# theAdamColton/spiht

Measured on AMD Instinct MI355X. Metric: Mpixels/sec encode+decode at fixed bpp; bitstream-exact vs Rust ref, higher is better.
Workload: dtype f64 DWT / int32 bit-plane coding; 1 GPU; cfg2 image (1920x1080 RGB, bior2.2 reflect level 7, q=50, 0.5 bpp) x 256 per GPU (cfg4 shard), encode+decode, HBM-resident; images_per_gpu=256, distinct_images_per_gpu=256, seeds=1000 + global image index, streams=1, images_per_launch=256, decoder_waves=8, max_bits=1036800

## Files before the change

include/spiht_hip.h:

```cpp
#ifndef SPIHT_HIP_H
#define SPIHT_HIP_H

#include <stdint.h>

#ifdef __cplusplus
extern "C" {
#endif

enum {
    SPIHT_OK = 0,
    SPIHT_ERR_LL = 1,
    SPIHT_ERR_EMPTY = 2,
    SPIHT_ERR_SHAPE = 3,
    SPIHT_ERR_CAPACITY = 4,
    SPIHT_ERR_HIP = 5,
    SPIHT_ERR_ARG = 6,
    SPIHT_ERR_MAGNITUDE = 7,
    SPIHT_ERR_INTERNAL = 8,
    SPIHT_ERR_TOO_LARGE = 9,
    SPIHT_ERR_NOMEM = 10
};

enum { SPIHT_MODE_REFLECT = 0, SPIHT_MODE_SYMMETRIC = 1, SPIHT_MODE_PERIODIC = 2, SPIHT_MODE_ZERO = 3,
       SPIHT_MODE_CONSTANT = 4,
// ... 85 lines not shown
                                 int64_t H, int64_t W, int wavelet, int mode, int level, double q_scale,
                                 const double *channel_mults, uint64_t max_bits, uint8_t *d_out, uint64_t slot_stride,
                                 uint64_t *d_nbits, uint8_t *d_max_n, int32_t *d_coeffs);
int spiht_decode_image_batch_u8(spiht_ctx *ctx, const uint8_t *d_data, uint64_t slot_stride,
                                const uint64_t *d_nbytes, const uint8_t *d_max_n, int64_t B, int64_t c, int64_t H,
                                int64_t W, int wavelet, int mode, int level, double q_scale,
                                const double *channel_mults, uint8_t *d_img_out, const int64_t *out_strides,
                                int32_t *d_rec);
int spiht_decode_image_batch_u16(spiht_ctx *ctx, const uint8_t *d_data, uint64_t slot_stride,
                                 const uint64_t *d_nbytes, const uint8_t *d_max_n, int64_t B, int64_t c, int64_t H,
                                 int64_t W, int wavelet, int mode, int level, double q_scale,
                                 const double *channel_mults, uint16_t *d_img_out, const int64_t *out_strides,
                                 int32_t *d_rec);

int spiht_dwt_quant_batch_f64(spiht_ctx *ctx, const double *d_img, int64_t B, int64_t c, int64_t H, int64_t W,
                              int wavelet, int mode, int level, double q_scale, const double *channel_mults,
                              int32_t *d_coeffs);
int spiht_dequant_idwt_batch_f64(spiht_ctx *ctx, const int32_t *d_rec, int64_t B, int64_t c, int64_t H, int64_t W,
                                 int wavelet, int mode, int level, double q_scale, const double *channel_mults,
                                 double *d_img_out);

int spiht_dwt_quant_batch_f32(spiht_ctx *ctx, const float *d_img, int64_t B, int64_t c, int64_t H, int64_t W,
                              int wavelet, int mode, int level, double q_scale, const double *channel_mults,
                              int32_t *d_coeffs);
int spiht_encode_image_batch_f32(spiht_ctx *ctx, const float *d_img, int64_t B, int64_t c, int64_t H, int64_t W,
                                 int wavelet, int mode, int level, double q_scale, const double *channel_mults,
                                 uint64_t max_bits, uint8_t *d_out, uint64_t slot_stride, uint64_t *d_nbits,
                                 uint8_t *d_max_n, int32_t *d_coeffs);

int spiht_pyramid_batch_i32(spiht_ctx *ctx, const int32_t *d_x, int64_t B, int64_t c, int64_t h, int64_t w,
                            int64_t ll_h, int64_t ll_w, uint8_t *d_dmsb, uint8_t *d_lmsb, uint32_t *d_maxabs);

int spiht_dwt_pyramid_batch_f64(spiht_ctx *ctx, const double *d_img, int64_t B, int64_t c, int64_t H, int64_t W,
                                int wavelet, int mode, int level, double q_scale, const double *channel_mults,
                                int32_t *d_coeffs, uint8_t *d_dmsb, uint8_t *d_lmsb, uint32_t *d_maxabs);
int spiht_dwt_pyramid_batch_u8(spiht_ctx *ctx, const uint8_t *d_img, const int64_t *strides, int64_t B, int64_t c, int64_t H,
                               int64_t W, int wavelet, int mode, int level, double q_scale, const double *channel_mults,
                               int32_t *d_coeffs, uint8_t *d_dmsb, uint8_t *d_lmsb, uint32_t *d_maxabs);
int spiht_dwt_pyramid_batch_u16(spiht_ctx *ctx, const uint16_t *d_img, const int64_t *strides, int64_t B, int64_t c, int64_t H,
                                int64_t W, int wavelet, int mode, int level, double q_scale, const double *channel_mults,
                                int32_t *d_coeffs, uint8_t *d_dmsb, uint8_t *d_lmsb, uint32_t *d_maxabs);
int spiht_encode_lists_batch_i32(spiht_ctx *ctx, const int32_t *d_x, const uint8_t *d_dmsb, const uint8_t *d_lmsb,
                                 const uint32_t *d_maxabs, int64_t B, int64_t c, int64_t h, int64_t w, int64_t ll_h,
                                 int64_t ll_w, uint64_t max_bits, uint8_t *d_out, uint64_t slot_stride,
                                 uint64_t *d_nbits, uint8_t *d_max_n);
int spiht_decode_lists_batch_i32(spiht_ctx *ctx, const uint8_t *d_data, uint64_t slot_stride, const uint64_t *d_nbytes,
                                 const uint8_t *d_max_n, int64_t B, int64_t c, int64_t h, int64_t w, int64_t ll_h,
                                 int64_t ll_w, int32_t *d_out_zeroed);
int spiht_unscatter_lists_batch_i32(spiht_ctx *ctx, int32_t *d_out, int64_t B, int64_t c, int64_t h, int64_t w);
int spiht_l1_flags_words(int64_t c, int64_t H, int64_t W, int wavelet, int mode, int level, uint64_t *words_per_image);
int spiht_decode_lists_flags_batch_i32(spiht_ctx *ctx, const uint8_t *d_data, uint64_t slot_stride, const uint64_t *d_nbytes,
                                       const uint8_t *d_max_n, int64_t B, int64_t c, int64_t H, int64_t W, int wavelet,
                                       int mode, int level, int32_t *d_out_zeroed, uint32_t *d_flags);
int spiht_dequant_idwt_flags_batch_f64(spiht_ctx *ctx, const int32_t *d_rec, const uint32_t *d_flags, int64_t B, int64_t c,
                                       int64_t H, int64_t W, int wavelet, int mode, int level, double q_scale,
                                       const double *channel_mults, double *d_img_out);
int spiht_dequant_idwt_flags_batch_u8(spiht_ctx *ctx, const int32_t *d_rec, const uint32_t *d_flags, int64_t B, int64_t c,
                                      int64_t H, int64_t W, int wavelet, int mode, int level, double q_scale,
                                      const double *channel_mults, uint8_t *d_img_out, const int64_t *out_strides);
int spiht_dequant_idwt_flags_batch_u16(spiht_ctx *ctx, const int32_t *d_rec, const uint32_t *d_flags, int64_t B, int64_t c,
                                       int64_t H, int64_t W, int wavelet, int mode, int level, double q_scale,
                                       const double *channel_mults, uint16_t *d_img_out, const int64_t *out_strides);
int spiht_ctx_set_option(spiht_ctx *ctx, const char *name, int64_t value);
int spiht_ctx_get_option(spiht_ctx *ctx, const char *name, int64_t *value);
int spiht_ctx_wide_stats(spiht_ctx *ctx, uint32_t *groups, uint32_t *gave_up);

int spiht_idwt_coarse_batch_f64(spiht_ctx *ctx, const int32_t *d_rec, int64_t B, int64_t c, int64_t H, int64_t W,
                                int wavelet, int mode, int level, double q_scale, const double *channel_mults,
                                double *d_approx);
int spiht_idwt_level1_batch_f64(spiht_ctx *ctx, const int32_t *d_rec, const double *d_approx, int64_t B, int64_t c,
                                int64_t H, int64_t W, int wavelet, int mode, int level, double q_scale,
                                const double *channel_mults, double *d_img_out);
int spiht_idwt_approx_shape(int64_t H, int64_t W, int wavelet, int level, int64_t *a_h, int64_t *a_w);
int spiht_idwt_level1_flags_batch_f64(spiht_ctx *ctx, const int32_t *d_rec, const double *d_approx, const uint32_t *d_flags,
                                      int64_t B, int64_t c, int64_t H, int64_t W, int wavelet, int mode, int level, double q_scale,
                                      const double *channel_mults, double *d_img_out);
int spiht_idwt_level1_flags_batch_u8(spiht_ctx *ctx, const int32_t *d_rec, const double *d_approx, const uint32_t *d_flags,
                                     int64_t B, int64_t c, int64_t H, int64_t W, int wavelet, int mode, int level, double q_scale,
                                     const double *channel_mults, uint8_t *d_img_out, const int64_t *out_strides);
int spiht_idwt_level1_flags_batch_u16(spiht_ctx *ctx, const int32_t *d_rec, const double *d_approx, const uint32_t *d_flags,
                                      int64_t B, int64_t c, int64_t H, int64_t W, int wavelet, int mode, int level, double q_scale,
                                      const double *channel_mults, uint16_t *d_img_out, const int64_t *out_strides);

int spiht_color3_batch_f64(spiht_ctx *ctx, const double *d_in, double *d_out, int64_t B, int64_t npix, const double *A,
                           const double *M, double p);
int spiht_ctx_set_color3(spiht_ctx *ctx, const double *A_f, const double *M_f, double p_f, const double *A_i,
                         const double *M_i, double p_i);
int spiht_ctx_get_color3(spiht_ctx *ctx, int *on, double *A_f, double *M_f, double *p_f, double *A_i, double *M_i, double *p_i);

int spiht_decode_budgets_i32(spiht_ctx *ctx, const uint8_t *data, uint64_t nbytes, uint8_t n, int64_t c, int64_t h, int64_t w,
                             int64_t ll_h, int64_t ll_w, const uint64_t *budgets_bits, int64_t K, int32_t *out);
int spiht_decode_budgets_dev_i32(spiht_ctx *ctx, const uint8_t *data, uint64_t nbytes, uint8_t n, int64_t c, int64_t h,
                                 int64_t w, int64_t ll_h, int64_t ll_w, const uint64_t *budgets_bits, int64_t K, int32_t *d_out);

int spiht_ctx_lock(spiht_ctx *ctx);
int spiht_ctx_unlock(spiht_ctx *ctx);

int spiht_ctx_set_decoder_waves(spiht_ctx *ctx, int waves);

int spiht_nbits_to_nbytes(spiht_ctx *ctx, const uint64_t *d_nbits, int64_t B, uint64_t *d_nbytes);

int spiht_encode_image_host_f64(spiht_ctx *ctx, const double *img, int64_t c, int64_t H, int64_t W, int wavelet,
                                int mode, int level, double q_scale, const double *channel_mults, uint64_t max_bits,
                                uint8_t *out, uint64_t out_cap, uint64_t *out_nbits, uint8_t *max_n);
int spiht_encode_image_host_f32(spiht_ctx *ctx, const float *img, int64_t c, int64_t H, int64_t W, int wavelet,
                                int mode, int level, double q_scale, const double *channel_mults, uint64_t max_bits,
                                uint8_t *out, uint64_t out_cap, uint64_t *out_nbits, uint8_t *max_n);
int spiht_decode_image_host_f64(spiht_ctx *ctx, const uint8_t *data, uint64_t nbytes, uint8_t n, int64_t c, int64_t H,
                                int64_t W, int wavelet, int mode, int level, double q_scale, const double *channel_mults,
                                double *img_out);
int spiht_dequant_idwt_host_f64(spiht_ctx *ctx, const int32_t *rec, int64_t c, int64_t H, int64_t W, int wavelet, int mode,
                                int level, double q_scale, const double *channel_mults, double *img_out);
int spiht_encode_image_host_u8(spiht_ctx *ctx, const uint8_t *img, const int64_t *strides, int64_t c, int64_t H, int64_t W,
                               int wavelet, int mode, int level, double q_scale, const double *channel_mults,
                               uint64_t max_bits, uint8_t *out, uint64_t out_cap, uint64_t *out_nbits, uint8_t *max_n);
int spiht_encode_image_host_u16(spiht_ctx *ctx, const uint16_t *img, const int64_t *strides, int64_t c, int64_t H, int64_t W,
                                int wavelet, int mode, int level, double q_scale, const double *channel_mults,
                                uint64_t max_bits, uint8_t *out, uint64_t out_cap, uint64_t *out_nbits, uint8_t *max_n);
int spiht_decode_image_host_u8(spiht_ctx *ctx, const uint8_t *data, uint64_t nbytes, uint8_t n, int64_t c, int64_t H,
                               int64_t W, int wavelet, int mode, int level, double q_scale, const double *channel_mults,
                               uint8_t *img_out, const int64_t *strides);
int spiht_decode_image_host_u16(spiht_ctx *ctx, const uint8_t *data, uint64_t nbytes, uint8_t n, int64_t c, int64_t H,
                                int64_t W, int wavelet, int mode, int level, double q_scale, const double *channel_mults,
                                uint16_t *img_out, const int64_t *strides);

int spiht_reduced_shape(int64_t H, int64_t W, int wavelet, int mode, int level, int reduce, int *level_used, int64_t *rec_h,
                        int64_t *rec_w, int64_t *pic_h, int64_t *pic_w, int64_t *off_y, int64_t *off_x, int64_t *in_h,
                        int64_t *in_w);
int spiht_dequant_idwt_reduced_batch_f64(spiht_ctx *ctx, const int32_t *d_rec, int64_t B, int64_t c, int64_t H, int64_t W,
                                         int wavelet, int mode, int level, double q_scale, const double *channel_mults,
                                         double *d_img_out, int reduce);
int spiht_dequant_idwt_reduced_batch_u8(spiht_ctx *ctx, const int32_t *d_rec, int64_t B, int64_t c, int64_t H, int64_t W,
                                        int wavelet, int mode, int level, double q_scale, const double *channel_mults,
                                        uint8_t *d_img_out, const int64_t *out_strides, int reduce);
int spiht_dequant_idwt_reduced_batch_u16(spiht_ctx *ctx, const int32_t *d_rec, int64_t B, int64_t c, int64_t H, int64_t W,
// ... 277 lines not shown
```

spiht_amd/_lib.py:

```python
import ctypes as C
import os
import threading

_HERE = os.path.dirname(os.path.abspath(__file__))
LIB_PATH = os.environ.get("SPIHT_HIP_LIB") or os.path.join(_HERE, "libspiht_hip.so")

OK, ERR_LL, ERR_EMPTY, ERR_SHAPE, ERR_CAPACITY, ERR_HIP, ERR_ARG, ERR_MAGNITUDE, ERR_INTERNAL, ERR_TOO_LARGE, \
    ERR_NOMEM = range(11)
ERR_BUSY, ERR_TIMEOUT, ERR_IDLE = 11, 12, 13

MODES = {"reflect": 0, "symmetric": 1, "periodic": 2, "zero": 3, "constant": 4}


class SpihtHipError(RuntimeError):
    """A HIP runtime failure or an internal guard of libspiht_hip."""


class PanicException(BaseException):
    """Counterpart of pyo3_runtime.PanicException, which the reference raises when the Rust core panics
    (assert!(ll_h > 1), encoder_decoder.rs:160-161; out-of-bounds index; unwrap on an empty array).
    Like PyO3's, it derives from BaseException."""


_lib = None
_lib_lock = threading.Lock()

SYMBOLS = [
    "spiht_strerror", "spiht_last_hip_error", "spiht_abi_version", "spiht_ctx_create", "spiht_ctx_create_priority", "spiht_ctx_resident_ticket", "spiht_ctx_wait_resident",
    "spiht_ctx_destroy",
    "spiht_ctx_synchronize", "spiht_ctx_wait_on", "spiht_event_create", "spiht_event_destroy", "spiht_event_record",
    "spiht_ctx_wait_event", "spiht_ctx_stream", "spiht_dwt_pyramid_batch_f64", "spiht_encode_lists_batch_i32",
    "spiht_decode_lists_batch_i32", "spiht_unscatter_lists_batch_i32", "spiht_ctx_set_timing", "spiht_ctx_reset_timing", "spiht_ctx_num_stages",
    "spiht_ctx_stage_name", "spiht_ctx_get_timing", "spiht_encode_i32", "spiht_encode_bound", "spiht_decode_i32",
    "spiht_decode_with_metadata_i32", "spiht_encode_batch_i32", "spiht_decode_batch_i32", "spiht_wavelet_id", "spiht_mode_id", "spiht_geometry",
    "spiht_encode_image_batch_f64", "spiht_decode_image_batch_f64", "spiht_dwt_quant_batch_f64",
    "spiht_encode_image_batch_f32", "spiht_dwt_quant_batch_f32",
    "spiht_dequant_idwt_batch_f64", "spiht_pyramid_batch_i32", "spiht_color3_batch_f64", "spiht_ctx_set_color3", "spiht_ctx_get_color3", "spiht_ctx_set_decoder_waves", "spiht_decode_budgets_i32", "spiht_decode_budgets_dev_i32", "spiht_nbits_to_nbytes", "spiht_dev_alloc", "spiht_dev_free", "spiht_host_alloc", "spiht_host_free",
    "spiht_dev_upload", "spiht_dev_download", "spiht_dev_memset", "spiht_dev_copy",
    "spiht_idwt_coarse_batch_f64", "spiht_idwt_level1_batch_f64", "spiht_idwt_level1_flags_batch_f64", "spiht_idwt_approx_shape",
    "spiht_encode_image_host_f64", "spiht_encode_image_host_f32", "spiht_decode_image_host_f64",
    "spiht_dequant_idwt_host_f64",
    "spiht_comm_unique_id", "spiht_comm_create", "spiht_comm_destroy", "spiht_comm_info", "spiht_gather_streams", "spiht_gather_row_offsets",
    "spiht_comm_barrier", "spiht_comm_allreduce_max_f64", "spiht_rccl_library", "spiht_ctx_lock", "spiht_ctx_unlock",
    "spiht_pipeline_create", "spiht_pipeline_create_on", "spiht_pipeline_destroy", "spiht_pipeline_info", "spiht_pipeline_set_color3", "spiht_pipeline_submit",
    "spiht_pipeline_submit_gather", "spiht_pipeline_flush", "spiht_pipeline_synchronize", "spiht_pipeline_contexts",
    "spiht_geometry_mode", "spiht_wavelet_taps", "spiht_ctx_set_option", "spiht_ctx_get_option", "spiht_ctx_wide_stats", "spiht_l1_flags_words", "spiht_decode_lists_flags_batch_i32", "spiht_dequant_idwt_flags_batch_f64",
    "spiht_encode_image_batch_u8", "spiht_decode_image_batch_u8", "spiht_encode_image_host_u8", "spiht_decode_image_host_u8",
    "spiht_dwt_pyramid_batch_u8", "spiht_dequant_idwt_flags_batch_u8", "spiht_idwt_level1_flags_batch_u8", "spiht_pipeline_submit_u8",
    "spiht_check_view_u8", "spiht_decode_with_metadata_batch_i32",
    "spiht_encode_image_batch_u16", "spiht_decode_image_batch_u16", "spiht_encode_image_host_u16", "spiht_decode_image_host_u16",
    "spiht_dwt_pyramid_batch_u16", "spiht_dequant_idwt_flags_batch_u16", "spiht_idwt_level1_flags_batch_u16", "spiht_pipeline_submit_u16",
    "spiht_check_view_u16",
    "spiht_reduced_shape",
    "spiht_dequant_idwt_reduced_batch_f64", "spiht_dequant_idwt_reduced_batch_u8", "spiht_dequant_idwt_reduced_batch_u16",
    "spiht_decode_image_reduced_batch_f64", "spiht_decode_image_reduced_batch_u8", "spiht_decode_image_reduced_batch_u16",
    "spiht_decode_image_reduced_host_f64", "spiht_decode_image_reduced_host_u8", "spiht_decode_image_reduced_host_u16",
    "spiht_sqerr_i32", "spiht_sse_f64", "spiht_sse_u8", "spiht_sse_u16",
    "spiht_tile_grid", "spiht_tile_cut_u8", "spiht_tile_cut_u16", "spiht_tile_cut_f32", "spiht_tile_cut_f64",
    "spiht_tile_paste_u8", "spiht_tile_paste_u16", "spiht_tile_paste_f32", "spiht_tile_paste_f64",
    "spiht_tile_pack", "spiht_tile_unpack",
    "spiht_tile_reduced_grid", "spiht_tile_mosaic_u8", "spiht_tile_mosaic_u16", "spiht_tile_mosaic_f64",
    "spiht_tile_prefix_slots", "spiht_sse_tiles_f64", "spiht_sse_tiles_u8", "spiht_sse_tiles_u16", "spiht_tile_allocate",
    "spiht_layer_pack", "spiht_layer_unpack",
    "spiht_sse_tiles_w_f64", "spiht_sse_tiles_w_u8", "spiht_sse_tiles_w_u16",
    "spiht_tile_allocate_target",
    "spiht_tile_cut_overlap_u8", "spiht_tile_cut_overlap_u16", "spiht_tile_cut_overlap_f32", "spiht_tile_cut_overlap_f64",
    "spiht_tile_blend_u8", "spiht_tile_blend_u16", "spiht_tile_blend_f64",
    "spiht_check_view_flt", "spiht_convert_batch_flt", "spiht_decode_image_batch_flt", "spiht_decode_image_host_flt",
    "spiht_dequant_idwt_flags_batch_flt", "spiht_dequant_idwt_reduced_batch_flt", "spiht_decode_image_reduced_batch_flt",
    "spiht_decode_image_reduced_host_flt", "spiht_tile_blend_flt", "spiht_tile_paste_f32s", "spiht_tile_mosaic_f32",
    "spiht_dwt_addr32",
    "spiht_widen_batch_flt", "spiht_encode_image_batch_flt", "spiht_encode_image_host_flt", "spiht_dwt_pyramid_batch_flt",
    "spiht_sse_tiles_flt", "spiht_sse_tiles_w_flt", "spiht_tile_cut_f32s", "spiht_tile_cut_overlap_f32s",
    "spiht_hstream_create", "spiht_hstream_destroy", "spiht_hstream_info", "spiht_hstream_input", "spiht_hstream_decode_input",
    "spiht_hstream_submit", "spiht_hstream_next", "spiht_hstream_pending",
    "spiht_tile_cut_set", "spiht_tile_paste_set",
]


class HStreamResult(C.Structure):
    _fields_ = [("n", C.c_int64), ("nbytes", C.c_uint64), ("bytes", C.c_void_p), ("lens", C.c_void_p), ("max_n", C.c_void_p),
                ("pictures", C.c_void_p), ("step", C.c_uint64)]


class TileSetPic(C.Structure):
    _fields_ = [("d_img", C.c_void_p), ("sc", C.c_int64), ("sh", C.c_int64), ("sw", C.c_int64), ("H", C.c_int64), ("W", C.c_int64)]


class TileSetItem(C.Structure):
    _fields_ = [("d_out", C.c_void_p), ("sc", C.c_int64), ("sh", C.c_int64), ("sw", C.c_int64), ("H", C.c_int64), ("W", C.c_int64),
                ("i0", C.c_int64), ("i1", C.c_int64), ("j0", C.c_int64), ("j1", C.c_int64),
                ("y0", C.c_int64), ("x0", C.c_int64), ("wh", C.c_int64), ("ww", C.c_int64)]


def lib():
    global _lib
    with _lib_lock:
        if _lib is not None:
            return _lib
        if not os.path.exists(LIB_PATH):
            raise ImportError(
                "libspiht_hip.so is missing (%s): build it with `python -c 'import __graft_entry__ as g; g.build()'` "
                "or `make -C spiht_amd/csrc`; spiht_amd has no CPU fallback" % LIB_PATH)
        try:
            L = C.CDLL(LIB_PATH)
        except OSError as e:
            raise ImportError("cannot load %s: %s" % (LIB_PATH, e))
        i64, u64, u8, i32 = C.c_int64, C.c_uint64, C.c_uint8, C.c_int
        vp = C.c_void_p
        L.spiht_strerror.restype = C.c_char_p
        L.spiht_strerror.argtypes = [i32]
        L.spiht_last_hip_error.restype = C.c_char_p
        L.spiht_ctx_create.argtypes = [i32, C.POINTER(vp)]
        L.spiht_ctx_create_priority.argtypes = [i32, i32, C.POINTER(vp)]
        L.spiht_ctx_resident_ticket.argtypes = [vp, C.POINTER(vp), C.POINTER(C.c_uint32)]
        L.spiht_ctx_wait_resident.argtypes = [vp, vp, C.c_uint32, C.c_uint32]
        L.spiht_ctx_destroy.argtypes = [vp]
        L.spiht_ctx_destroy.restype = None
        L.spiht_ctx_synchronize.argtypes = [vp]
        L.spiht_ctx_wait_on.argtypes = [vp, vp]
        L.spiht_event_create.argtypes = [vp, C.POINTER(vp)]
        L.spiht_event_destroy.argtypes = [vp]
        L.spiht_event_destroy.restype = None
        L.spiht_event_record.argtypes = [vp, vp]
        L.spiht_ctx_wait_event.argtypes = [vp, vp]
        L.spiht_ctx_stream.argtypes = [vp, C.POINTER(vp)]
        L.spiht_dwt_pyramid_batch_f64.argtypes = [vp, vp, i64, i64, i64, i64, i32, i32, i32, C.c_double, vp, vp, vp, vp, vp]
        L.spiht_encode_lists_batch_i32.argtypes = [vp, vp, vp, vp, vp, i64, i64, i64, i64, i64, i64, u64, vp, u64, vp, vp]
        L.spiht_decode_lists_batch_i32.argtypes = [vp, vp, u64, vp, vp, i64, i64, i64, i64, i64, i64, vp]
        L.spiht_unscatter_lists_batch_i32.argtypes = [vp, vp, i64, i64, i64, i64]
        L.spiht_color3_batch_f64.argtypes = [vp, vp, vp, i64, i64, vp, vp, C.c_double]
        L.spiht_ctx_set_color3.argtypes = [vp, vp, vp, C.c_double, vp, vp, C.c_double]
        L.spiht_ctx_get_color3.argtypes = [vp, C.POINTER(i32), vp, vp, C.POINTER(C.c_double), vp, vp, C.POINTER(C.c_double)]
        L.spiht_ctx_set_decoder_waves.argtypes = [vp, C.c_int]
        L.spiht_decode_budgets_i32.argtypes = [vp, vp, u64, C.c_uint8, i64, i64, i64, i64, i64, vp, i64, vp]
        L.spiht_decode_budgets_dev_i32.argtypes = [vp, vp, u64, C.c_uint8, i64, i64, i64, i64, i64, vp, i64, vp]
        L.spiht_ctx_set_timing.argtypes = [vp, i32]
        L.spiht_ctx_reset_timing.argtypes = [vp]
        L.spiht_ctx_stage_name.restype = C.c_char_p
        L.spiht_ctx_stage_name.argtypes = [i32]
        L.spiht_ctx_get_timing.argtypes = [vp, i32, C.POINTER(C.c_double), C.POINTER(u64)]
        L.spiht_encode_i32.argtypes = [vp, vp, i64, i64, i64, i64, i64, i64, i64, i64, u64, vp, u64, C.POINTER(u64),
                                       C.POINTER(u8)]
        L.spiht_encode_bound.argtypes = [i64, i64, i64, i64, i64, C.c_uint32, u64, C.POINTER(u64)]
        L.spiht_decode_i32.argtypes = [vp, vp, u64, u8, i64, i64, i64, i64, i64, vp]
        L.spiht_decode_with_metadata_i32.argtypes = [vp, vp, u64, u8, i64, i64, i64, i64, i64, vp, vp, i64, vp, vp]
        L.spiht_encode_batch_i32.argtypes = [vp, vp, i64, i64, i64, i64, i64, i64, u64, vp, u64, vp, vp]
        L.spiht_decode_batch_i32.argtypes = [vp, vp, u64, vp, vp, i64, i64, i64, i64, i64, i64, vp]
        L.spiht_decode_with_metadata_batch_i32.argtypes = [vp, vp, u64, vp, vp, i64, i64, i64, i64, i64, i64, vp, vp, i64, vp,
                                                           vp, u64]
        L.spiht_wavelet_id.argtypes = [C.c_char_p]
        L.spiht_mode_id.argtypes = [C.c_char_p]
        L.spiht_wavelet_taps.argtypes = [i32]
        L.spiht_geometry.argtypes = [i64, i64, i32, i32, C.POINTER(i32)] + [C.POINTER(i64)] * 6
        L.spiht_encode_image_batch_f64.argtypes = [vp, vp, i64, i64, i64, i64, i32, i32, i32, C.c_double, vp, u64, vp,
                                                   u64, vp, vp, vp]
        L.spiht_decode_image_batch_f64.argtypes = [vp, vp, u64, vp, vp, i64, i64, i64, i64, i32, i32, i32, C.c_double,
                                                   vp, vp, vp]
        L.spiht_dwt_quant_batch_f64.argtypes = [vp, vp, i64, i64, i64, i64, i32, i32, i32, C.c_double, vp, vp]
        L.spiht_dwt_quant_batch_f32.argtypes = L.spiht_dwt_quant_batch_f64.argtypes
        L.spiht_encode_image_batch_f32.argtypes = L.spiht_encode_image_batch_f64.argtypes
        L.spiht_dequant_idwt_batch_f64.argtypes = [vp, vp, i64, i64, i64, i64, i32, i32, i32, C.c_double, vp, vp]
        L.spiht_pyramid_batch_i32.argtypes = [vp, vp, i64, i64, i64, i64, i64, i64, vp, vp, vp]
        L.spiht_nbits_to_nbytes.argtypes = [vp, vp, i64, vp]
        L.spiht_dev_alloc.argtypes = [vp, u64, C.POINTER(vp)]
        L.spiht_dev_free.argtypes = [vp, vp]
        L.spiht_dev_upload.argtypes = [vp, vp, vp, u64]
        L.spiht_dev_download.argtypes = [vp, vp, vp, u64]
        L.spiht_dev_memset.argtypes = [vp, vp, i32, u64]
        L.spiht_dev_copy.argtypes = [vp, vp, vp, u64]
        L.spiht_idwt_coarse_batch_f64.argtypes = [vp, vp, i64, i64, i64, i64, i32, i32, i32, C.c_double, vp, vp]
        L.spiht_idwt_level1_batch_f64.argtypes = [vp, vp, vp, i64, i64, i64, i64, i32, i32, i32, C.c_double, vp, vp]
        L.spiht_idwt_level1_flags_batch_f64.argtypes = [vp, vp, vp, vp, i64, i64, i64, i64, i32, i32, i32, C.c_double, vp, vp]
        L.spiht_idwt_approx_shape.argtypes = [i64, i64, i32, i32, C.POINTER(i64), C.POINTER(i64)]
        L.spiht_encode_image_host_f64.argtypes = [vp, vp, i64, i64, i64, i32, i32, i32, C.c_double, vp, u64, vp, u64,
                                                  C.POINTER(u64), C.POINTER(u8)]
        L.spiht_encode_image_host_f32.argtypes = L.spiht_encode_image_host_f64.argtypes
        L.spiht_decode_image_host_f64.argtypes = [vp, vp, u64, u8, i64, i64, i64, i32, i32, i32, C.c_double, vp, vp]
        L.spiht_dequant_idwt_host_f64.argtypes = [vp, vp, i64, i64, i64, i32, i32, i32, C.c_double, vp, vp]
        L.spiht_comm_unique_id.argtypes = [vp]
        L.spiht_comm_create.argtypes = [vp, vp, i32, i32, C.POINTER(vp)]
        L.spiht_comm_destroy.argtypes = [vp]
        L.spiht_comm_destroy.restype = None
        L.spiht_comm_info.argtypes = [vp, C.POINTER(i32), C.POINTER(i32), C.POINTER(i32)]
        L.spiht_gather_streams.argtypes = [vp, vp, vp, vp, vp, i64, u64, vp, vp, vp]
        L.spiht_gather_row_offsets.argtypes = [i32, i32, i64, u64, C.POINTER(u64), C.POINTER(u64), C.POINTER(u64)]
        L.spiht_comm_barrier.argtypes = [vp, vp]
        L.spiht_comm_allreduce_max_f64.argtypes = [vp, vp, C.POINTER(C.c_double)]
        L.spiht_rccl_library.restype = C.c_char_p
        L.spiht_rccl_library.argtypes = []
        L.spiht_host_alloc.argtypes = [u64, C.POINTER(vp)]
        L.spiht_host_free.argtypes = [vp]
        L.spiht_ctx_set_option.argtypes = [vp, C.c_char_p, i64]
        L.spiht_ctx_get_option.argtypes = [vp, C.c_char_p, C.POINTER(i64)]
        L.spiht_ctx_wide_stats.argtypes = [vp, C.POINTER(C.c_uint32), C.POINTER(C.c_uint32)]
        L.spiht_l1_flags_words.argtypes = [i64, i64, i64, i32, i32, i32, C.POINTER(u64)]
        L.spiht_decode_lists_flags_batch_i32.argtypes = [vp, vp, u64, vp, vp, i64, i64, i64, i64, i32, i32, i32, vp, vp]
        L.spiht_geometry_mode.argtypes = [i64, i64, i32, i32, i32, C.POINTER(i32)] + [C.POINTER(i64)] * 6
        L.spiht_dequant_idwt_flags_batch_f64.argtypes = [vp, vp, vp, i64, i64, i64, i64, i32, i32, i32, C.c_double, vp, vp]
        L.spiht_pipeline_create.argtypes = [i32, i64, i64, i64, i64, i32, i32, i32, C.c_double, vp, u64, C.POINTER(vp)]
        L.spiht_pipeline_create_on.argtypes = [vp, i32, i64, i64, i64, i64, i32, i32, i32, C.c_double, vp, u64, C.POINTER(vp)]
        L.spiht_pipeline_destroy.argtypes = [vp]
        L.spiht_pipeline_destroy.restype = None
        L.spiht_pipeline_info.argtypes = [vp, C.POINTER(u64), C.POINTER(i64), C.POINTER(i64)]
        L.spiht_pipeline_set_color3.argtypes = [vp, vp, vp, C.c_double, vp, vp, C.c_double]
        L.spiht_pipeline_submit.argtypes = [vp, vp, vp, vp, vp, vp]
        L.spiht_pipeline_submit_gather.argtypes = [vp, vp, vp, vp, vp, vp, vp, vp, vp, vp, i32]
        L.spiht_pipeline_flush.argtypes = [vp]
        L.spiht_pipeline_synchronize.argtypes = [vp]
        L.spiht_pipeline_contexts.argtypes = [vp, C.POINTER(vp), C.POINTER(vp), C.POINTER(vp)]
        L.spiht_encode_image_batch_u8.argtypes = [vp, vp, vp, i64, i64, i64, i64, i32, i32, i32, C.c_double, vp, u64, vp,
                                                  u64, vp, vp, vp]
        L.spiht_decode_image_batch_u8.argtypes = [vp, vp, u64, vp, vp, i64, i64, i64, i64, i32, i32, i32, C.c_double,
                                                  vp, vp, vp, vp]
        L.spiht_encode_image_host_u8.argtypes = [vp, vp, vp, i64, i64, i64, i32, i32, i32, C.c_double, vp, u64, vp, u64,
                                                 C.POINTER(u64), C.POINTER(u8)]
        L.spiht_decode_image_host_u8.argtypes = [vp, vp, u64, u8, i64, i64, i64, i32, i32, i32, C.c_double, vp, vp, vp]
        L.spiht_dwt_pyramid_batch_u8.argtypes = [vp, vp, vp, i64, i64, i64, i64, i32, i32, i32, C.c_double, vp, vp, vp, vp, vp]
        L.spiht_dequant_idwt_flags_batch_u8.argtypes = [vp, vp, vp, i64, i64, i64, i64, i32, i32, i32, C.c_double, vp, vp, vp]
        L.spiht_idwt_level1_flags_batch_u8.argtypes = [vp, vp, vp, vp, i64, i64, i64, i64, i32, i32, i32, C.c_double, vp, vp, vp]
        L.spiht_pipeline_submit_u8.argtypes = [vp, vp, vp, vp, vp, vp, vp, vp]
        L.spiht_check_view_u8.argtypes = [i64, i64, i64, i64, vp, i32]
        L.spiht_reduced_shape.argtypes = [i64, i64, i32, i32, i32, i32, C.POINTER(i32)] + [C.POINTER(i64)] * 8
        L.spiht_dequant_idwt_reduced_batch_f64.argtypes = L.spiht_dequant_idwt_batch_f64.argtypes + [i32]
        L.spiht_dequant_idwt_reduced_batch_u8.argtypes = [vp, vp, i64, i64, i64, i64, i32, i32, i32, C.c_double, vp, vp, vp, i32]
        L.spiht_decode_image_reduced_batch_f64.argtypes = L.spiht_decode_image_batch_f64.argtypes + [i32]
        L.spiht_decode_image_reduced_batch_u8.argtypes = L.spiht_decode_image_batch_u8.argtypes + [i32]
        L.spiht_decode_image_reduced_host_f64.argtypes = L.spiht_decode_image_host_f64.argtypes + [i32]
        L.spiht_decode_image_reduced_host_u8.argtypes = L.spiht_decode_image_host_u8.argtypes + [i32]
        L.spiht_sqerr_i32.argtypes = [vp, vp, vp, i64, i64, i64, i64, vp]
        L.spiht_sse_f64.argtypes = [vp, vp, vp, i64, i64, i64, i64, i64, i64, vp]
        L.spiht_sse_u8.argtypes = [vp, vp, vp, vp, i64, i64, i64, i64, vp]
        L.spiht_tile_grid.argtypes = [i64, i64, i64, i64, C.POINTER(i64), C.POINTER(i64)]
        L.spiht_tile_cut_u8.argtypes = [vp, vp, vp] + [i64] * 6 + [vp]
        L.spiht_tile_cut_f32.argtypes = L.spiht_tile_cut_f64.argtypes = [vp, vp] + [i64] * 6 + [vp]
        L.spiht_tile_paste_u8.argtypes = [vp, vp] + [i64] * 15 + [vp, vp]
        L.spiht_tile_paste_f32.argtypes = L.spiht_tile_paste_f64.argtypes = [vp, vp] + [i64] * 15 + [vp]
        L.spiht_tile_pack.argtypes = [vp, vp, u64, vp, i64, vp, u64, vp]
        L.spiht_tile_unpack.argtypes = [vp, vp, u64, vp, i64, vp, u64, vp]
        L.spiht_tile_reduced_grid.argtypes = [i64, i64, i64, i64, i32, i32, i32, i32, C.POINTER(i32)] + [C.POINTER(i64)] * 12
        L.spiht_tile_mosaic_u8.argtypes = [vp, vp] + [i64] * 17 + [vp, vp]
        L.spiht_tile_mosaic_f64.argtypes = [vp, vp] + [i64] * 17 + [vp]
        L.spiht_tile_prefix_slots.argtypes = [vp, vp, u64, vp, i64, i64, i64, i64, vp, u64, vp, vp, vp]
        L.spiht_sse_tiles_f64.argtypes = L.spiht_sse_tiles_u8.argtypes = [vp, vp, vp] + [i64] * 9 + [vp]
        L.spiht_tile_allocate.argtypes = [vp, vp, vp, i32, i64, i64, i64, u64, vp, vp]
        L.spiht_tile_allocate_target.argtypes = [vp, vp, vp, i32, i64, i64, i64, u64, vp, vp, vp, vp, vp]
        L.spiht_sse_tiles_w_f64.argtypes = L.spiht_sse_tiles_w_u8.argtypes = L.spiht_sse_tiles_f64.argtypes + [vp, u64]
        L.spiht_layer_pack.argtypes = [vp, vp, u64, vp, i64, i64, i64, vp, u64, vp, vp]
        L.spiht_layer_unpack.argtypes = [vp, vp, u64, vp, i64, i64, i64, vp, i64, vp, u64, vp]
        L.spiht_tile_cut_overlap_u8.argtypes = [vp, vp, vp] + [i64] * 7 + [vp]
        L.spiht_tile_cut_overlap_f32.argtypes = L.spiht_tile_cut_overlap_f64.argtypes = [vp, vp] + [i64] * 7 + [vp]
        L.spiht_tile_blend_u8.argtypes = [vp, vp] + [i64] * 16 + [vp, vp]
        L.spiht_tile_blend_f64.argtypes = [vp, vp] + [i64] * 16 + [vp]
        for name in SYMBOLS:
            if name.endswith("_u16"):
                getattr(L, name).argtypes = getattr(L, name[:-2] + "8").argtypes
                getattr(L, name).restype = getattr(L, name[:-2] + "8").restype
        for name in SYMBOLS:
            if name.endswith("_flt") and name not in ("spiht_convert_batch_flt", "spiht_widen_batch_flt"):
                a = getattr(L, name[:-3] + "u8").argtypes
                getattr(L, name).argtypes = [i32] + a if name == "spiht_check_view_flt" else a[:1] + [i32] + a[1:]
        L.spiht_convert_batch_flt.argtypes = [vp, i32, vp] + [i64] * 6 + [vp, vp]
        L.spiht_widen_batch_flt.argtypes = [vp, i32, vp, vp] + [i64] * 4 + [vp]
        L.spiht_tile_paste_f32s.argtypes = L.spiht_tile_paste_u8.argtypes
        L.spiht_tile_cut_f32s.argtypes = L.spiht_tile_cut_u8.argtypes
        L.spiht_tile_cut_overlap_f32s.argtypes = L.spiht_tile_cut_overlap_u8.argtypes
        L.spiht_tile_mosaic_f32.argtypes = L.spiht_tile_mosaic_u8.argtypes
        L.spiht_ctx_lock.argtypes = [vp]
        L.spiht_ctx_unlock.argtypes = [vp]
        L.spiht_hstream_create.argtypes = [vp, i32, i32, i64, i32, i64, i64, i64, i32, i32, i32, C.c_double, vp, u64, vp, C.POINTER(vp)]
        L.spiht_hstream_destroy.argtypes = [vp]
        L.spiht_hstream_info.argtypes = [vp, C.POINTER(u64), C.POINTER(u64), C.POINTER(i64), C.POINTER(i64)]
        L.spiht_hstream_input.argtypes = [vp, C.POINTER(vp)]
# ... 186 lines not shown
```

spiht_amd/csrc/api_coder.cpp:

```cpp
#include "api_internal.h"

int make_geom(int64_t c, int64_t h, int64_t w, int64_t ll_h, int64_t ll_w, Geom *g) {
    if (!(ll_h > 1) || !(ll_w > 1)) return SPIHT_ERR_LL;
    if (c <= 0 || h <= 0 || w <= 0) return SPIHT_ERR_EMPTY;
    int64_t need_h = (ll_h % 2 == 0) ? 2 * ll_h : 2 * ll_h - 1;
    int64_t need_w = (ll_w % 2 == 0) ? 2 * ll_w : 2 * ll_w - 1;
    if (h < need_h || w < need_w) return SPIHT_ERR_SHAPE;
    if ((double)c * (double)h * (double)w >= 1073741824.0) return SPIHT_ERR_TOO_LARGE;
    g->c = (int32_t)c; g->h = (int32_t)h; g->w = (int32_t)w;
    g->ll_h = (int32_t)ll_h; g->ll_w = (int32_t)ll_w;
    g->hw = (uint32_t)(h * w);
    g->n = (uint32_t)(c * h * w);
    g->pad = 0;
    g->div_w = fastdiv_make((uint32_t)w);
    g->div_hw = fastdiv_make(g->hw);
    return SPIHT_OK;
}

static void instance_counts(const Geom &g, uint64_t *nodes, uint64_t *parents) {
    const uint64_t h = (uint64_t)g.h, w = (uint64_t)g.w;
    const uint64_t he = h & ~1ull, we = w & ~1ull;
    const uint64_t hp = h / 2, wp = w / 2;
    uint64_t nn = (uint64_t)g.ll_h * g.ll_w, pp = 0;
    for (int64_t i = 0; i < g.ll_h; i++)
// ... 165 lines not shown
        static std::mutex wide_mu;
        static hipEvent_t wide_last[64] = {};
        {
            std::lock_guard<std::mutex> wl(wide_mu);
            hipEvent_t &ev = wide_last[ctx->device & 63];
            if (ev) HIPCHK(hipStreamWaitEvent(ctx->stream, ev, 0));
            else HIPCHK(hipEventCreateWithFlags(&ev, hipEventDisableTiming));
            LAUNCHCHK(spiht_launch_encode_wide(&a, &w, B, ctx->stream));
            HIPCHK(hipEventRecord(ev, ctx->stream));
        }
        a.redo = w.ctl;
        a.nslots = B;
        LAUNCHCHK(spiht_launch_encode(&a, ctx->stream));
        return SPIHT_OK;
    }
    {
        StageTimer t(ctx, ST_ENC_LISTS);
        LAUNCHCHK(spiht_launch_encode(&a, ctx->stream));
    }
    return SPIHT_OK;
}

int decode_device(spiht_ctx *ctx, const Geom &g, const uint8_t *d_data, uint64_t slot_stride, const uint64_t *d_nbytes,
                  const uint8_t *d_maxn, int B, int32_t *d_out, uint32_t *d_tr_ent, uint8_t *d_tr_act, uint64_t tr_stride,
                  bool zero_out, DecArgs *args_out, const L1Flags *fl) {
    if (slot_stride % 4 != 0) return SPIHT_ERR_ARG;
    if (slot_stride * 8 >= 0xFFFFFF00ull) return SPIHT_ERR_TOO_LARGE;
    ListCaps caps;
    list_caps(g, slot_stride * 8, &caps, nullptr);
    int nslots = 0;
    ListPtrs lp;
    CHK(alloc_lists(ctx, caps, std::min(B, ctx->num_cu * 8), true, &nslots, &lp));
    if (zero_out) {
        StageTimer t(ctx, ST_MEMSET);
        HIPCHK(hipMemsetAsync(d_out, 0, (size_t)B * g.n * 4, ctx->stream));
    }
    DecArgs a;
    memset(&a, 0, sizeof(a));
    a.g = g;
    a.caps = caps;
    a.B = B;
    a.nslots = nslots;
    a.data = d_data;
    a.slot_stride = slot_stride;
    a.nbytes = d_nbytes;
    a.max_n = d_maxn;
    a.out = d_out;
    a.lip0 = lp.lip0; a.lip1 = lp.lip1; a.lsp_idx = lp.lsp; a.lsp_val = lp.lsp_val;
    a.lis0 = lp.lis0; a.lis1 = lp.lis1; a.lis2 = lp.lis2;
    a.err = (uint32_t *)ctx->err.p;
    a.tr_ent = d_tr_ent; a.tr_act = d_tr_act; a.tr_stride = tr_stride;
    if (fl && fl->p) {
        a.fl = *fl;
        HIPCHK(hipMemsetAsync(fl->p, 0, (size_t)B * g.c * fl->gy * fl->gx * 4, ctx->stream));
    }
    if (args_out) {
        CHK(ensure(ctx, ctx->lspcnt, (size_t)nslots * 4));
        a.lsp_count = (uint32_t *)ctx->lspcnt.p;
    }
    {
        StageTimer t(ctx, ST_DEC_LISTS);
        LAUNCHCHK(ctx->dec_waves == 8 ? spiht_launch_decode_w8(&a, ctx->stream) : spiht_launch_decode(&a, ctx->stream));
    }
    if (args_out) *args_out = a;
    return SPIHT_OK;
}


extern "C" int spiht_encode_bound(int64_t c, int64_t h, int64_t w, int64_t ll_h, int64_t ll_w, uint32_t max_abs,
                                  uint64_t max_bits, uint64_t *bound_bytes) {
    if (!bound_bytes) return SPIHT_ERR_ARG;
    Geom g;
    CHK(make_geom(c, h, w, ll_h, ll_w, &g));
    uint64_t bits = bound_bits(g, max_abs);
    if (max_bits != 0) bits = std::min(bits, max_bits);
    *bound_bytes = ((bits + 7) / 8 + 3) & ~3ull;
    return SPIHT_OK;
}

int read_encoded(spiht_ctx *ctx, uint8_t *out, uint64_t out_cap, uint64_t *out_nbits, uint8_t *max_n) {
    uint64_t nbits = 0;
    uint8_t mn = 0;
    HIPCHK(hipMemcpyAsync(&nbits, ctx->nbits.p, 8, hipMemcpyDeviceToHost, ctx->stream));
    HIPCHK(hipMemcpyAsync(&mn, ctx->maxn.p, 1, hipMemcpyDeviceToHost, ctx->stream));
    CHK(take_err(ctx));
    *out_nbits = nbits;
    *max_n = mn;
    const uint64_t nbytes = (nbits + 7) / 8;
    if (nbytes > out_cap) return SPIHT_ERR_CAPACITY;
    if (nbytes) {
        StageTimer t(ctx, ST_D2H);
        HIPCHK(hipMemcpyAsync(out, ctx->out.p, nbytes, hipMemcpyDeviceToHost, ctx->stream));
    }
    HIPCHK(hipStreamSynchronize(ctx->stream));
    return SPIHT_OK;
}

int stage_stream(spiht_ctx *ctx, const uint8_t *data, uint64_t nbytes, uint8_t n, uint64_t *slot) {
    *slot = std::max<uint64_t>(4, (nbytes + 3) & ~3ull);
    CHK(ensure(ctx, ctx->data, *slot));
    CHK(ensure(ctx, ctx->nbytes, 8));
    CHK(ensure(ctx, ctx->maxn, 4));
    CHK(take_err(ctx));
    StageTimer t(ctx, ST_H2D);
    HIPCHK(hipMemsetAsync((char *)ctx->data.p + (*slot - 4), 0, 4, ctx->stream));
    if (nbytes) HIPCHK(hipMemcpyAsync(ctx->data.p, data, nbytes, hipMemcpyHostToDevice, ctx->stream));
    HIPCHK(hipMemcpyAsync(ctx->nbytes.p, &nbytes, 8, hipMemcpyHostToDevice, ctx->stream));
// ... 343 lines not shown
        StageTimer t(ctx, ST_PYRAMID);
        LAUNCHCHK(spiht_launch_pyramid(&g, (int)B, d_x, d_dmsb, d_lmsb, ctx->stream));
    }
    return SPIHT_OK;
}

extern "C" int spiht_encode_lists_batch_i32(spiht_ctx *ctx, const int32_t *d_x, const uint8_t *d_dmsb,
                                            const uint8_t *d_lmsb, const uint32_t *d_maxabs, int64_t B, int64_t c,
                                            int64_t h, int64_t w, int64_t ll_h, int64_t ll_w, uint64_t max_bits_in,
                                            uint8_t *d_out, uint64_t slot_stride, uint64_t *d_nbits, uint8_t *d_max_n) {
    if (!ctx || !d_x || !d_dmsb || !d_lmsb || !d_maxabs || !d_out || !d_nbits || !d_max_n || B < 0) return SPIHT_ERR_ARG;
    Geom g;
    CHK(make_geom(c, h, w, ll_h, ll_w, &g));
    if (B == 0) return SPIHT_OK;
    if (slot_stride % 4 != 0) return SPIHT_ERR_ARG;
    std::lock_guard<std::recursive_mutex> lk(ctx->mu);
    HIPCHK(hipSetDevice(ctx->device));
    const uint64_t max_bits = max_bits_in == 0 ? SPIHT_MAX_BITS_UNLIMITED : max_bits_in;
    ListCaps caps;
    list_caps(g, std::min<uint64_t>(max_bits, slot_stride * 8), &caps, nullptr);
    return batch_chunks(B, c, [&](int64_t b0, int nb) -> int {
        int nslots = 0;
        ListPtrs lp;
        CHK(alloc_lists(ctx, caps, std::min(nb, ctx->num_cu), false, &nslots, &lp));
        return encode_lists_device(ctx, g, d_x + (size_t)b0 * g.n, d_dmsb + (size_t)b0 * g.n, d_lmsb + (size_t)b0 * g.n,
                                   d_maxabs + b0, nb, max_bits, caps, nslots, lp, d_out + (size_t)b0 * slot_stride, slot_stride,
                                   d_nbits + b0, d_max_n + b0);
    });
}

static int decode_lists_batch(spiht_ctx *ctx, const uint8_t *d_data, uint64_t slot_stride, const uint64_t *d_nbytes,
                              const uint8_t *d_max_n, int64_t B, const Geom &g, int32_t *d_out_zeroed, const L1Flags *fl) {
    if (B == 0) return SPIHT_OK;
    std::lock_guard<std::recursive_mutex> lk(ctx->mu);
    HIPCHK(hipSetDevice(ctx->device));
    DecArgs da;
    CHK(decode_device(ctx, g, d_data, slot_stride, d_nbytes, d_max_n, (int)B, d_out_zeroed, nullptr, nullptr, 0, false, &da, fl));
    ctx->last_dec = da;
    ctx->last_dec_valid = da.nslots >= (int)B;
    return SPIHT_OK;
}
extern "C" int spiht_decode_lists_batch_i32(spiht_ctx *ctx, const uint8_t *d_data, uint64_t slot_stride,
                                            const uint64_t *d_nbytes, const uint8_t *d_max_n, int64_t B, int64_t c,
                                            int64_t h, int64_t w, int64_t ll_h, int64_t ll_w, int32_t *d_out_zeroed) {
    if (!ctx || !d_data || !d_nbytes || !d_max_n || !d_out_zeroed || B < 0) return SPIHT_ERR_ARG;
    Geom g;
    CHK(make_geom(c, h, w, ll_h, ll_w, &g));
    return decode_lists_batch(ctx, d_data, slot_stride, d_nbytes, d_max_n, B, g, d_out_zeroed, nullptr);
}
extern "C" int spiht_decode_lists_flags_batch_i32(spiht_ctx *ctx, const uint8_t *d_data, uint64_t slot_stride,
                                                  const uint64_t *d_nbytes, const uint8_t *d_max_n, int64_t B, int64_t c,
                                                  int64_t H, int64_t W, int wavelet, int mode, int level, int32_t *d_out_zeroed,
                                                  uint32_t *d_flags) {
    if (!ctx || !d_data || !d_nbytes || !d_max_n || !d_out_zeroed || B < 0) return SPIHT_ERR_ARG;
    ImgCall k;
    int st;
    if (!k.open(&st, ctx, 1, c, H, W, wavelet, mode, level, true)) return st;
    L1Flags fl;
    const bool flagged = d_flags && l1flags_geometry(k.ig, k.F, &fl);
    if (flagged) fl.p = d_flags;
    return decode_lists_batch(ctx, d_data, slot_stride, d_nbytes, d_max_n, B, k.g, d_out_zeroed, flagged ? &fl : nullptr);
}

extern "C" int spiht_unscatter_lists_batch_i32(spiht_ctx *ctx, int32_t *d_out, int64_t B, int64_t c, int64_t h, int64_t w) {
    if (!ctx || !d_out || B < 0 || c < 1 || h < 1 || w < 1) return SPIHT_ERR_ARG;
    if (B == 0) return SPIHT_OK;
    std::lock_guard<std::recursive_mutex> lk(ctx->mu);
    HIPCHK(hipSetDevice(ctx->device));
    StageTimer t(ctx, ST_MEMSET);
    const DecArgs &da = ctx->last_dec;
    if (ctx->last_dec_valid && da.out == d_out && da.B == (int)B && (int64_t)da.g.n == c * h * w) {
        LAUNCHCHK(spiht_launch_unscatter(&da, ctx->stream));
    } else {
        HIPCHK(hipMemsetAsync(d_out, 0, (size_t)B * (size_t)(c * h * w) * 4, ctx->stream));
    }
    return SPIHT_OK;
}

extern "C" int spiht_nbits_to_nbytes(spiht_ctx *ctx, const uint64_t *d_nbits, int64_t B, uint64_t *d_nbytes) {
    if (!ctx || !d_nbits || !d_nbytes || B < 0) return SPIHT_ERR_ARG;
    if (B == 0) return SPIHT_OK;
    std::lock_guard<std::recursive_mutex> lk(ctx->mu);
    HIPCHK(hipSetDevice(ctx->device));
    LAUNCHCHK(spiht_launch_nbits_to_nbytes(d_nbits, (int)B, d_nbytes, ctx->stream));
    return SPIHT_OK;
}
```

spiht_amd/csrc/api_dwt.cpp:

```cpp
#include "api_internal.h"
#include "wavelets.h"

static int dwt_max_level(int64_t len, int F) {
    if (F <= 1 || len < F - 1) return 0;
    int64_t q = len / (F - 1);
    int l = 0;
    while (q > 1) { q >>= 1; l++; }
    return l;
}

int img_geometry(int64_t H, int64_t W, int F_real, int level, ImgGeom *g, int mode) {
    if (H < 1 || W < 1) return SPIHT_ERR_ARG;
    int L = level;
    if (L < 0) L = std::min(dwt_max_level(H, F_real), dwt_max_level(W, F_real));
    if (L > SPIHT_MAX_LEVELS) return SPIHT_ERR_ARG;
    g->per = mode == SPIHT_MODE_PERIODIZATION;
    g->l0 = 0;
    const int F = g->per ? 2 : F_real;
    g->L = L;
    g->hs[0] = H;
    g->ws[0] = W;
    for (int l = 1; l <= L; l++) {
        g->hs[l] = (g->hs[l - 1] + F - 1) / 2;
        g->ws[l] = (g->ws[l - 1] + F - 1) / 2;
// ... 294 lines not shown
        memcpy(a.hi_f, wv.dec_hi_f, sizeof(float) * Fc);
        if (twopass) {
            StageTimer t(ctx, l == 1 ? ST_DWT_L1 : ST_DWT_REST);
            const size_t esz = f32 ? 4 : 8;
            const size_t n_t = (size_t)a.out_h * a.in_w, n_b = (size_t)a.out_h * a.out_w;
            const size_t per_plane = (2 * n_t + 4 * n_b) * esz;
            int pc = (int)std::max<size_t>(1, ((size_t)1 << 30) / per_plane);
            pc = std::max(c, pc / c * c);
            CHK(ensure(ctx, ctx->exttmp, per_plane * (size_t)std::min(pc, planes)));
            for (int p0 = 0; p0 < planes; p0 += pc) {
                const int np = std::min(pc, planes - p0);
                DwtKArgs b = a;
                b.in = (const double *)((const char *)a.in + (size_t)p0 * a.in_h * a.in_w * esz);
                if (b.ll_out) b.ll_out = (double *)((char *)a.ll_out + (size_t)p0 * n_b * esz);
                b.coeffs = a.coeffs + (size_t)p0 * a.enc_h * a.enc_w;
                if (b.maxabs) b.maxabs = a.maxabs + p0 / c;
                char *base = (char *)ctx->exttmp.p;
                void *t_lo = base, *t_hi = base + (size_t)np * n_t * esz;
                char *bb = base + 2 * (size_t)np * n_t * esz;
                LAUNCHCHK(spiht_launch_dwt_level_ext(&b, np, t_lo, t_hi, bb, bb + (size_t)np * n_b * esz, bb + 2 * (size_t)np * n_b * esz,
                                                     bb + 3 * (size_t)np * n_b * esz, d_filt, ctx->stream));
            }
        } else {
            StageTimer t(ctx, l == 1 ? ST_DWT_L1 : ST_DWT_REST);
            LAUNCHCHK(spiht_launch_dwt_level(&a, planes, ctx->stream));
        }
        d_img = a.ll_out;
    }
    return SPIHT_OK;
}

bool l1flags_geometry(const ImgGeom &ig, int F, L1Flags *fl) {
    memset(fl, 0, sizeof(*fl));
    if (ig.per) return false;
    if (ig.L < 2 || F / 2 - 1 > IW_TH / 2 || F / 2 - 1 > IW_TW / 2) return false;
    fl->off_h = (int32_t)ig.offh[1]; fl->off_w = (int32_t)ig.offw[1];
    fl->band_h = (int32_t)ig.hs[1]; fl->band_w = (int32_t)ig.ws[1];
    fl->hf1 = F / 2 - 1;
    fl->gx = (int32_t)((2 * ig.ws[1] - F + 2 + IW_TW - 1) / IW_TW);
    fl->gy = (int32_t)((2 * ig.hs[1] - F + 2 + IW_TH - 1) / IW_TH);
    return fl->gx > 0 && fl->gy > 0;
}
extern "C" int spiht_l1_flags_words(int64_t c, int64_t H, int64_t W, int wavelet, int mode, int level, uint64_t *words_per_image) {
    if (!words_per_image || wavelet < 0 || wavelet >= SPIHT_NWAVELETS || c < 1 || mode < 0 || mode > SPIHT_MODE_PERIODIZATION)
        return SPIHT_ERR_ARG;
    ImgGeom ig;
    CHK(img_geometry(H, W, SPIHT_WAVELETS[wavelet].F, level, &ig, mode));
    L1Flags fl;
    *words_per_image = l1flags_geometry(ig, SPIHT_WAVELETS[wavelet].F, &fl) ? (uint64_t)c * fl.gy * fl.gx : 0;
    return SPIHT_OK;
}

int dwt_inverse(spiht_ctx *ctx, const int32_t *d_rec, int planes, int c, const ImgGeom &ig, int wavelet, double q,
                const double *d_mults, const Pic &out, int l_hi, int l_lo, const double *d_a_in, const uint32_t *d_flags) {
    const WaveletDef &wv = SPIHT_WAVELETS[wavelet];
    const int F = wv.F;
    if (l_hi < 0) l_hi = ig.L;
    const bool strided = out.strided;
    if (strided && (l_lo != 1 || (ig.L == 0 && ig.l0 == 0))) return SPIHT_ERR_ARG;
    double *d_out = strided ? nullptr : (double *)out.p;
    const bool color = ctx->color_on && c == 3;
    if (ig.L == 0 && ig.l0 > 0) {
        StageTimer t(ctx, ST_IDWT_REST);
        LlPicArgs a;
        memset(&a, 0, sizeof(a));
        a.rec = d_rec;
        a.enc_h = (int32_t)ig.enc_h; a.enc_w = (int32_t)ig.enc_w; a.ll_h = (int32_t)ig.ll_h; a.ll_w = (int32_t)ig.ll_w;
        a.c = c; a.mults = d_mults; a.q = q; a.out = d_out;
        if (color) { a.color = 1; a.col = ctx->col_inv; }
        if (strided) a.px = out.view();
        LAUNCHCHK(spiht_launch_ll_to_pic(&a, planes, ctx->stream));
        return SPIHT_OK;
    }
    if (ig.L == 0) {
        StageTimer t(ctx, ST_IDWT_REST);
        LAUNCHCHK(spiht_launch_dequant_plain(d_rec, d_out, (size_t)ig.enc_h * ig.enc_w, planes, c, d_mults, q, ctx->stream));
        if (color)
            LAUNCHCHK(spiht_launch_color3(d_out, d_out, planes / 3, (size_t)ig.enc_h * ig.enc_w, ctx->col_inv.A, ctx->col_inv.M,
                                          ctx->col_inv.p, ctx->stream));
        return SPIHT_OK;
    }
    size_t maxa = 0;
    const int Fg = ig.per ? 2 : F;
    for (int l = l_hi; l > l_lo; l--) maxa = std::max(maxa, (size_t)(2 * ig.hs[l] - Fg + 2) * (size_t)(2 * ig.ws[l] - Fg + 2));
    if (maxa) {
        CHK(ensure(ctx, ctx->a0, maxa * planes * 8));
        CHK(ensure(ctx, ctx->a1, maxa * planes * 8));
    }
    const double *a_in = d_a_in;
    int64_t ah = ig.ll_h, aw = ig.ll_w;
    if (l_hi < ig.L) { ah = 2 * ig.hs[l_hi + 1] - Fg + 2; aw = 2 * ig.ws[l_hi + 1] - Fg + 2; }
    for (int l = l_hi; l >= l_lo; l--) {
        IdwtKArgs a;
        memset(&a, 0, sizeof(a));
        a.c = c;
        a.F = F;
        a.band_h = (int32_t)ig.hs[l]; a.band_w = (int32_t)ig.ws[l];
        a.out_h = (int32_t)(2 * ig.hs[l] - F + 2); a.out_w = (int32_t)(2 * ig.ws[l] - F + 2);
        a.a_h = (int32_t)ah; a.a_w = (int32_t)aw;
        if (!((ah == ig.hs[l] || ah == ig.hs[l] + 1) && (aw == ig.ws[l] || aw == ig.ws[l] + 1))) return SPIHT_ERR_ARG;
        if (ig.per) { a.out_h = (int32_t)(2 * ig.hs[l]); a.out_w = (int32_t)(2 * ig.ws[l]); }
        a.off_h = (int32_t)ig.offh[l]; a.off_w = (int32_t)ig.offw[l];
        a.enc_h = (int32_t)ig.enc_h; a.enc_w = (int32_t)ig.enc_w;
        a.first = (l == ig.L) ? 1 : 0;
        a.a_in = a_in;
        a.rec = d_rec;
        a.out = (l == l_lo) ? d_out : (double *)((l & 1) ? ctx->a1.p : ctx->a0.p);
        a.mults = d_mults;
        a.q = q;
        if (color && l == 1) { a.color = 1; a.col = ctx->col_inv; }
        if (l == 1 && !a.first && !a.color) a.flags = d_flags;
        memcpy(a.lo, wv.rec_lo, sizeof(double) * std::min(F, SPIHT_MAX_TAPS));
        memcpy(a.hi, wv.rec_hi, sizeof(double) * std::min(F, SPIHT_MAX_TAPS));
        const bool conv8 = strided && l == 1 && (ig.per || F > SPIHT_MAX_TAPS);
        if (conv8) {
            CHK(ensure(ctx, ctx->pix, (size_t)planes * a.out_h * a.out_w * 8));
            a.out = (double *)ctx->pix.p;
        }
        if (ig.per || F > SPIHT_MAX_TAPS) {
            const double *d_filt;
            CHK(upload_filters(ctx, wavelet, &d_filt));
            StageTimer t(ctx, l + ig.l0 == 1 ? ST_IDWT_L1 : ST_IDWT_REST);
            a.color = 0;
            const size_t per_plane = (size_t)2 * a.band_h * a.out_w * 8;
            int pc = (int)std::max<size_t>(1, ((size_t)1 << 30) / per_plane);
            pc = std::max(c, pc / c * c);
            CHK(ensure(ctx, ctx->exttmp, per_plane * (size_t)std::min(pc, planes)));
            for (int p0 = 0; p0 < planes; p0 += pc) {
                const int np = std::min(pc, planes - p0);
                IdwtKArgs b = a;
                if (b.a_in) b.a_in = a.a_in + (size_t)p0 * a.a_h * a.a_w;
                b.rec = a.rec + (size_t)p0 * a.enc_h * a.enc_w;
                b.out = a.out + (size_t)p0 * a.out_h * a.out_w;
                double *t_lo = (double *)ctx->exttmp.p, *t_hi = t_lo + (size_t)np * a.band_h * a.out_w;
                LAUNCHCHK(spiht_launch_idwt_level_per(&b, np, t_lo, t_hi, d_filt, ig.per ? 1 : 0, ctx->stream));
            }
            if (color && l == 1)
                LAUNCHCHK(spiht_launch_color3(a.out, a.out, planes / 3, (size_t)a.out_h * a.out_w, ctx->col_inv.A, ctx->col_inv.M,
                                              ctx->col_inv.p, ctx->stream));
            if (conv8) {
                const PxView px = out.view();
                LAUNCHCHK(spiht_launch_f64_to_px(a.out, a.out_h, a.out_w, &px, planes / c, ctx->stream));
            }
        } else {
            if (strided && l == 1) a.px = out.view();
            StageTimer t(ctx, l + ig.l0 == 1 ? ST_IDWT_L1 : ST_IDWT_REST);
            LAUNCHCHK(spiht_launch_idwt_level(&a, planes, ctx->stream, ctx->tilectr.dev ? &ctx->tilectr : nullptr));
        }
        a_in = a.out;
        ah = a.out_h;
        aw = a.out_w;
    }
    return SPIHT_OK;
}

bool ImgCall::open(int *st, spiht_ctx *ctx_, int64_t B_, int64_t c_, int64_t H, int64_t W, int wavelet, int mode, int level, bool coded) {
    ctx = ctx_; B = B_; c = c_;
    *st = check_img_args(wavelet, mode, B, c, H, W);
    if (*st != SPIHT_OK || B == 0) return false;
    F = SPIHT_WAVELETS[wavelet].F;
    *st = img_geometry(H, W, F, level, &ig, mode);
    if (*st == SPIHT_OK && coded) *st = make_geom(c, ig.enc_h, ig.enc_w, ig.ll_h, ig.ll_w, &g);
    pig = ig;
    return *st == SPIHT_OK;
// ... 15 lines not shown
```

spiht_amd/csrc/api_image.cpp:

```cpp
#include "api_internal.h"

static int dwt_quant_batch(spiht_ctx *ctx, const Pic &in, int64_t B, int64_t c, int64_t H, int64_t W, int wavelet, int mode,
                           int level, double q_scale, const double *channel_mults, int32_t *d_coeffs) {
    if (!ctx || !in.p || !d_coeffs) return SPIHT_ERR_ARG;
    ImgCall k;
    int st;
    if (!k.open(&st, ctx, B, c, H, W, wavelet, mode, level, false)) return st;
    CHK(k.enter(channel_mults));
    return k.chunks([&](int64_t b0, int nb) -> int {
        return dwt_forward(ctx, k.at(in, b0), nb * (int)c, (int)c, k.ig, wavelet, mode, q_scale, k.d_mults,
                           d_coeffs + (size_t)b0 * c * k.ig.enc_h * k.ig.enc_w);
    });
}
extern "C" int spiht_dwt_quant_batch_f64(spiht_ctx *ctx, const double *d_img, int64_t B, int64_t c, int64_t H, int64_t W,
                                         int wavelet, int mode, int level, double q_scale, const double *channel_mults,
                                         int32_t *d_coeffs) {
    return dwt_quant_batch(ctx, dense_pic(d_img, EL_F64), B, c, H, W, wavelet, mode, level, q_scale, channel_mults, d_coeffs);
}
extern "C" int spiht_dwt_quant_batch_f32(spiht_ctx *ctx, const float *d_img, int64_t B, int64_t c, int64_t H, int64_t W,
                                         int wavelet, int mode, int level, double q_scale, const double *channel_mults,
                                         int32_t *d_coeffs) {
    return dwt_quant_batch(ctx, dense_pic(d_img, EL_F32), B, c, H, W, wavelet, mode, level, q_scale, channel_mults, d_coeffs);
}

// ... 3 lines not shown
    if (!ctx || !d_rec || !out.p) return SPIHT_ERR_ARG;
    ImgCall k;
    int st;
    if (!k.open(&st, ctx, B, c, H, W, wavelet, mode, level, false) || !k.reduce(&st, reduce, q_scale)) return st;
    CHK(k.enter(channel_mults));
    L1Flags fl;
    const bool flagged = d_flags && reduce == 0 && !(ctx->color_on && c == 3) && l1flags_geometry(k.ig, k.F, &fl);
    return k.chunks([&](int64_t b0, int nb) -> int {
        return dwt_inverse(ctx, d_rec + (size_t)b0 * c * k.ig.enc_h * k.ig.enc_w, nb * (int)c, (int)c, k.pig, wavelet, k.q,
                           k.d_mults, k.at(out, b0), -1, 1, nullptr, flagged ? d_flags + (size_t)b0 * c * fl.gy * fl.gx : nullptr);
    });
}
extern "C" int spiht_dequant_idwt_batch_f64(spiht_ctx *ctx, const int32_t *d_rec, int64_t B, int64_t c, int64_t H,
                                            int64_t W, int wavelet, int mode, int level, double q_scale,
                                            const double *channel_mults, double *d_img_out) {
    return dequant_idwt_batch(ctx, d_rec, nullptr, B, c, H, W, wavelet, mode, level, q_scale, channel_mults,
                              dense_pic(d_img_out, EL_F64, true));
}
extern "C" int spiht_dequant_idwt_flags_batch_f64(spiht_ctx *ctx, const int32_t *d_rec, const uint32_t *d_flags, int64_t B,
                                                  int64_t c, int64_t H, int64_t W, int wavelet, int mode, int level,
                                                  double q_scale, const double *channel_mults, double *d_img_out) {
    return dequant_idwt_batch(ctx, d_rec, d_flags, B, c, H, W, wavelet, mode, level, q_scale, channel_mults,
                              dense_pic(d_img_out, EL_F64, true));
}
static int dequant_idwt_flags_view(PicElem el, spiht_ctx *ctx, const int32_t *d_rec, const uint32_t *d_flags, int64_t B, int64_t c,
                                   int64_t H, int64_t W, int wavelet, int mode, int level, double q_scale,
                                   const double *channel_mults, void *d_img_out, const int64_t *out_strides) {
    Pic out;
    CHK(view_pic(&out, d_img_out, el, true, out_strides, 4, B, c, H, W, PIC_NULL_FIRST));
    return dequant_idwt_batch(ctx, d_rec, d_flags, B, c, H, W, wavelet, mode, level, q_scale, channel_mults, out);
}
extern "C" int spiht_dequant_idwt_flags_batch_u8(spiht_ctx *ctx, const int32_t *d_rec, const uint32_t *d_flags, int64_t B,
                                                 int64_t c, int64_t H, int64_t W, int wavelet, int mode, int level, double q_scale,
                                                 const double *channel_mults, uint8_t *d_img_out, const int64_t *out_strides) {
    return dequant_idwt_flags_view(EL_U8, ctx, d_rec, d_flags, B, c, H, W, wavelet, mode, level, q_scale, channel_mults, d_img_out,
                                   out_strides);
}
extern "C" int spiht_dequant_idwt_flags_batch_u16(spiht_ctx *ctx, const int32_t *d_rec, const uint32_t *d_flags, int64_t B,
                                                  int64_t c, int64_t H, int64_t W, int wavelet, int mode, int level, double q_scale,
                                                  const double *channel_mults, uint16_t *d_img_out, const int64_t *out_strides) {
    return dequant_idwt_flags_view(EL_U16, ctx, d_rec, d_flags, B, c, H, W, wavelet, mode, level, q_scale, channel_mults, d_img_out,
                                   out_strides);
}
extern "C" int spiht_dequant_idwt_flags_batch_flt(spiht_ctx *ctx, int kind, const int32_t *d_rec, const uint32_t *d_flags,
                                                  int64_t B, int64_t c, int64_t H, int64_t W, int wavelet, int mode, int level,
                                                  double q_scale, const double *channel_mults, void *d_img_out,
                                                  const int64_t *out_strides) {
    return dequant_idwt_flags_view(el_of_kind(kind), ctx, d_rec, d_flags, B, c, H, W, wavelet, mode, level, q_scale, channel_mults,
                                   d_img_out, out_strides);
}

static int idwt_part(spiht_ctx *ctx, const int32_t *d_rec, double *d_approx, int64_t B, int64_t c, int64_t H, int64_t W,
                     int wavelet, int mode, int level, double q_scale, const double *channel_mults, const Pic &out,
                     const uint32_t *d_flags = nullptr) {
    if (!ctx || !d_rec || (!d_approx && !out.p)) return SPIHT_ERR_ARG;
    ImgCall k;
    int st;
    if (!k.open(&st, ctx, B, c, H, W, wavelet, mode, level, false)) return st;
    const ImgGeom &ig = k.ig;
    if (ig.per) return SPIHT_ERR_ARG;
    const bool coarse = !out.p;
    if (coarse && ig.L < 2) return SPIHT_OK;
    if (!coarse && ig.L >= 2 && !d_approx) return SPIHT_ERR_ARG;
    CHK(k.enter(channel_mults));
    const int F = k.F;
    const size_t a_plane = ig.L >= 2 ? (size_t)(2 * ig.hs[2] - F + 2) * (size_t)(2 * ig.ws[2] - F + 2) : 0;
    L1Flags fl;
    const bool flagged = d_flags && !(ctx->color_on && c == 3) && l1flags_geometry(ig, F, &fl);
    return k.chunks([&](int64_t b0, int nb) -> int {
        const int32_t *rec = d_rec + (size_t)b0 * c * ig.enc_h * ig.enc_w;
        double *ap = d_approx ? d_approx + (size_t)b0 * c * a_plane : nullptr;
        if (coarse)
            return dwt_inverse(ctx, rec, nb * (int)c, (int)c, ig, wavelet, q_scale, k.d_mults, dense_pic(ap, EL_F64, true), ig.L, 2,
                               nullptr);
        return dwt_inverse(ctx, rec, nb * (int)c, (int)c, ig, wavelet, q_scale, k.d_mults, k.at(out, b0), std::min(ig.L, 1), 1,
                           ig.L >= 2 ? ap : nullptr, flagged ? d_flags + (size_t)b0 * c * fl.gy * fl.gx : nullptr);
    });
}
extern "C" int spiht_idwt_coarse_batch_f64(spiht_ctx *ctx, const int32_t *d_rec, int64_t B, int64_t c, int64_t H, int64_t W,
                                           int wavelet, int mode, int level, double q_scale, const double *channel_mults,
                                           double *d_approx) {
    return idwt_part(ctx, d_rec, d_approx, B, c, H, W, wavelet, mode, level, q_scale, channel_mults, Pic());
}
extern "C" int spiht_idwt_level1_batch_f64(spiht_ctx *ctx, const int32_t *d_rec, const double *d_approx, int64_t B, int64_t c,
                                           int64_t H, int64_t W, int wavelet, int mode, int level, double q_scale,
                                           const double *channel_mults, double *d_img_out) {
    return spiht_idwt_level1_flags_batch_f64(ctx, d_rec, d_approx, nullptr, B, c, H, W, wavelet, mode, level, q_scale, channel_mults,
                                             d_img_out);
}
extern "C" int spiht_idwt_level1_flags_batch_f64(spiht_ctx *ctx, const int32_t *d_rec, const double *d_approx, const uint32_t *d_flags,
                                                 int64_t B, int64_t c, int64_t H, int64_t W, int wavelet, int mode, int level,
                                                 double q_scale, const double *channel_mults, double *d_img_out) {
    if (!d_img_out) return SPIHT_ERR_ARG;
    return idwt_part(ctx, d_rec, const_cast<double *>(d_approx), B, c, H, W, wavelet, mode, level, q_scale, channel_mults,
                     dense_pic(d_img_out, EL_F64, true), d_flags);
}
static int idwt_level1_flags_view(PicElem el, spiht_ctx *ctx, const int32_t *d_rec, const double *d_approx, const uint32_t *d_flags,
                                  int64_t B, int64_t c, int64_t H, int64_t W, int wavelet, int mode, int level, double q_scale,
                                  const double *channel_mults, void *d_img_out, const int64_t *out_strides) {
    Pic out;
    CHK(view_pic(&out, d_img_out, el, true, out_strides, 4, B, c, H, W, PIC_NULL_FIRST));
    return idwt_part(ctx, d_rec, const_cast<double *>(d_approx), B, c, H, W, wavelet, mode, level, q_scale, channel_mults, out,
                     d_flags);
}
extern "C" int spiht_idwt_level1_flags_batch_u8(spiht_ctx *ctx, const int32_t *d_rec, const double *d_approx, const uint32_t *d_flags,
                                                int64_t B, int64_t c, int64_t H, int64_t W, int wavelet, int mode, int level,
                                                double q_scale, const double *channel_mults, uint8_t *d_img_out,
                                                const int64_t *out_strides) {
    return idwt_level1_flags_view(EL_U8, ctx, d_rec, d_approx, d_flags, B, c, H, W, wavelet, mode, level, q_scale, channel_mults,
                                  d_img_out, out_strides);
}
extern "C" int spiht_idwt_level1_flags_batch_u16(spiht_ctx *ctx, const int32_t *d_rec, const double *d_approx, const uint32_t *d_flags,
                                                 int64_t B, int64_t c, int64_t H, int64_t W, int wavelet, int mode, int level,
                                                 double q_scale, const double *channel_mults, uint16_t *d_img_out,
                                                 const int64_t *out_strides) {
    return idwt_level1_flags_view(EL_U16, ctx, d_rec, d_approx, d_flags, B, c, H, W, wavelet, mode, level, q_scale, channel_mults,
                                  d_img_out, out_strides);
}

int encode_image_batch(spiht_ctx *ctx, const Pic &in, int64_t B, int64_t c, int64_t H, int64_t W, int wavelet, int mode, int level,
                       double q_scale, const double *channel_mults, uint64_t max_bits, uint8_t *d_out, uint64_t slot_stride,
                       uint64_t *d_nbits, uint8_t *d_max_n, int32_t *d_coeffs) {
    if (!ctx || !in.p || !d_out || !d_nbits || !d_max_n) return SPIHT_ERR_ARG;
    ImgCall k;
    int st;
    if (!k.open(&st, ctx, B, c, H, W, wavelet, mode, level, true)) return st;
    CHK(k.enter(channel_mults));
    const Geom &g = k.g;
    return k.chunks([&](int64_t b0, int nb) -> int {
        int32_t *co = d_coeffs ? d_coeffs + (size_t)b0 * g.n : nullptr;
        if (!co) {
            CHK(ensure(ctx, ctx->coeffs, (size_t)nb * g.n * 4));
            co = (int32_t *)ctx->coeffs.p;
        }
        CHK(ensure(ctx, ctx->maxabs, (size_t)nb * 4));
        HIPCHK(hipMemsetAsync(ctx->maxabs.p, 0, (size_t)nb * 4, ctx->stream));
        CHK(dwt_forward(ctx, k.at(in, b0), nb * (int)c, (int)c, k.ig, wavelet, mode, q_scale, k.d_mults, co,
                        (uint32_t *)ctx->maxabs.p));
        return encode_device(ctx, g, co, nb, max_bits, d_out + (size_t)b0 * slot_stride, slot_stride, d_nbits + b0, d_max_n + b0,
                             true);
    });
}
extern "C" int spiht_encode_image_batch_f64(spiht_ctx *ctx, const double *d_img, int64_t B, int64_t c, int64_t H, int64_t W,
                                            int wavelet, int mode, int level, double q_scale, const double *channel_mults,
                                            uint64_t max_bits, uint8_t *d_out, uint64_t slot_stride, uint64_t *d_nbits,
                                            uint8_t *d_max_n, int32_t *d_coeffs) {
    return encode_image_batch(ctx, dense_pic(d_img, EL_F64), B, c, H, W, wavelet, mode, level, q_scale, channel_mults, max_bits,
                              d_out, slot_stride, d_nbits, d_max_n, d_coeffs);
}
extern "C" int spiht_encode_image_batch_f32(spiht_ctx *ctx, const float *d_img, int64_t B, int64_t c, int64_t H, int64_t W,
                                            int wavelet, int mode, int level, double q_scale, const double *channel_mults,
                                            uint64_t max_bits, uint8_t *d_out, uint64_t slot_stride, uint64_t *d_nbits,
                                            uint8_t *d_max_n, int32_t *d_coeffs) {
    return encode_image_batch(ctx, dense_pic(d_img, EL_F32), B, c, H, W, wavelet, mode, level, q_scale, channel_mults, max_bits,
                              d_out, slot_stride, d_nbits, d_max_n, d_coeffs);
}
int encode_image_batch_view(PicElem el, spiht_ctx *ctx, const void *d_img, const int64_t *strides, int64_t B, int64_t c, int64_t H,
                            int64_t W, int wavelet, int mode, int level, double q_scale, const double *channel_mults,
                            uint64_t max_bits, uint8_t *d_out, uint64_t slot_stride, uint64_t *d_nbits, uint8_t *d_max_n,
                            int32_t *d_coeffs) {
    Pic in;
    CHK(view_pic(&in, d_img, el, false, strides, 4, B, c, H, W, PIC_NULL_FIRST | PIC_IMG_ARGS, wavelet, mode));
    return encode_image_batch(ctx, in, B, c, H, W, wavelet, mode, level, q_scale, channel_mults, max_bits, d_out, slot_stride,
                              d_nbits, d_max_n, d_coeffs);
}
extern "C" int spiht_encode_image_batch_u8(spiht_ctx *ctx, const uint8_t *d_img, const int64_t *strides, int64_t B, int64_t c,
                                           int64_t H, int64_t W, int wavelet, int mode, int level, double q_scale,
                                           const double *channel_mults, uint64_t max_bits, uint8_t *d_out,
                                           uint64_t slot_stride, uint64_t *d_nbits, uint8_t *d_max_n, int32_t *d_coeffs) {
    return encode_image_batch_view(EL_U8, ctx, d_img, strides, B, c, H, W, wavelet, mode, level, q_scale, channel_mults, max_bits,
                                   d_out, slot_stride, d_nbits, d_max_n, d_coeffs);
}
extern "C" int spiht_encode_image_batch_u16(spiht_ctx *ctx, const uint16_t *d_img, const int64_t *strides, int64_t B, int64_t c,
                                            int64_t H, int64_t W, int wavelet, int mode, int level, double q_scale,
                                            const double *channel_mults, uint64_t max_bits, uint8_t *d_out,
                                            uint64_t slot_stride, uint64_t *d_nbits, uint8_t *d_max_n, int32_t *d_coeffs) {
    return encode_image_batch_view(EL_U16, ctx, d_img, strides, B, c, H, W, wavelet, mode, level, q_scale, channel_mults, max_bits,
                                   d_out, slot_stride, d_nbits, d_max_n, d_coeffs);
}
extern "C" int spiht_encode_image_batch_flt(spiht_ctx *ctx, int kind, const void *d_img, const int64_t *strides, int64_t B,
                                            int64_t c, int64_t H, int64_t W, int wavelet, int mode, int level, double q_scale,
                                            const double *channel_mults, uint64_t max_bits, uint8_t *d_out,
                                            uint64_t slot_stride, uint64_t *d_nbits, uint8_t *d_max_n, int32_t *d_coeffs) {
    return encode_image_batch_view(el_of_kind(kind), ctx, d_img, strides, B, c, H, W, wavelet, mode, level, q_scale, channel_mults,
                                   max_bits, d_out, slot_stride, d_nbits, d_max_n, d_coeffs);
}

int decode_image_batch(spiht_ctx *ctx, const uint8_t *d_data, uint64_t slot_stride, const uint64_t *d_nbytes, const uint8_t *d_max_n,
                       int64_t B, int64_t c, int64_t H, int64_t W, int wavelet, int mode, int level, double q_scale,
                       const double *channel_mults, const Pic &out, int32_t *d_rec, int reduce) {
    if (!ctx || !d_data || !d_nbytes || !d_max_n || !out.p) return SPIHT_ERR_ARG;
    ImgCall k;
    int st;
    if (!k.open(&st, ctx, B, c, H, W, wavelet, mode, level, true) || !k.reduce(&st, reduce, q_scale)) return st;
    CHK(k.enter(channel_mults));
    const Geom &g = k.g;
    return k.chunks([&](int64_t b0, int nb) -> int {
        int32_t *rec = d_rec ? d_rec + (size_t)b0 * g.n : nullptr;
        L1Flags fl;
        const bool flagged = ctx->opt_l1_flags && reduce == 0 && !(ctx->color_on && c == 3) && l1flags_geometry(k.ig, k.F, &fl);
        if (flagged) {
            CHK(ensure(ctx, ctx->l1flags, (size_t)nb * c * fl.gy * fl.gx * 4));
            fl.p = (uint32_t *)ctx->l1flags.p;
        }
        if (rec) {
            CHK(decode_device(ctx, g, d_data + (size_t)b0 * slot_stride, slot_stride, d_nbytes + b0, d_max_n + b0, nb, rec,
                              nullptr, nullptr, 0, true, nullptr, flagged ? &fl : nullptr));
            return dwt_inverse(ctx, rec, nb * (int)c, (int)c, k.pig, wavelet, k.q, k.d_mults, k.at(out, b0), -1, 1, nullptr,
                               flagged ? fl.p : nullptr);
        }
        const size_t old_cap = ctx->recz.cap;
        CHK(ensure(ctx, ctx->recz, (size_t)nb * g.n * 4));
        if (ctx->recz.cap != old_cap || !ctx->recz_clean) {
            StageTimer t(ctx, ST_MEMSET);
            HIPCHK(hipMemsetAsync(ctx->recz.p, 0, ctx->recz.cap, ctx->stream));
            ctx->recz_clean = true;
        }
        rec = (int32_t *)ctx->recz.p;
        DecArgs da;
        CHK(decode_device(ctx, g, d_data + (size_t)b0 * slot_stride, slot_stride, d_nbytes + b0, d_max_n + b0, nb, rec, nullptr,
                          nullptr, 0, false, &da, flagged ? &fl : nullptr));
        CHK(dwt_inverse(ctx, rec, nb * (int)c, (int)c, k.pig, wavelet, k.q, k.d_mults, k.at(out, b0), -1, 1, nullptr,
                        flagged ? fl.p : nullptr));
        if (da.nslots >= nb) {
            StageTimer t(ctx, ST_MEMSET);
            LAUNCHCHK(spiht_launch_unscatter(&da, ctx->stream));
        } else {
            ctx->recz_clean = false;
        }
        return SPIHT_OK;
    });
}
extern "C" int spiht_decode_image_batch_f64(spiht_ctx *ctx, const uint8_t *d_data, uint64_t slot_stride,
                                            const uint64_t *d_nbytes, const uint8_t *d_max_n, int64_t B, int64_t c,
                                            int64_t H, int64_t W, int wavelet, int mode, int level, double q_scale,
                                            const double *channel_mults, double *d_img_out, int32_t *d_rec) {
    return decode_image_batch(ctx, d_data, slot_stride, d_nbytes, d_max_n, B, c, H, W, wavelet, mode, level, q_scale,
                              channel_mults, dense_pic(d_img_out, EL_F64, true), d_rec);
}
int decode_image_batch_view(PicElem el, spiht_ctx *ctx, const uint8_t *d_data, uint64_t slot_stride, const uint64_t *d_nbytes,
                            const uint8_t *d_max_n, int64_t B, int64_t c, int64_t H, int64_t W, int wavelet, int mode, int level,
                            double q_scale, const double *channel_mults, void *d_img_out, const int64_t *out_strides,
                            int32_t *d_rec) {
    Pic out;
    CHK(view_pic(&out, d_img_out, el, true, out_strides, 4, B, c, H, W, PIC_NULL_FIRST | PIC_IMG_ARGS, wavelet, mode));
    return decode_image_batch(ctx, d_data, slot_stride, d_nbytes, d_max_n, B, c, H, W, wavelet, mode, level, q_scale,
                              channel_mults, out, d_rec);
}
extern "C" int spiht_decode_image_batch_u8(spiht_ctx *ctx, const uint8_t *d_data, uint64_t slot_stride, const uint64_t *d_nbytes,
                                           const uint8_t *d_max_n, int64_t B, int64_t c, int64_t H, int64_t W, int wavelet,
                                           int mode, int level, double q_scale, const double *channel_mults, uint8_t *d_img_out,
                                           const int64_t *out_strides, int32_t *d_rec) {
    return decode_image_batch_view(EL_U8, ctx, d_data, slot_stride, d_nbytes, d_max_n, B, c, H, W, wavelet, mode, level, q_scale,
                                   channel_mults, d_img_out, out_strides, d_rec);
}
extern "C" int spiht_decode_image_batch_u16(spiht_ctx *ctx, const uint8_t *d_data, uint64_t slot_stride, const uint64_t *d_nbytes,
                                            const uint8_t *d_max_n, int64_t B, int64_t c, int64_t H, int64_t W, int wavelet,
                                            int mode, int level, double q_scale, const double *channel_mults, uint16_t *d_img_out,
                                            const int64_t *out_strides, int32_t *d_rec) {
    return decode_image_batch_view(EL_U16, ctx, d_data, slot_stride, d_nbytes, d_max_n, B, c, H, W, wavelet, mode, level, q_scale,
                                   channel_mults, d_img_out, out_strides, d_rec);
}
extern "C" int spiht_decode_image_batch_flt(spiht_ctx *ctx, int kind, const uint8_t *d_data, uint64_t slot_stride,
                                            const uint64_t *d_nbytes, const uint8_t *d_max_n, int64_t B, int64_t c, int64_t H,
                                            int64_t W, int wavelet, int mode, int level, double q_scale,
                                            const double *channel_mults, void *d_img_out, const int64_t *out_strides,
                                            int32_t *d_rec) {
    return decode_image_batch_view(el_of_kind(kind), ctx, d_data, slot_stride, d_nbytes, d_max_n, B, c, H, W, wavelet, mode, level,
                                   q_scale, channel_mults, d_img_out, out_strides, d_rec);
}

static int encode_image_host(spiht_ctx *ctx, const Pic &img, int64_t c, int64_t H, int64_t W, int wavelet, int mode, int level,
                             double q_scale, const double *channel_mults, uint64_t max_bits, uint8_t *out, uint64_t out_cap,
                             uint64_t *out_nbits, uint8_t *max_n) {
    if (!ctx || !img.p || !out_nbits || !max_n || (!out && out_cap)) return SPIHT_ERR_ARG;
    ImgCall k;
// ... 352 lines not shown
```

spiht_amd/csrc/api_internal.h:

```cpp
#pragma once
#include "../../include/spiht_hip.h"

#include <math.h>
#include <stdio.h>
#include <stdlib.h>
#include <string.h>

#include <algorithm>
#include <cmath>
#include <mutex>
#include <string>
#include <vector>

#include "alloc.h"
#include "common.h"
#include "floatpx.h"
#include "rd.h"
#include "tiles.h"
#include "tileset.h"

#pragma GCC visibility push(hidden)

extern thread_local std::string g_hip_err;

// ... 188 lines not shown
        v.p = (char *)base;
        return v;
    }
};
static inline Pic dense_pic(const void *p, PicElem el, bool out = false) {
    Pic v;
    v.el = el;
    v.p = (char *)p;
    v.out = out;
    return v;
}
enum { PIC_NULL_FIRST = 1, PIC_IMG_ARGS = 2, PIC_EMPTY_OK = 4 };
int view_pic(Pic *v, const void *p, PicElem el, bool out, const int64_t *strides, int n, int64_t B, int64_t c, int64_t h,
             int64_t w, int rules = 0, int wavelet = 0, int mode = 0);
int check_view(PicElem el, int64_t B, int64_t c, int64_t H, int64_t W, const int64_t *strides, int output);

struct ImgCall {
    spiht_ctx *ctx = nullptr;
    int64_t B = 0, c = 0;
    int F = 0;
    ImgGeom ig;
    ImgGeom pig;
    double q = 0;
    Geom g;
    const double *d_mults = nullptr;
    std::unique_lock<std::recursive_mutex> lk;

    bool open(int *st, spiht_ctx *ctx_, int64_t B_, int64_t c_, int64_t H, int64_t W, int wavelet, int mode, int level, bool coded);
    bool reduce(int *st, int k, double q_scale);
    int enter(const double *channel_mults);
    template <class Fn> int chunks(Fn fn) const { return batch_chunks(B, c, fn); }
    void extents(const Pic &v, int64_t *h, int64_t *w) const {
        const ImgGeom &vg = v.out ? pig : ig;
        const bool rec = v.out && !v.strided;
        *h = rec ? vg.rec_H : vg.hs[0];
        *w = rec ? vg.rec_W : vg.ws[0];
    }
    uint64_t bytes(const Pic &v, int64_t nb) const {
        int64_t h, w;
        extents(v, &h, &w);
        return v.bytes(nb, c, h, w);
    }
    Pic at(const Pic &v, int64_t b0) const {
        int64_t h, w;
        extents(v, &h, &w);
        return v.at(b0, c, h, w);
    }
};

int dwt_forward(spiht_ctx *ctx, const Pic &in, int planes, int c, const ImgGeom &ig, int wavelet, int mode, double q,
                const double *d_mults, int32_t *d_coeffs, uint32_t *d_maxabs = nullptr);
int dwt_inverse(spiht_ctx *ctx, const int32_t *d_rec, int planes, int c, const ImgGeom &ig, int wavelet, double q,
                const double *d_mults, const Pic &out, int l_hi = -1, int l_lo = 1, const double *d_a_in = nullptr,
                const uint32_t *d_flags = nullptr);

int encode_image_batch(spiht_ctx *ctx, const Pic &in, int64_t B, int64_t c, int64_t H, int64_t W, int wavelet, int mode, int level,
                       double q_scale, const double *channel_mults, uint64_t max_bits, uint8_t *d_out, uint64_t slot_stride,
                       uint64_t *d_nbits, uint8_t *d_max_n, int32_t *d_coeffs);
int decode_image_batch(spiht_ctx *ctx, const uint8_t *d_data, uint64_t slot_stride, const uint64_t *d_nbytes, const uint8_t *d_max_n,
                       int64_t B, int64_t c, int64_t H, int64_t W, int wavelet, int mode, int level, double q_scale,
                       const double *channel_mults, const Pic &out, int32_t *d_rec, int reduce = 0);
int encode_image_batch_view(PicElem el, spiht_ctx *ctx, const void *d_img, const int64_t *strides, int64_t B, int64_t c, int64_t H,
                            int64_t W, int wavelet, int mode, int level, double q_scale, const double *channel_mults,
                            uint64_t max_bits, uint8_t *d_out, uint64_t slot_stride, uint64_t *d_nbits, uint8_t *d_max_n,
                            int32_t *d_coeffs);
int decode_image_batch_view(PicElem el, spiht_ctx *ctx, const uint8_t *d_data, uint64_t slot_stride, const uint64_t *d_nbytes,
                            const uint8_t *d_max_n, int64_t B, int64_t c, int64_t H, int64_t W, int wavelet, int mode, int level,
                            double q_scale, const double *channel_mults, void *d_img_out, const int64_t *out_strides,
                            int32_t *d_rec);

#pragma GCC visibility pop
```

spiht_amd/csrc/common.h:

```cpp
#pragma once
#include <hip/hip_runtime.h>
#include <stdint.h>

#define SPIHT_MAX_LEVELS 32
#define SPIHT_MAX_TAPS 20

struct FastDiv {
    uint32_t m, sh, d, pad;
};

static inline FastDiv fastdiv_make(uint32_t d) {
    FastDiv f;
    f.d = d;
    f.pad = 0;
    if (d < 2) { f.m = 0; f.sh = 0; return f; }
    uint32_t l = 0;
    while ((1ull << l) < d) l++;
    uint64_t m = ((1ull << 32) * ((1ull << l) - d)) / d + 1;
    f.m = (uint32_t)m;
    f.sh = l - 1;
    return f;
}

#ifdef __HIPCC__
// ... 40 lines not shown

#define ENT_A 0x80000000u
#define ENT_LEAF 0x40000000u
#define ENT_IDX 0x3FFFFFFFu

struct ListCaps {
    uint32_t lip, lsp, lis;
    uint32_t pad;
};

struct WideCtl {
    uint32_t bar_count, bar_gen;
    uint32_t go;
    uint32_t bad;
    uint32_t st[12];
    uint32_t tot[8];
    uint32_t bad_at;
    uint32_t pad[3];
};
struct WideArgs {
    WideCtl *ctl;
    uint64_t *desc;
    uint32_t maxchunks;
    uint32_t G;
    uint32_t solo;
    uint32_t pad;
};

struct EncArgs {
    Geom g;
    ListCaps caps;
    int32_t B;
    int32_t nslots;
    const int32_t *x;
    const uint8_t *dmsb;
    const uint8_t *lmsb;
    const uint32_t *maxabs;
    uint64_t max_bits;
    uint8_t *out;
    uint64_t slot_stride;
    uint64_t *out_nbits;
    uint8_t *out_maxn;
    uint32_t *lip0, *lip1, *lsp, *lis0, *lis1, *lis2;
    uint32_t *err;
    const WideCtl *redo;
    float log2_thresh[32];
};

#define IW_TH 24
#define IW_TW 128

struct L1Flags {
    uint32_t *p;
    int32_t off_h, off_w;
    int32_t band_h, band_w;
    int32_t hf1;
    int32_t gx, gy;
    int32_t pad;
};

struct DecArgs {
    Geom g;
    ListCaps caps;
    int32_t B;
    int32_t nslots;
    const uint8_t *data;
    uint64_t slot_stride;
    const uint64_t *nbytes;
    const uint8_t *max_n;
    int32_t *out;
    uint32_t *lip0, *lip1, *lsp_idx, *lis0, *lis1, *lis2;
    int32_t *lsp_val;
    uint32_t *err;
    uint32_t *lsp_count;
    L1Flags fl;
    uint32_t *tr_ent;
    uint8_t *tr_act;
    uint64_t tr_stride;
};

#define ENT_IDX_META 0x0FFFFFFFu
#define ENT_FILT_SHIFT 28
#define TR_NONE 0xFFu

struct MetaArgs {
    Geom g;
    int32_t level;
    int32_t pad;
    uint64_t rows;
    const uint32_t *tr_ent;
    const uint8_t *tr_act;
    const uint8_t *data;
    const int32_t *slices;
    int32_t *meta;
    const uint32_t *skey;
    const uint32_t *spos;
};

#define META_MAX_GEN 32
struct MetaBatchArgs {
    Geom g;
    int32_t level;
    int32_t nb;
    uint32_t tr_stride;
    uint32_t pad0;
    FastDiv div_tr;
// ... 53 lines not shown
    float lo_f[SPIHT_MAX_TAPS], hi_f[SPIHT_MAX_TAPS];
    int32_t color, pad2;
    Color3 col;
    PxView px;
    FastDivU dv_gx, dv_gy, dv_c;
    uint32_t gx, gy, nt;
    int32_t narrow;
    uint32_t in_pb;
    uint32_t in_rb, in_cb;
    uint32_t co_pb, co_rb;
    uint32_t ll_pb, ll_rb;
    uint32_t pad3;
};

static inline bool dwt_narrow_ok(int64_t in_h, int64_t in_w, int64_t out_h, int64_t out_w, int64_t enc_h, int64_t enc_w, int px_es,
                                 int64_t px_sh, int64_t px_sw) {
    const int64_t lim = (int64_t)1 << 30;
    if (in_h < 1 || in_w < 1 || out_h < 1 || out_w < 1 || enc_h < 1 || enc_w < 1) return false;
    if (in_h >= lim || in_w >= lim || out_h >= lim / 16 || out_w >= lim / 16 || enc_h >= lim || enc_w >= lim) return false;
    if (px_es) {
        if (px_sh < 0 || px_sw < 0 || px_sh >= lim || px_sw >= lim) return false;
        if ((in_h - 1) * px_sh + (in_w - 1) * px_sw + px_es >= lim) return false;
    } else if (in_h * in_w * 8 >= lim) return false;
    if (enc_h * enc_w * 4 >= lim) return false;
    if (out_h * out_w * 8 >= lim) return false;
    if ((out_h + 64) * enc_w * 4 >= 2 * lim || (out_h + 64) * out_w * 8 >= 2 * lim) return false;
    return true;
}

struct TileCtr {
    uint32_t *dev;
    uint32_t base[8];
    int32_t wg_per_cu;
    int32_t num_cu;
    int32_t lds_per_cu;
    uint32_t started;
};
#define TILECTR_WORDS (9 * 32)
#define TILECTR_STARTED (8 * 32)
struct TileBase { uint32_t v[8]; };

struct IdwtKArgs {
    int32_t c;
    int32_t F;
    int32_t band_h, band_w;
    int32_t out_h, out_w;
    int32_t a_h, a_w;
    int32_t off_h, off_w, enc_h, enc_w;
    int32_t first;
    int32_t planes;
    const double *a_in;
    const int32_t *rec;
    const uint32_t *flags;
    double *out;
    const double *mults;
    double q;
    double lo[SPIHT_MAX_TAPS], hi[SPIHT_MAX_TAPS];
    int32_t color, pad2;
    Color3 col;
    PxView px;
};

struct LlPicArgs {
    const int32_t *rec;
    int32_t enc_h, enc_w, ll_h, ll_w;
    int32_t c, color;
    const double *mults;
    double q;
    double *out;
    PxView px;
    Color3 col;
};

extern "C" {
int spiht_launch_absmax(const int32_t *d_x, int B, uint32_t n, uint32_t *d_maxabs, hipStream_t st);
int spiht_launch_pyramid(const Geom *g, int B, const int32_t *d_x, uint8_t *d_dmsb, uint8_t *d_lmsb, hipStream_t st);
int spiht_launch_encode(const EncArgs *a, hipStream_t st);
int spiht_launch_encode_wide(const EncArgs *a, const WideArgs *w, int groups, hipStream_t st);
int spiht_wide_groups_per_cu(void);
int spiht_launch_decode(const DecArgs *a, hipStream_t st);
int spiht_launch_decode_w8(const DecArgs *a, hipStream_t st);
int spiht_launch_unscatter(const DecArgs *a, hipStream_t st);
int spiht_meta_sort_temp_bytes(uint64_t rows, size_t *bytes);
int spiht_launch_metadata(const MetaArgs *a, uint32_t *keys_in, uint32_t *vals_in, uint32_t *keys_out, uint32_t *vals_out,
                          void *temp, size_t temp_bytes, hipStream_t st);
int spiht_launch_budget_fold(const MetaArgs *a, uint32_t *keys_in, uint32_t *vals_in, uint32_t *keys_out, uint32_t *vals_out,
                             void *temp, size_t temp_bytes, const uint64_t *d_budgets, int K, int32_t *d_out, hipStream_t st);
int spiht_meta_batch_sort_temp_bytes(const MetaBatchArgs *a, size_t *bytes);
int spiht_launch_metadata_batch(const MetaBatchArgs *a, uint32_t *keys_in, uint32_t *vals_in, uint32_t *keys_out,
                                uint32_t *vals_out, void *temp, size_t temp_bytes, hipStream_t st);
int spiht_launch_nbits_to_nbytes(const uint64_t *d_nbits, int B, uint64_t *d_nbytes, hipStream_t st);
int spiht_launch_color3(const double *d_in, double *d_out, int B, size_t npix, const double *A, const double *M, double p,
                        hipStream_t st);
int spiht_launch_dwt_level(const DwtKArgs *a, int planes, hipStream_t st);
int spiht_launch_dwt_level_ext(const DwtKArgs *a, int planes, void *t_lo, void *t_hi, void *b_aa, void *b_ad, void *b_da,
                               void *b_dd, const double *d_filt, hipStream_t st);
int spiht_launch_idwt_level_per(const IdwtKArgs *a, int planes, double *t_lo, double *t_hi, const double *d_filt, int per,
                                hipStream_t st);
int spiht_launch_idwt_level(const IdwtKArgs *a, int planes, hipStream_t st, TileCtr *tc);
int spiht_launch_px_to_f64(const PxView *px, int64_t B, double *out, hipStream_t st);
int spiht_launch_f64_to_px(const double *in, int rec_h, int rec_w, const PxView *px, int64_t B, hipStream_t st);
int spiht_launch_quant_plain(const double *in, int32_t *out, size_t n_per_plane, int planes, int c, const double *mults,
                             double q, uint32_t *maxabs, hipStream_t st);
int spiht_launch_zero_pads(int L, const int64_t *hs, const int64_t *ws, const int64_t *offh, const int64_t *offw, int enc_h,
                           int enc_w, int32_t *coeffs, int planes, hipStream_t st);
int spiht_launch_ll_to_pic(const LlPicArgs *a, int planes, hipStream_t st);
// ... 7 lines not shown
```

spiht_amd/csrc/decode.hip:

```cpp
#include "common.h"

#ifndef DEC_NW
#define DEC_NW 12
#endif
#define DEC_NWK (DEC_NW - 2)
#define DEC_WK(wave) ((wave) - 2)
#define DEC_IS_WORKER(wave) ((wave) >= 2)
#define DEC_PREP 64
#define DEC_PREP_B 32
#ifndef DEC_RING
#define DEC_RING 64
#endif
static_assert((DEC_RING & (DEC_RING - 1)) == 0 && DEC_RING <= DEC_NW * 64, "ring: power of two, reset by one pass of the block");
#ifndef DEC_WSLEEP
#define DEC_WSLEEP 1
#endif
#define SEQ_OPEN 0xFFFFFFFFu
#define SPIN_LIMIT (1u << 24)

#ifdef DEC_PROF
#define PF_ADD(k) do { uint64_t _n = __builtin_amdgcn_s_memtime(); pf[k] += _n - pt; pt = _n; } while (0)
#define PF_CNT(k, v) pf[k] += (v)
#else
#define PF_ADD(k)
// ... 263 lines not shown
#endif
        while (__ballot(lds_load(&sh.wdone[w]) < need) != 0) {
            __builtin_amdgcn_s_sleep(1);
            if (++spins > SPIN_LIMIT) { sh.bad = 2; break; }
        }
#ifdef DEC_PROF
        if (pfw) *pfw += __builtin_amdgcn_s_memtime() - tws;
#endif
    }
}

__device__ __forceinline__ void seq_publish(DecShared &sh, uint32_t seq, uint32_t &fc, uint64_t fm, uint32_t e_start,
                                            uint32_t pos0, uint32_t pos1, uint32_t lane, uint32_t kw, uint64_t *pfw = nullptr) {
    if (fc == 0) seq_ring_check(sh, seq, fc, lane, kw, pfw);
    asm volatile("s_add_i32 %0, %0, -1" : "+s"(fc) : : "scc");
    if (lane == 0) {
        Slot *slot = &sh.ring[seq % DEC_RING];
        *reinterpret_cast<uint4 *>(slot) = make_uint4((uint32_t)fm, (uint32_t)(fm >> 32), e_start, pos0 | (pos1 << 8));
        asm volatile("" ::: "memory");
        __hip_atomic_store(&slot->ready, seq + 1, __ATOMIC_RELAXED, __HIP_MEMORY_SCOPE_WORKGROUP);
    }
}

__device__ __forceinline__ Item slot_unpack(DecShared &sh, const BitSrc &bs, uint32_t k) {
    const uint4 a = *reinterpret_cast<const uint4 *>(&sh.ring[k % DEC_RING]);
    const uint32_t seq0 = sh.ph.seq0;
    const uint32_t widx = sh.ph.widx0 + (k - seq0);
    Item it;
    it.kind = 1; it.cin = 0; it.m_rem = 0; it.b_nxt = 0;
    it.fm = (uint64_t)a.x | ((uint64_t)a.y << 32);
    it.e_start = a.z;
    it.pos0 = a.w & 0xFFu; it.pos1 = (a.w >> 8) & 0xFFu;
    it.first = k == seq0;
    it.b_lsp = sh.ph.b_lsp; it.b_lip = sh.ph.b_lip; it.b_ret = sh.ph.b_ret;
    it.Wb = widx << 6;
    const uint64_t *wb = sh.wbits[(k - seq0) % (DEC_PREP + DEC_RING)];
    it.lo = wb[0];
    it.hi = wb[1];
    return it;
}

struct Trace {
    uint32_t *ent;
    uint8_t *act;
    uint32_t nbits;
};
__device__ __forceinline__ void tr_put(const Trace &tr, uint32_t pos, uint32_t act, int n, uint32_t e) {
    if (pos <= tr.nbits) {
        tr.ent[pos] = e;
        tr.act[pos] = (uint8_t)(act | ((uint32_t)n << 3));
    }
}

__device__ __forceinline__ void l1_mark(const Geom &g, const L1Flags &f, uint32_t plane0, uint32_t idx) {
    uint32_t k, i, j;
    decomp(g, idx, k, i, j);
    if ((int)i < f.off_h && (int)j < f.off_w) return;
    const uint32_t bi = (int)i >= f.off_h ? i - (uint32_t)f.off_h : i, bj = (int)j >= f.off_w ? j - (uint32_t)f.off_w : j;
    if (bi >= (uint32_t)f.band_h || bj >= (uint32_t)f.band_w) return;
    constexpr uint32_t TR = IW_TH / 2, TC = IW_TW / 2;
    const uint32_t ty = bi / TR, tx = bj / TC;
    const bool up = bi - ty * TR < (uint32_t)f.hf1 && ty > 0, lf = bj - tx * TC < (uint32_t)f.hf1 && tx > 0;
    const uint32_t gx = (uint32_t)f.gx, gy = (uint32_t)f.gy;
    uint32_t *p = f.p + (size_t)(plane0 + k) * gy * gx;
    if (ty < gy && tx < gx) p[ty * gx + tx] = 1u;
    if (up && ty - 1u < gy && tx < gx) p[(ty - 1u) * gx + tx] = 1u;
    if (lf && ty < gy && tx - 1u < gx) p[ty * gx + tx - 1u] = 1u;
    if (up && lf && ty - 1u < gy && tx - 1u < gx) p[(ty - 1u) * gx + tx - 1u] = 1u;
}

__device__ __forceinline__ bool dup_cell(const Geom &g, uint32_t idx) {
    uint32_t k, i, j;
    decomp(g, idx, k, i, j);
    const uint32_t lh = (uint32_t)g.ll_h, lw = (uint32_t)g.ll_w;
    const int si = (int)__clz((int)lh) - (int)__clz((int)i), sj = (int)__clz((int)lw) - (int)__clz((int)j);
    const bool ri = (lh & 1u) && i >= lh && (i >> si) == lh, rj = (lw & 1u) && j >= lw && (j >> sj) == lw;
    if (!ri && !rj) return false;
    while (!((i >> 1) < lh && (j >> 1) < lw)) { i >>= 1; j >>= 1; }
    const bool io = i >= lh && (((i - lh) & ~1u) + 1u) < lh;
    const bool jo = j >= lw && (((j - lw) & ~1u) + 1u) < lw;
    return ((lh & 1u) && i == lh && jo) || ((lw & 1u) && j == lw && io);
}

__device__ __forceinline__ int32_t replay_dup(const uint32_t (&ts)[3], const int32_t (&vs)[3], int cnt, uint32_t ref_plane,
                                              uint32_t ref_count) {
    int nx[3] = {-1, -1, -1};
    uint32_t mag[3] = {0, 0, 0};
    int top = 0;
#pragma unroll
    for (int q = 0; q < 3; q++) {
        if (q < cnt) {
            mag[q] = (uint32_t)(vs[q] < 0 ? -vs[q] : vs[q]);
            nx[q] = 31 - (int)__clz((int)mag[q]);
            top = nx[q] > top ? nx[q] : top;
        }
    }
    int32_t cur = 0;
    for (int m = top; m >= 0; --m) {
#pragma unroll
        for (int q = 0; q < 3; q++)
            if (q < cnt && nx[q] == m) {
                const int32_t base = m == 0 ? 1 : (int32_t)(3u << (m - 1));
                cur = vs[q] < 0 ? -base : base;
            }
        if ((uint32_t)m >= ref_plane) {
#pragma unroll
            for (int q = 0; q < 3; q++)
                if (q < cnt && nx[q] > m && ((uint32_t)m > ref_plane || ts[q] < ref_count)) cur = set_bit_i32(cur, (uint32_t)m, (mag[q] >> m) & 1u);
        }
    }
    return cur;
}

__device__ __forceinline__ uint32_t ld_l2(const uint32_t *p) {
    return __hip_atomic_load(p, __ATOMIC_RELAXED, __HIP_MEMORY_SCOPE_AGENT);
}

template <uint32_t IDXM>
__device__ __forceinline__ void resolve_dups(const Geom &g, int32_t *out, const uint32_t *lsp_idx, const int32_t *lsp_val,
                                             uint32_t lsp_len, uint32_t *mailA, uint32_t *mailB, uint32_t ref_plane,
                                             uint32_t ref_count, const uint32_t *dlist, uint32_t ndup) {
// ... 1112 lines not shown
```

spiht_amd/csrc/dwt_inv.hip:

```cpp
#include "dwt_device.h"


template <int F, uint32_t LOM, uint32_t HIM, int PX = PX_F64>
__global__ __launch_bounds__(DW_BLOCK) void k_idwt_level(IdwtKArgs a) {
    constexpr int HF = F / 2;
    constexpr int KH = IW_TH / 2 + HF - 1;
    constexpr int KW = IW_TW / 2 + HF - 1;
    constexpr int KHH = IW_TH / 4 + HF - 1;
    __shared__ double s_b[4][KH][KW + 1];
    uint32_t tbx, tby, tbz;
    xcd_tile((a.out_w + IW_TW - 1) / IW_TW, (a.out_h + IW_TH - 1) / IW_TH, a.planes, tbx, tby, tbz);
    const int plane = (int)tbz;
    const int k = plane % a.c;
    const int m0 = (int)tby * IW_TH, n0 = (int)tbx * IW_TW;
    const int kh0 = m0 / 2, kw0 = n0 / 2;
    const bool has_m = a.mults != nullptr;
    const double mk = has_m ? a.mults[k] : 1.0;
    const bool zero_ok = (!has_m || mk > 0.0) && a.q > 0.0;
    const int32_t *__restrict__ rec = a.rec + (size_t)plane * a.enc_h * a.enc_w;
    const double *__restrict__ ain = a.first ? nullptr : a.a_in + (size_t)plane * a.a_h * a.a_w;
    const int tid = threadIdx.x;
    const bool occupied = a.flags == nullptr ||
        a.flags[((size_t)plane * ((a.out_h + IW_TH - 1) / IW_TH) + tby) * ((a.out_w + IW_TW - 1) / IW_TW) + tbx] != 0u;

    for (int p = tid; p < KH * KW; p += DW_BLOCK) {
        const int r = p / KW, cidx = p - r * KW;
        const int bi = kh0 + r, bj = kw0 + cidx;
        double vaa = 0.0, vad = 0.0, vda = 0.0, vdd = 0.0;
        if (bi < a.band_h && bj < a.band_w) {
            const int32_t rad = occupied ? rec[(size_t)bi * a.enc_w + a.off_w + bj] : 0;
            const int32_t rda = occupied ? rec[(size_t)(a.off_h + bi) * a.enc_w + bj] : 0;
            const int32_t rdd = occupied ? rec[(size_t)(a.off_h + bi) * a.enc_w + a.off_w + bj] : 0;
            if (a.first) {
                const int32_t raa = rec[(size_t)bi * a.enc_w + bj];
                vaa = (raa == 0 && zero_ok) ? 0.0 : dequant(raa, mk, a.q, has_m);
            } else {
                vaa = ain[(size_t)bi * a.a_w + bj];
            }
            vad = (rad == 0 && zero_ok) ? 0.0 : dequant(rad, mk, a.q, has_m);
            vda = (rda == 0 && zero_ok) ? 0.0 : dequant(rda, mk, a.q, has_m);
            vdd = (rdd == 0 && zero_ok) ? 0.0 : dequant(rdd, mk, a.q, has_m);
        }
        s_b[0][r][cidx] = vaa; s_b[1][r][cidx] = vad; s_b[2][r][cidx] = vda; s_b[3][r][cidx] = vdd;
    }
    __syncthreads();

    const int nn = tid & (IW_TW - 1), half = tid / IW_TW;
    const int n = n0 + nn;
    const int np = n & 1;
    const int cl = nn / 2;
    double tlo[HF], thi[HF];
#pragma unroll
    for (int s = 0; s < HF; s++) {
        tlo[s] = a.lo[np + F - 2 - 2 * s];
        thi[s] = a.hi[np + F - 2 - 2 * s];
    }
    double wl[HF], wh[HF];
#pragma unroll
    for (int s = 0; s < HF; s++) { wl[s] = 0.0; wh[s] = 0.0; }
    double *__restrict__ out = PX ? nullptr : a.out + (size_t)plane * a.out_h * a.out_w;
    uint8_t *__restrict__ out8 = PX ? a.px.out + (int64_t)(plane / a.c) * a.px.sb + (int64_t)(plane % a.c) * a.px.sc : nullptr;
    const int rbase = half * (IW_TH / 4);
#pragma unroll
    for (int rr = 0; rr < KHH; rr++) {
        const int r = rbase + rr;
        double ta = 0.0, td = 0.0, ua = 0.0, ud = 0.0;
#pragma unroll
        for (int j = 0; j < HF; j++) {
            const int s = HF - 1 - j;
            constexpr uint32_t PAIR = 3u;
            const bool lnz = ((LOM >> (F - 2 - 2 * s)) & PAIR) != 0, hnz = ((HIM >> (F - 2 - 2 * s)) & PAIR) != 0;
            if (lnz) {
                ta += s_b[0][r][cl + s] * tlo[s];
                ua += s_b[2][r][cl + s] * tlo[s];
            }
            if (hnz) {
                td += s_b[1][r][cl + s] * thi[s];
                ud += s_b[3][r][cl + s] * thi[s];
            }
        }
        const double tl = (0.0 + ta) + td, th = (0.0 + ua) + ud;
#pragma unroll
        for (int s = 0; s < HF - 1; s++) { wl[s] = wl[s + 1]; wh[s] = wh[s + 1]; }
        wl[HF - 1] = tl;
        wh[HF - 1] = th;
        if (rr >= HF - 1) {
            const int m = 2 * (kh0 + r - (HF - 1));
#pragma unroll
            for (int mp = 0; mp < 2; mp++) {
                double sa = 0.0, sd = 0.0;
#pragma unroll
                for (int j = 0; j < HF; j++) {
                    const int s = HF - 1 - j;
                    const bool lnz = (LOM >> (mp + F - 2 - 2 * s)) & 1u, hnz = (HIM >> (mp + F - 2 - 2 * s)) & 1u;
                    if (lnz) sa += wl[s] * a.lo[mp + F - 2 - 2 * s];
                    if (hnz) sd += wh[s] * a.hi[mp + F - 2 - 2 * s];
                }
                const double sacc = (0.0 + sa) + sd;
                if (PX) {
                    if (m + mp < a.px.h && n < a.px.w) PX_STORE(PX, out8, (int64_t)(m + mp) * a.px.sh + (int64_t)n * a.px.sw, sacc, a.px.kind);
                } else {
                    if (m + mp < a.out_h && n < a.out_w) out[(size_t)(m + mp) * a.out_w + n] = sacc;
                }
            }
        }
    }
}

#ifndef IWP_WG
#define IWP_WG 4
#endif

template <int F, uint32_t LOM, uint32_t HIM, bool FIRST, bool FLAGS = false, int PX = PX_F64>
__global__ __launch_bounds__(DW_BLOCK) void k_idwt_level_pf(IdwtKArgs a, uint32_t gx, uint32_t gy, uint32_t *ctr,
                                                                      TileBase cb) {
    static_assert(!(FIRST && FLAGS), "the flags are those of level 1 of a transform with two levels or more");
    constexpr int HF = F / 2;
    constexpr int KH = IW_TH / 2 + HF - 1, KW = IW_TW / 2 + HF - 1, KHH = IW_TH / 4 + HF - 1;
    constexpr int NE = (KH * KW + DW_BLOCK - 1) / DW_BLOCK;
    __shared__ double s_b[4][KH][KW + 1];
    const int tid = threadIdx.x;
    const uint32_t nt = gx * gy * (uint32_t)a.planes;
    const uint32_t x = blockIdx.x & 7u, q = nt >> 3, r8 = nt & 7u;
    const uint32_t base = x * q + (x < r8 ? x : r8), cnt = q + (x < r8 ? 1u : 0u);
    __shared__ uint32_t s_next[2];
    uint32_t *const myctr = ctr + 32u * x;
    const uint32_t cbase = cb.v[x];
    if (tid == 0) atomicAdd(ctr + TILECTR_STARTED, 1u);
    uint32_t k, kn;
    if (tid == 0) {
        s_next[0] = atomicAdd(myctr, 1u) - cbase;
        s_next[1] = atomicAdd(myctr, 1u) - cbase;
    }
    __syncthreads();
    k = __builtin_amdgcn_readfirstlane(s_next[0]);
    kn = __builtin_amdgcn_readfirstlane(s_next[1]);
    __syncthreads();

    struct Stage {
        int32_t rad[NE], rda[NE], rdd[NE], raa[NE];
        double vaa[NE];
        double mk;
    };
    auto request = [&](Stage &g, uint32_t T, uint32_t occ) {
        const uint32_t bx = T % gx, t2 = T / gx, by = t2 % gy, plane = t2 / gy;
        const int kh0 = (int)(by * IW_TH) / 2, kw0 = (int)(bx * IW_TW) / 2;
        const int32_t *__restrict__ rec = a.rec + (size_t)plane * a.enc_h * a.enc_w;
        const double *__restrict__ ain = FIRST ? nullptr : a.a_in + (size_t)plane * a.a_h * a.a_w;
        const __amdgpu_buffer_rsrc_t rrsrc = plane_rsrc(rec, (uint32_t)a.enc_h * (uint32_t)a.enc_w * 4u);
#pragma unroll
        for (int e = 0; e < NE; e++) {
            const int p = min(tid + e * DW_BLOCK, KH * KW - 1);
            const int rr = p / KW, cidx = p - rr * KW;
            const int bi = min(kh0 + rr, a.band_h - 1), bj = min(kw0 + cidx, a.band_w - 1);
            if (FLAGS) {
                const uint32_t o_ad = ((uint32_t)bi * (uint32_t)a.enc_w + (uint32_t)(a.off_w + bj)) * 4u;
                const uint32_t o_da = ((uint32_t)(a.off_h + bi) * (uint32_t)a.enc_w + (uint32_t)bj) * 4u;
                g.rad[e] = __builtin_amdgcn_raw_buffer_load_b32(rrsrc, occ ? o_ad : BUF_OOB, 0, 0);
                g.rda[e] = __builtin_amdgcn_raw_buffer_load_b32(rrsrc, occ ? o_da : BUF_OOB, 0, 0);
                g.rdd[e] = __builtin_amdgcn_raw_buffer_load_b32(rrsrc, occ ? o_da + (uint32_t)a.off_w * 4u : BUF_OOB, 0, 0);
            } else {
                g.rad[e] = rec[(size_t)bi * a.enc_w + a.off_w + bj];
                g.rda[e] = rec[(size_t)(a.off_h + bi) * a.enc_w + bj];
                g.rdd[e] = rec[(size_t)(a.off_h + bi) * a.enc_w + a.off_w + bj];
            }
            if (FIRST) { g.raa[e] = rec[(size_t)bi * a.enc_w + bj]; g.vaa[e] = 0.0; }
            else { g.vaa[e] = ain[(size_t)bi * a.a_w + bj]; g.raa[e] = 0; }
        }
        g.mk = a.mults != nullptr ? a.mults[plane % (uint32_t)a.c] : 1.0;
    };
    const int nn = tid & (IW_TW - 1), half = tid / IW_TW, np = nn & 1, cl = nn / 2;
    double tlo[HF], thi[HF];
#pragma unroll
    for (int s2 = 0; s2 < HF; s2++) {
        tlo[s2] = a.lo[np + F - 2 - 2 * s2];
        thi[s2] = a.hi[np + F - 2 - 2 * s2];
    }
    const bool has_m = a.mults != nullptr;
    auto tile = [&](Stage &g, uint32_t kk, uint32_t knext, uint32_t occ_next) {
        const uint32_t T = base + kk;
        const uint32_t bx = T % gx, t2 = T / gx, by = t2 % gy, plane = t2 / gy;
        const int kh0s = (int)(by * IW_TH) / 2, kw0s = (int)(bx * IW_TW) / 2;
        const double mk = g.mk;
        const bool zero_ok = (!has_m || mk > 0.0) && a.q > 0.0;
#pragma unroll
        for (int e = 0; e < NE; e++) {
            const int p = tid + e * DW_BLOCK;
            if (p < KH * KW) {
                const int rr = p / KW, cidx = p - rr * KW;
                const bool in = kh0s + rr < a.band_h && kw0s + cidx < a.band_w;
                const double va = FIRST ? ((g.raa[e] == 0 && zero_ok) ? 0.0 : dequant(g.raa[e], mk, a.q, has_m)) : g.vaa[e];
                s_b[0][rr][cidx] = in ? va : 0.0;
                s_b[1][rr][cidx] = (!in || (g.rad[e] == 0 && zero_ok)) ? 0.0 : dequant(g.rad[e], mk, a.q, has_m);
                s_b[2][rr][cidx] = (!in || (g.rda[e] == 0 && zero_ok)) ? 0.0 : dequant(g.rda[e], mk, a.q, has_m);
                s_b[3][rr][cidx] = (!in || (g.rdd[e] == 0 && zero_ok)) ? 0.0 : dequant(g.rdd[e], mk, a.q, has_m);
            }
        }
        uint32_t drawn = 0;
        if (tid == 0) drawn = atomicAdd(myctr, 1u);
        request(g, base + min(knext, cnt - 1u), occ_next);
        lds_barrier();
        const int m0 = (int)by * IW_TH, n0 = (int)bx * IW_TW, kh0 = m0 / 2;
        const int n = n0 + nn;
        double wl[HF], wh[HF];
#pragma unroll
        for (int s2 = 0; s2 < HF; s2++) { wl[s2] = 0.0; wh[s2] = 0.0; }
        const int rbase = half * (IW_TH / 4);
        const uint32_t row_bytes = (uint32_t)a.out_w * 8u;
        const __amdgpu_buffer_rsrc_t orsrc = PX ? plane_rsrc(a.px.out + (int64_t)(plane / (uint32_t)a.c) * a.px.sb + (int64_t)(plane % (uint32_t)a.c) * a.px.sc,
                                                             (uint32_t)((int64_t)(a.px.h - 1) * a.px.sh + (int64_t)(a.px.w - 1) * a.px.sw + (PX == PX_FLT ? a.px.es : PX)))
                                                : plane_rsrc(a.out + (size_t)plane * a.out_h * a.out_w, (uint32_t)a.out_h * row_bytes);
        const uint32_t voff0 = n < a.out_w ? (uint32_t)(2 * (kh0 + rbase)) * row_bytes + (uint32_t)n * 8u : BUF_OOB;
        const int y0 = 2 * (kh0 + rbase);
        const uint32_t voff8 = n < a.px.w ? (uint32_t)y0 * (uint32_t)a.px.sh + (uint32_t)n * (uint32_t)a.px.sw : BUF_OOB;
#pragma unroll
        for (int rr = 0; rr < KHH; rr++) {
            const int r = rbase + rr;
            double ta = 0.0, td = 0.0, ua = 0.0, ud = 0.0;
#pragma unroll
            for (int j = 0; j < HF; j++) {
                const int s2 = HF - 1 - j;
                constexpr uint32_t PAIR = 3u;
                const bool lnz = ((LOM >> (F - 2 - 2 * s2)) & PAIR) != 0, hnz = ((HIM >> (F - 2 - 2 * s2)) & PAIR) != 0;
                if (lnz) {
                    ta += s_b[0][r][cl + s2] * tlo[s2];
                    ua += s_b[2][r][cl + s2] * tlo[s2];
                }
                if (hnz) {
                    td += s_b[1][r][cl + s2] * thi[s2];
                    ud += s_b[3][r][cl + s2] * thi[s2];
                }
            }
            const double tl = (0.0 + ta) + td, th = (0.0 + ua) + ud;
#pragma unroll
            for (int s2 = 0; s2 < HF - 1; s2++) { wl[s2] = wl[s2 + 1]; wh[s2] = wh[s2 + 1]; }
            wl[HF - 1] = tl;
            wh[HF - 1] = th;
            if (rr >= HF - 1) {
#pragma unroll
                for (int mp = 0; mp < 2; mp++) {
                    double sa = 0.0, sd = 0.0;
#pragma unroll
                    for (int j = 0; j < HF; j++) {
                        const int s2 = HF - 1 - j;
                        const bool lnz = (LOM >> (mp + F - 2 - 2 * s2)) & 1u, hnz = (HIM >> (mp + F - 2 - 2 * s2)) & 1u;
                        if (lnz) sa += wl[s2] * a.lo[mp + F - 2 - 2 * s2];
                        if (hnz) sd += wh[s2] * a.hi[mp + F - 2 - 2 * s2];
                    }
                    const double sacc = (0.0 + sa) + sd;
                    if constexpr (PX == PX_U8) {
                        const int dy = 2 * (rr - (HF - 1)) + mp;
                        __builtin_amdgcn_raw_buffer_store_b8(px8_store_value(sacc), orsrc,
                                                             y0 + dy < a.px.h ? voff8 + (uint32_t)dy * (uint32_t)a.px.sh : BUF_OOB, 0, 0);
                    } else if constexpr (PX == PX_U16) {
                        const int dy = 2 * (rr - (HF - 1)) + mp;
                        __builtin_amdgcn_raw_buffer_store_b16(px16_store_value(sacc), orsrc,
                                                              y0 + dy < a.px.h ? voff8 + (uint32_t)dy * (uint32_t)a.px.sh : BUF_OOB, 0, 0);
                    } else if constexpr (PX == PX_FLT) {
                        const int dy = 2 * (rr - (HF - 1)) + mp;
                        const uint32_t b = flt_store_value(sacc, a.px.kind);
                        const uint32_t vo = y0 + dy < a.px.h ? voff8 + (uint32_t)dy * (uint32_t)a.px.sh : BUF_OOB;
                        __builtin_amdgcn_raw_buffer_store_b32(b, orsrc, a.px.kind == SPIHT_FLT_F32 ? vo : BUF_OOB, 0, 0);
                        __builtin_amdgcn_raw_buffer_store_b16((uint16_t)b, orsrc, a.px.kind == SPIHT_FLT_F32 ? BUF_OOB : vo, 0, 0);
                    } else {
                        __builtin_amdgcn_raw_buffer_store_b64(__builtin_bit_cast(u32x2, sacc), orsrc,
                                                              voff0 + (uint32_t)(2 * (rr - (HF - 1)) + mp) * row_bytes, 0, 0);
                    }
                }
            }
        }
        if (tid == 0) s_next[0] = drawn - cbase;
        lds_barrier();
    };
    Stage g0;
    if (k >= cnt) return;
    auto occupancy = [&](uint32_t kk) -> uint32_t {
        return FLAGS ? a.flags[base + min(kk, cnt - 1u)] : 1u;
    };
    request(g0, base + k, occupancy(k));
    uint32_t occ_n = occupancy(kn);
    tile(g0, k, kn, occ_n);
    k = kn;
    kn = __builtin_amdgcn_readfirstlane(s_next[0]);
    occ_n = occupancy(kn);
    while (k < cnt) {
        tile(g0, k, kn, occ_n);
        k = kn;
        kn = __builtin_amdgcn_readfirstlane(s_next[0]);
        occ_n = occupancy(kn);
    }
}

#define IWC_TH 8
template <int F, uint32_t LOM, uint32_t HIM, int PX = PX_F64>
__global__ __launch_bounds__(DW_BLOCK) void k_idwt1_color(IdwtKArgs a) {
    constexpr int HF = F / 2;
    constexpr int KH = IWC_TH / 2 + HF - 1, KW = IW_TW / 2 + HF - 1, KHH = IWC_TH / 4 + HF - 1;
    __shared__ double s_b[3][4][KH][KW + 1];
    __shared__ SpowLds s_pw;
    spow_lds_fill(s_pw, threadIdx.x);
    uint32_t tbx, tby, tbz;
    xcd_tile((a.out_w + IW_TW - 1) / IW_TW, (a.out_h + IWC_TH - 1) / IWC_TH, a.planes / 3, tbx, tby, tbz);
    const int img = (int)tbz;
    const int m0 = (int)tby * IWC_TH, n0 = (int)tbx * IW_TW;
    const int kh0 = m0 / 2, kw0 = n0 / 2;
    const bool has_m = a.mults != nullptr;
    const int tid = threadIdx.x;
    const size_t cpl = (size_t)a.enc_h * a.enc_w, apl = (size_t)a.a_h * a.a_w, opl = (size_t)a.out_h * a.out_w;

    for (int p = tid; p < 3 * KH * KW; p += DW_BLOCK) {
        const int ch = p / (KH * KW), q = p - ch * (KH * KW);
        const int r = q / KW, cidx = q - r * KW;
        const int bi = kh0 + r, bj = kw0 + cidx;
        const double mk = has_m ? a.mults[ch] : 1.0;
        const bool zero_ok = (!has_m || mk > 0.0) && a.q > 0.0;
        const int32_t *__restrict__ rec = a.rec + ((size_t)img * 3 + ch) * cpl;
        double vaa = 0.0, vad = 0.0, vda = 0.0, vdd = 0.0;
        if (bi < a.band_h && bj < a.band_w) {
            const int32_t rad = rec[(size_t)bi * a.enc_w + a.off_w + bj];
            const int32_t rda = rec[(size_t)(a.off_h + bi) * a.enc_w + bj];
            const int32_t rdd = rec[(size_t)(a.off_h + bi) * a.enc_w + a.off_w + bj];
            if (a.first) {
                const int32_t raa = rec[(size_t)bi * a.enc_w + bj];
                vaa = (raa == 0 && zero_ok) ? 0.0 : dequant(raa, mk, a.q, has_m);
            } else {
                vaa = a.a_in[((size_t)img * 3 + ch) * apl + (size_t)bi * a.a_w + bj];
            }
            vad = (rad == 0 && zero_ok) ? 0.0 : dequant(rad, mk, a.q, has_m);
            vda = (rda == 0 && zero_ok) ? 0.0 : dequant(rda, mk, a.q, has_m);
            vdd = (rdd == 0 && zero_ok) ? 0.0 : dequant(rdd, mk, a.q, has_m);
        }
        s_b[ch][0][r][cidx] = vaa; s_b[ch][1][r][cidx] = vad; s_b[ch][2][r][cidx] = vda; s_b[ch][3][r][cidx] = vdd;
    }
    __syncthreads();

    const int nn = tid & (IW_TW - 1), half = tid / IW_TW;
    const int n = n0 + nn, np = n & 1, cl = nn / 2;
    double tlo[HF], thi[HF];
#pragma unroll
    for (int s = 0; s < HF; s++) {
        tlo[s] = a.lo[np + F - 2 - 2 * s];
// ... 25 lines not shown
                if (hnz) {
                    td += s_b[ch][1][r][cl + s] * thi[s];
                    ud += s_b[ch][3][r][cl + s] * thi[s];
                }
            }
            const double tl = (0.0 + ta) + td, th = (0.0 + ua) + ud;
#pragma unroll
            for (int s = 0; s < HF - 1; s++) { wl[ch][s] = wl[ch][s + 1]; wh[ch][s] = wh[ch][s + 1]; }
            wl[ch][HF - 1] = tl;
            wh[ch][HF - 1] = th;
        }
        if (rr >= HF - 1) {
            const int m = 2 * (kh0 + r - (HF - 1));
#pragma unroll
            for (int mp = 0; mp < 2; mp++) {
                double px[3];
#pragma unroll
                for (int ch = 0; ch < 3; ch++) {
                    double sa = 0.0, sd = 0.0;
#pragma unroll
                    for (int j = 0; j < HF; j++) {
                        const int s = HF - 1 - j;
                        const bool lnz = (LOM >> (mp + F - 2 - 2 * s)) & 1u, hnz = (HIM >> (mp + F - 2 - 2 * s)) & 1u;
                        if (lnz) sa += wl[ch][s] * a.lo[mp + F - 2 - 2 * s];
                        if (hnz) sd += wh[ch][s] * a.hi[mp + F - 2 - 2 * s];
                    }
                    px[ch] = (0.0 + sa) + sd;
                }
                if (PX ? (m + mp < a.px.h && n < a.px.w) : (m + mp < a.out_h && n < a.out_w)) {
                    double w0, w1, w2;
                    color3_px(a.col, s_pw, px[0], px[1], px[2], w0, w1, w2);
                    if (PX) {
                        const int64_t o = (int64_t)(m + mp) * a.px.sh + (int64_t)n * a.px.sw;
                        PX_STORE(PX, out8, o, w0, a.px.kind);
                        PX_STORE(PX, out8, o + a.px.sc, w1, a.px.kind);
                        PX_STORE(PX, out8, o + 2 * a.px.sc, w2, a.px.kind);
                    } else {
                        const size_t o = (size_t)(m + mp) * a.out_w + n;
                        out[o] = w0;
                        out[o + opl] = w1;
                        out[o + 2 * opl] = w2;
                    }
                }
            }
        }
    }
}

template <int F, uint32_t LOM, uint32_t HIM, int PX>
static void launch_idwt_pf(IdwtKArgs &a, uint32_t G, uint32_t pad, hipStream_t st, uint32_t gx, uint32_t gy, uint32_t *ctr, const TileBase &cb) {
    if (a.first) hipLaunchKernelGGL((k_idwt_level_pf<F, LOM, HIM, true, false, PX>), dim3(G), dim3(DW_BLOCK), pad, st, a, gx, gy, ctr, cb);
    else if (a.flags && (uint64_t)a.enc_h * a.enc_w * 4u < (1ull << 31))
        hipLaunchKernelGGL((k_idwt_level_pf<F, LOM, HIM, false, true, PX>), dim3(G), dim3(DW_BLOCK), pad, st, a, gx, gy, ctr, cb);
    else { a.flags = nullptr; hipLaunchKernelGGL((k_idwt_level_pf<F, LOM, HIM, false, false, PX>), dim3(G), dim3(DW_BLOCK), pad, st, a, gx, gy, ctr, cb); }
}
template <int F, uint32_t LOM, uint32_t HIM>
static int launch_idwt_FM(IdwtKArgs a, int planes, hipStream_t st, TileCtr *tc) {
    a.planes = planes;
    const int px = a.px.out == nullptr ? PX_F64 : px_kind_of(a.px);
    if (a.color) {
        uint32_t ntc = (uint32_t)((a.out_w + IW_TW - 1) / IW_TW) * (uint32_t)((a.out_h + IWC_TH - 1) / IWC_TH) * (uint32_t)(planes / 3);
        with_px(px, [&](auto PX) { hipLaunchKernelGGL((k_idwt1_color<F, LOM, HIM, PX>), dim3(ntc), dim3(DW_BLOCK), 0, st, a); });
        return (int)hipGetLastError();
    }
    const uint32_t gx = (uint32_t)((a.out_w + IW_TW - 1) / IW_TW), gy = (uint32_t)((a.out_h + IW_TH - 1) / IW_TH);
    const uint32_t nt = gx * gy * (uint32_t)planes;
    constexpr uint32_t pf_min = 20000u;
    const int num_cu = tc ? tc->num_cu : 0;
    const bool off32 = px ? (uint64_t)((a.px.h - 1) * a.px.sh + (a.px.w - 1) * a.px.sw) + (uint64_t)a.px.es < (1ull << 31)
                          : (uint64_t)(a.out_h + IW_TH) * a.out_w * 8u < (1ull << 31);
    if (tc && tc->dev && num_cu >= 2 && nt >= pf_min && off32) {
        const int g = tc->wg_per_cu > 0 ? tc->wg_per_cu : IWP_WG;
        const uint32_t G = (uint32_t)(num_cu * g);
        uint32_t pad = 0;
        if (g < IWP_WG && tc->lds_per_cu > 0) {
            constexpr int HFk = F / 2;
            constexpr uint32_t own = 4u * (IW_TH / 2 + HFk - 1) * (IW_TW / 2 + HFk) * 8u + 64u;
            const uint32_t want = (uint32_t)tc->lds_per_cu / (uint32_t)(g + 1) + 512u;
            if (want > own && want <= 65536u) pad = want - own;
        }
        TileBase cb;
        uint32_t *ctr = tc->dev;
        for (uint32_t x = 0; x < 8; x++) {
            cb.v[x] = tc->base[x];
            tc->base[x] += (nt >> 3) + (x < (nt & 7u) ? 1u : 0u) + 2u * ((G + 7u - x) >> 3);
        }
        tc->started += G;
        with_px(px, [&](auto PX) { launch_idwt_pf<F, LOM, HIM, PX>(a, G, pad, st, gx, gy, ctr, cb); });
        const hipError_t e = hipGetLastError();
        if (e != hipSuccess) {
            (void)hipMemsetAsync(tc->dev, 0, TILECTR_WORDS * sizeof(uint32_t), st);
            for (uint32_t x = 0; x < 8; x++) tc->base[x] = 0;
            tc->started = 0;
        }
        return (int)e;
    }
    with_px(px, [&](auto PX) { hipLaunchKernelGGL((k_idwt_level<F, LOM, HIM, PX>), dim3(nt), dim3(DW_BLOCK), 0, st, a); });
    return (int)hipGetLastError();
}
template <int F, uint32_t LOM, uint32_t HIM>
static int launch_idwt_F(const IdwtKArgs &a, int planes, hipStream_t st, TileCtr *tc) {
    uint32_t lom, him;
    tap_masks(a.lo, a.hi, F, lom, him);
    if (lom == LOM && him == HIM) return launch_idwt_FM<F, LOM, HIM>(a, planes, st, tc);
    return launch_idwt_FM<F, (1u << F) - 1u, (1u << F) - 1u>(a, planes, st, tc);
}

// ... 16 lines not shown
```

spiht_amd/csrc/pipeline.cpp:

```cpp
#include "../../include/spiht_hip.h"

#ifndef PIPE_DEC_WAVES
#define PIPE_DEC_WAVES 8
#endif

#include <stdlib.h>
#include <string.h>

#include <new>
#include <vector>

#define CHK(expr)                      \
    do {                               \
        int _s = (expr);               \
        if (_s != SPIHT_OK) return _s; \
    } while (0)

struct StepPics {
    void *p = nullptr;
    int es = 0;
    bool strided = false;
    int64_t st[4] = {0, 0, 0, 0};
    StepPics() = default;
    StepPics(const void *p_, int es_, const int64_t *strides = nullptr) : p(const_cast<void *>(p_)), es(es_), strided(strides != nullptr) {
        if (strides) memcpy(st, strides, sizeof(st));
    }
    const int64_t *strides() const { return strided ? st : nullptr; }
};

struct spiht_pipeline {
    int device = 0;
    int64_t B = 0, c = 0, H = 0, W = 0;
    int wavelet = 0, mode = 0, level = -1;
    double q = 1.0;
    std::vector<double> mults;
    uint64_t max_bits = 0, slot_stride = 0, flag_words = 0;
    int64_t ll_h = 0, ll_w = 0, enc_h = 0, enc_w = 0;
    spiht_ctx *Hc = nullptr, *Lc[2] = {nullptr, nullptr};
    bool owns_h = true;
    spiht_event *ev_a[2] = {nullptr, nullptr}, *ev_d[2] = {nullptr, nullptr}, *ev_i[2] = {nullptr, nullptr};
    spiht_event *ev_c = nullptr;
    double *approx = nullptr;
    int32_t *coeffs[2] = {nullptr, nullptr}, *rec[2] = {nullptr, nullptr};
    uint8_t *dmsb[2] = {nullptr, nullptr}, *lmsb[2] = {nullptr, nullptr};
    uint32_t *maxabs[2] = {nullptr, nullptr}, *flags[2] = {nullptr, nullptr};
    uint64_t *nbytes[2] = {nullptr, nullptr};
    bool used[2] = {false, false};
    uint64_t step = 0;
    bool pending = false;
    int pending_slot = 0;
    StepPics pending_out;
    bool color_on = false;
    double cAf[9], cMf[9], cAi[9], cMi[9], cpf = 1.0, cpi = 1.0;
    int poisoned = SPIHT_OK;
    const double *mp() const { return mults.empty() ? nullptr : mults.data(); }
};

struct HScope {
    spiht_pipeline *p;
    int64_t old_pads = 0, old_groups = 0;
    int old_on = 0;
    double oAf[9], oMf[9], oAi[9], oMi[9], opf = 1.0, opi = 1.0;
    int st = SPIHT_OK;
    explicit HScope(spiht_pipeline *pp) : p(pp) {
        st = spiht_ctx_lock(p->Hc);
        if (st != SPIHT_OK) { p = nullptr; return; }
        (void)spiht_ctx_get_option(p->Hc, "pads_persist", &old_pads);
        (void)spiht_ctx_get_option(p->Hc, "idwt_groups", &old_groups);
        (void)spiht_ctx_get_color3(p->Hc, &old_on, oAf, oMf, &opf, oAi, oMi, &opi);
        (void)spiht_ctx_set_option(p->Hc, "pads_persist", 1);
        (void)spiht_ctx_set_option(p->Hc, "idwt_groups", 3);
        if (p->color_on) st = spiht_ctx_set_color3(p->Hc, p->cAf, p->cMf, p->cpf, p->cAi, p->cMi, p->cpi);
        else st = spiht_ctx_set_color3(p->Hc, nullptr, nullptr, 1.0, nullptr, nullptr, 1.0);
    }
    ~HScope() {
        if (!p) return;
        (void)spiht_ctx_set_option(p->Hc, "pads_persist", old_pads);
        (void)spiht_ctx_set_option(p->Hc, "idwt_groups", old_groups);
        if (old_on) (void)spiht_ctx_set_color3(p->Hc, oAf, oMf, opf, oAi, oMi, opi);
        else (void)spiht_ctx_set_color3(p->Hc, nullptr, nullptr, 1.0, nullptr, nullptr, 1.0);
        (void)spiht_ctx_unlock(p->Hc);
    }
};

static void pipeline_free(spiht_pipeline *p) {
    if (!p) return;
    if (p->Hc) {
        (void)spiht_ctx_synchronize(p->Hc);
        for (int s = 0; s < 2; s++) {
            if (p->Lc[s]) (void)spiht_ctx_synchronize(p->Lc[s]);
            void *bufs[] = {p->coeffs[s], p->rec[s], p->dmsb[s], p->lmsb[s], p->maxabs[s], p->flags[s], p->nbytes[s]};
            for (void *b : bufs)
                if (b) (void)spiht_dev_free(p->Hc, b);
            spiht_event_destroy(p->ev_a[s]);
            spiht_event_destroy(p->ev_d[s]);
            spiht_event_destroy(p->ev_i[s]);
        }
    }
    if (p->Hc && p->approx) (void)spiht_dev_free(p->Hc, p->approx);
    spiht_event_destroy(p->ev_c);
    for (int s = 0; s < 2; s++)
        if (p->Lc[s]) spiht_ctx_destroy(p->Lc[s]);
    if (p->Hc && p->owns_h) spiht_ctx_destroy(p->Hc);
    delete p;
}

static int pipeline_create(spiht_ctx *h_ctx, int device, int64_t B, int64_t c, int64_t H, int64_t W, int wavelet, int mode, int level,
                           double q_scale, const double *channel_mults, uint64_t max_bits, spiht_pipeline **out) {
    if (!out || B < 1 || c < 1 || H < 1 || W < 1) return SPIHT_ERR_ARG;
    *out = nullptr;
    spiht_pipeline *p = new (std::nothrow) spiht_pipeline();
    if (!p) return SPIHT_ERR_NOMEM;
    p->Hc = h_ctx;
    p->owns_h = h_ctx == nullptr;
    p->device = device; p->B = B; p->c = c; p->H = H; p->W = W;
    p->wavelet = wavelet; p->mode = mode; p->level = level; p->q = q_scale;
    if (channel_mults) p->mults.assign(channel_mults, channel_mults + c);
    p->max_bits = max_bits == 0 ? SPIHT_MAX_BITS_UNLIMITED : max_bits;
    int st = spiht_geometry_mode(H, W, wavelet, mode, level, nullptr, &p->ll_h, &p->ll_w, &p->enc_h, &p->enc_w, nullptr, nullptr);
    if (st == SPIHT_OK) st = spiht_encode_bound(c, p->enc_h, p->enc_w, p->ll_h, p->ll_w, 0x3FFFFFFFu, p->max_bits, &p->slot_stride);
    if (st == SPIHT_OK) st = spiht_l1_flags_words(c, H, W, wavelet, mode, level, &p->flag_words);
    if (st != SPIHT_OK) { pipeline_free(p); return st; }
    if (p->slot_stride < 4) p->slot_stride = 4;
    if (!p->Hc && (st = spiht_ctx_create(device, &p->Hc)) != SPIHT_OK) { pipeline_free(p); return st; }
    const uint64_t n = (uint64_t)c * p->enc_h * p->enc_w;
    for (int s = 0; s < 2 && st == SPIHT_OK; s++) {
        if ((st = spiht_ctx_create(device, &p->Lc[s])) != SPIHT_OK) break;
        if ((st = spiht_ctx_set_decoder_waves(p->Lc[s], PIPE_DEC_WAVES)) != SPIHT_OK) break;
        if ((st = spiht_ctx_set_option(p->Lc[s], "wide_encode", 0)) != SPIHT_OK) break;
        if ((st = spiht_event_create(p->Hc, &p->ev_a[s])) != SPIHT_OK) break;
        if ((st = spiht_event_create(p->Lc[s], &p->ev_d[s])) != SPIHT_OK) break;
        if ((st = spiht_event_create(p->Hc, &p->ev_i[s])) != SPIHT_OK) break;
        struct { void **ptr; uint64_t bytes; } al[] = {
            {(void **)&p->coeffs[s], (uint64_t)B * n * 4}, {(void **)&p->rec[s], (uint64_t)B * n * 4},
            {(void **)&p->dmsb[s], (uint64_t)B * n},       {(void **)&p->lmsb[s], (uint64_t)B * n},
            {(void **)&p->maxabs[s], (uint64_t)B * 4},     {(void **)&p->nbytes[s], (uint64_t)B * 8},
            {(void **)&p->flags[s], (uint64_t)B * p->flag_words * 4}};
        for (auto &a : al) {
            if (a.bytes == 0) continue;
            if ((st = spiht_dev_alloc(p->Hc, a.bytes, a.ptr)) != SPIHT_OK) break;
        }
        if (st == SPIHT_OK) st = spiht_dev_memset(p->Hc, p->rec[s], 0, (uint64_t)B * n * 4);
    }
    if (st == SPIHT_OK) st = spiht_event_create(p->Hc, &p->ev_c);
    if (st == SPIHT_OK) {
        int64_t a_h = 0, a_w = 0;
        st = spiht_idwt_approx_shape(H, W, wavelet, level, &a_h, &a_w);
        if (st == SPIHT_OK && a_h > 0 && a_w > 0 && mode != SPIHT_MODE_PERIODIZATION)
            st = spiht_dev_alloc(p->Hc, (uint64_t)B * c * a_h * a_w * 8, (void **)&p->approx);
    }
    if (st == SPIHT_OK) st = spiht_ctx_synchronize(p->Hc);
    if (st != SPIHT_OK) { pipeline_free(p); return st; }
    *out = p;
    return SPIHT_OK;
}

extern "C" int spiht_pipeline_create(int device, int64_t B, int64_t c, int64_t H, int64_t W, int wavelet, int mode, int level,
                                     double q_scale, const double *channel_mults, uint64_t max_bits, spiht_pipeline **out) {
    return pipeline_create(nullptr, device, B, c, H, W, wavelet, mode, level, q_scale, channel_mults, max_bits, out);
}
extern "C" int spiht_pipeline_create_on(spiht_ctx *h_ctx, int device, int64_t B, int64_t c, int64_t H, int64_t W, int wavelet, int mode,
                                        int level, double q_scale, const double *channel_mults, uint64_t max_bits, spiht_pipeline **out) {
    if (!h_ctx) return SPIHT_ERR_ARG;
    return pipeline_create(h_ctx, device, B, c, H, W, wavelet, mode, level, q_scale, channel_mults, max_bits, out);
}

extern "C" void spiht_pipeline_destroy(spiht_pipeline *p) { pipeline_free(p); }

extern "C" int spiht_pipeline_info(spiht_pipeline *p, uint64_t *slot_stride, int64_t *rec_H, int64_t *rec_W) {
    if (!p) return SPIHT_ERR_ARG;
    if (slot_stride) *slot_stride = p->slot_stride;
    return spiht_geometry_mode(p->H, p->W, p->wavelet, p->mode, p->level, nullptr, nullptr, nullptr, nullptr, nullptr, rec_H, rec_W);
}

extern "C" int spiht_pipeline_contexts(spiht_pipeline *p, spiht_ctx **h, spiht_ctx **l0, spiht_ctx **l1) {
    if (!p) return SPIHT_ERR_ARG;
    if (h) *h = p->Hc;
    if (l0) *l0 = p->Lc[0];
    if (l1) *l1 = p->Lc[1];
    return SPIHT_OK;
}

extern "C" int spiht_pipeline_set_color3(spiht_pipeline *p, const double *A_f, const double *M_f, double p_f, const double *A_i,
                                         const double *M_i, double p_i) {
    if (!p) return SPIHT_ERR_ARG;
    if (!A_f) { p->color_on = false; return SPIHT_OK; }
    if (!M_f || !A_i || !M_i) return SPIHT_ERR_ARG;
    memcpy(p->cAf, A_f, sizeof(p->cAf)); memcpy(p->cMf, M_f, sizeof(p->cMf));
    memcpy(p->cAi, A_i, sizeof(p->cAi)); memcpy(p->cMi, M_i, sizeof(p->cMi));
    p->cpf = p_f; p->cpi = p_i;
    p->color_on = true;
    return SPIHT_OK;
}

static int queue_inverse_coarse(spiht_pipeline *p, int s) {
    CHK(spiht_ctx_wait_event(p->Hc, p->ev_d[s]));
    if (p->approx)
        CHK(spiht_idwt_coarse_batch_f64(p->Hc, p->rec[s], p->B, p->c, p->H, p->W, p->wavelet, p->mode, p->level, p->q, p->mp(), p->approx));
    CHK(spiht_event_record(p->ev_c, p->Hc));
    return SPIHT_OK;
}
static int queue_inverse_level1(spiht_pipeline *p, int s, const StepPics &out) {
    if (out.es == 2) {
        if (p->approx)
            CHK(spiht_idwt_level1_flags_batch_u16(p->Hc, p->rec[s], p->approx, p->flags[s], p->B, p->c, p->H, p->W, p->wavelet, p->mode,
                                                  p->level, p->q, p->mp(), (uint16_t *)out.p, out.strides()));
        else
            CHK(spiht_dequant_idwt_flags_batch_u16(p->Hc, p->rec[s], p->flags[s], p->B, p->c, p->H, p->W, p->wavelet, p->mode, p->level,
                                                   p->q, p->mp(), (uint16_t *)out.p, out.strides()));
    } else if (out.es == 1) {
        if (p->approx)
            CHK(spiht_idwt_level1_flags_batch_u8(p->Hc, p->rec[s], p->approx, p->flags[s], p->B, p->c, p->H, p->W, p->wavelet, p->mode,
                                                 p->level, p->q, p->mp(), (uint8_t *)out.p, out.strides()));
        else
            CHK(spiht_dequant_idwt_flags_batch_u8(p->Hc, p->rec[s], p->flags[s], p->B, p->c, p->H, p->W, p->wavelet, p->mode, p->level,
                                                  p->q, p->mp(), (uint8_t *)out.p, out.strides()));
    } else if (p->approx)
        CHK(spiht_idwt_level1_flags_batch_f64(p->Hc, p->rec[s], p->approx, p->flags[s], p->B, p->c, p->H, p->W, p->wavelet, p->mode,
                                              p->level, p->q, p->mp(), (double *)out.p));
    else
        CHK(spiht_dequant_idwt_flags_batch_f64(p->Hc, p->rec[s], p->flags[s], p->B, p->c, p->H, p->W, p->wavelet, p->mode, p->level,
                                               p->q, p->mp(), (double *)out.p));
    CHK(spiht_event_record(p->ev_i[s], p->Hc));
    CHK(spiht_ctx_wait_event(p->Lc[s], p->ev_i[s]));
    CHK(spiht_unscatter_lists_batch_i32(p->Lc[s], p->rec[s], p->B, p->c, p->enc_h, p->enc_w));
    return SPIHT_OK;
}
static int queue_inverse(spiht_pipeline *p, int s, const StepPics &out) {
    CHK(queue_inverse_coarse(p, s));
    return queue_inverse_level1(p, s, out);
}

static int submit_impl(spiht_pipeline *p, const StepPics &in, const StepPics &out, uint8_t *d_out, uint64_t *d_nbits, uint8_t *d_max_n,
                       spiht_comm *comm = nullptr, uint8_t *d_all_slots = nullptr, uint64_t *d_all_nbits = nullptr,
                       uint8_t *d_all_max_n = nullptr, int rank = 0) {
    const int s = (int)(p->step & 1), o = s ^ 1;
    spiht_ctx *L = p->Lc[s];
    if (in.es == 2)
        CHK(spiht_dwt_pyramid_batch_u16(p->Hc, (const uint16_t *)in.p, in.strides(), p->B, p->c, p->H, p->W, p->wavelet, p->mode, p->level,
                                        p->q, p->mp(), p->coeffs[s], p->dmsb[s], p->lmsb[s], p->maxabs[s]));
    else if (in.es == 1)
        CHK(spiht_dwt_pyramid_batch_u8(p->Hc, (const uint8_t *)in.p, in.strides(), p->B, p->c, p->H, p->W, p->wavelet, p->mode, p->level,
                                       p->q, p->mp(), p->coeffs[s], p->dmsb[s], p->lmsb[s], p->maxabs[s]));
    else
        CHK(spiht_dwt_pyramid_batch_f64(p->Hc, (const double *)in.p, p->B, p->c, p->H, p->W, p->wavelet, p->mode, p->level, p->q, p->mp(),
                                        p->coeffs[s], p->dmsb[s], p->lmsb[s], p->maxabs[s]));
    CHK(spiht_event_record(p->ev_a[s], p->Hc));
    if (p->used[o]) CHK(spiht_ctx_wait_event(L, p->ev_d[o]));
    CHK(spiht_ctx_wait_event(L, p->ev_a[s]));
    CHK(spiht_encode_lists_batch_i32(L, p->coeffs[s], p->dmsb[s], p->lmsb[s], p->maxabs[s], p->B, p->c, p->enc_h, p->enc_w, p->ll_h,
                                     p->ll_w, p->max_bits == SPIHT_MAX_BITS_UNLIMITED ? 0 : p->max_bits, d_out, p->slot_stride,
                                     d_nbits, d_max_n));
    const uint8_t *x_out = d_out;
    const uint64_t *x_nbits = d_nbits;
    const uint8_t *x_maxn = d_max_n;
    if (comm) {
        CHK(spiht_gather_streams(L, comm, d_out, d_nbits, d_max_n, p->B, p->slot_stride, d_all_slots, d_all_nbits, d_all_max_n));
        int world = 0;
        CHK(spiht_comm_info(comm, &world, nullptr, nullptr));
        uint64_t o_s = 0, o_n = 0, o_m = 0;
        CHK(spiht_gather_row_offsets(rank, world, p->B, p->slot_stride, &o_s, &o_n, &o_m));
        x_out = d_all_slots + o_s;
        x_nbits = (const uint64_t *)((const uint8_t *)d_all_nbits + o_n);
        x_maxn = d_all_max_n + o_m;
    }
    CHK(spiht_nbits_to_nbytes(L, x_nbits, p->B, p->nbytes[s]));
    if (p->pending) {
        CHK(queue_inverse_coarse(p, p->pending_slot));
        CHK(queue_inverse_level1(p, p->pending_slot, p->pending_out));
        p->pending = false;
        const void *ctr = nullptr;
        uint32_t target = 0;
        CHK(spiht_ctx_resident_ticket(p->Hc, &ctr, &target));
        CHK(spiht_ctx_wait_event(L, p->ev_c));
        CHK(spiht_ctx_wait_resident(L, ctr, target, 1000));
    }
    CHK(spiht_decode_lists_flags_batch_i32(L, x_out, p->slot_stride, p->nbytes[s], x_maxn, p->B, p->c, p->H, p->W, p->wavelet,
                                           p->mode, p->level, p->rec[s], p->flags[s]));
    CHK(spiht_event_record(p->ev_d[s], L));
    p->used[s] = true;
    p->pending = true;
    p->pending_slot = s;
    p->pending_out = out;
    p->step++;
    return SPIHT_OK;
}

extern "C" int spiht_pipeline_submit_gather(spiht_pipeline *p, const double *d_img, uint8_t *d_out, uint64_t *d_nbits,
                                            uint8_t *d_max_n, double *d_img_out, spiht_comm *comm, uint8_t *d_all_slots,
                                            uint64_t *d_all_nbits, uint8_t *d_all_max_n, int rank) {
    if (!p || !d_img || !d_out || !d_nbits || !d_max_n || !d_img_out) return SPIHT_ERR_ARG;
    if (comm && (!d_all_slots || !d_all_nbits || !d_all_max_n || rank < 0)) return SPIHT_ERR_ARG;
    if (p->poisoned != SPIHT_OK) return p->poisoned;
    HScope sc(p);
    int st = sc.st;
    if (st == SPIHT_OK)
        st = submit_impl(p, StepPics(d_img, 0), StepPics(d_img_out, 0), d_out, d_nbits, d_max_n, comm, d_all_slots, d_all_nbits,
                         d_all_max_n, rank);
    if (st != SPIHT_OK) p->poisoned = st;
    return st;
}

extern "C" int spiht_pipeline_submit(spiht_pipeline *p, const double *d_img, uint8_t *d_out, uint64_t *d_nbits, uint8_t *d_max_n,
                                     double *d_img_out) {
    return spiht_pipeline_submit_gather(p, d_img, d_out, d_nbits, d_max_n, d_img_out, nullptr, nullptr, nullptr, nullptr, 0);
}

static int submit_px(spiht_pipeline *p, int es, const void *d_img, const int64_t *in_strides, uint8_t *d_out, uint64_t *d_nbits,
                     uint8_t *d_max_n, void *d_img_out, const int64_t *out_strides) {
    if (!p || !d_img || !d_out || !d_nbits || !d_max_n || !d_img_out) return SPIHT_ERR_ARG;
    if (p->poisoned != SPIHT_OK) return p->poisoned;
    const auto check = es == 2 ? spiht_check_view_u16 : spiht_check_view_u8;
    if ((uintptr_t)d_img % (uintptr_t)es != 0 || (uintptr_t)d_img_out % (uintptr_t)es != 0) return SPIHT_ERR_ARG;
    if (in_strides) CHK(check(p->B, p->c, p->H, p->W, in_strides, 0));
    if (out_strides) CHK(check(p->B, p->c, p->H, p->W, out_strides, 1));
    HScope sc(p);
    int st = sc.st;
    if (st == SPIHT_OK) st = submit_impl(p, StepPics(d_img, es, in_strides), StepPics(d_img_out, es, out_strides), d_out, d_nbits, d_max_n);
    if (st != SPIHT_OK) p->poisoned = st;
    return st;
}
extern "C" int spiht_pipeline_submit_u8(spiht_pipeline *p, const uint8_t *d_img, const int64_t *in_strides, uint8_t *d_out,
                                        uint64_t *d_nbits, uint8_t *d_max_n, uint8_t *d_img_out, const int64_t *out_strides) {
    return submit_px(p, 1, d_img, in_strides, d_out, d_nbits, d_max_n, d_img_out, out_strides);
}
extern "C" int spiht_pipeline_submit_u16(spiht_pipeline *p, const uint16_t *d_img, const int64_t *in_strides, uint8_t *d_out,
                                         uint64_t *d_nbits, uint8_t *d_max_n, uint16_t *d_img_out, const int64_t *out_strides) {
    return submit_px(p, 2, d_img, in_strides, d_out, d_nbits, d_max_n, d_img_out, out_strides);
}

extern "C" int spiht_pipeline_flush(spiht_pipeline *p) {
// ... 23 lines not shown
```

Before: 33890 Mpixels/s.

## Add per-row occupancy masks from decoder to skip empty rows in level-1 IDWT

```diff
diff --git a/include/spiht_hip.h b/include/spiht_hip.h
--- a/include/spiht_hip.h
+++ b/include/spiht_hip.h
@@ -161,6 +161,9 @@
 int spiht_decode_lists_flags_batch_i32(spiht_ctx *ctx, const uint8_t *d_data, uint64_t slot_stride, const uint64_t *d_nbytes,
                                        const uint8_t *d_max_n, int64_t B, int64_t c, int64_t H, int64_t W, int wavelet,
                                        int mode, int level, int32_t *d_out_zeroed, uint32_t *d_flags);
+int spiht_decode_lists_rows_batch_i32(spiht_ctx *ctx, const uint8_t *d_data, uint64_t slot_stride, const uint64_t *d_nbytes,
+                                      const uint8_t *d_max_n, int64_t B, int64_t c, int64_t H, int64_t W, int wavelet,
+                                      int mode, int level, int32_t *d_out_zeroed, uint32_t *d_flags, uint32_t *d_rows);
 int spiht_dequant_idwt_flags_batch_f64(spiht_ctx *ctx, const int32_t *d_rec, const uint32_t *d_flags, int64_t B, int64_t c,
                                        int64_t H, int64_t W, int wavelet, int mode, int level, double q_scale,
                                        const double *channel_mults, double *d_img_out);
@@ -190,6 +193,17 @@
 int spiht_idwt_level1_flags_batch_u16(spiht_ctx *ctx, const int32_t *d_rec, const double *d_approx, const uint32_t *d_flags,
                                       int64_t B, int64_t c, int64_t H, int64_t W, int wavelet, int mode, int level, double q_scale,
                                       const double *channel_mults, uint16_t *d_img_out, const int64_t *out_strides);
+int spiht_idwt_level1_rows_batch_f64(spiht_ctx *ctx, const int32_t *d_rec, const double *d_approx, const uint32_t *d_flags,
+                                     const uint32_t *d_rows, int64_t B, int64_t c, int64_t H, int64_t W, int wavelet, int mode,
+                                     int level, double q_scale, const double *channel_mults, double *d_img_out);
+int spiht_idwt_level1_rows_batch_u8(spiht_ctx *ctx, const int32_t *d_rec, const double *d_approx, const uint32_t *d_flags,
+                                    const uint32_t *d_rows, int64_t B, int64_t c, int64_t H, int64_t W, int wavelet, int mode,
+                                    int level, double q_scale, const double *channel_mults, uint8_t *d_img_out,
+                                    const int64_t *out_strides);
+int spiht_idwt_level1_rows_batch_u16(spiht_ctx *ctx, const int32_t *d_rec, const double *d_approx, const uint32_t *d_flags,
+                                     const uint32_t *d_rows, int64_t B, int64_t c, int64_t H, int64_t W, int wavelet, int mode,
+                                     int level, double q_scale, const double *channel_mults, uint16_t *d_img_out,
+                                     const int64_t *out_strides);
 
 int spiht_color3_batch_f64(spiht_ctx *ctx, const double *d_in, double *d_out, int64_t B, int64_t npix, const double *A,
                            const double *M, double p);
diff --git a/spiht_amd/_lib.py b/spiht_amd/_lib.py
--- a/spiht_amd/_lib.py
+++ b/spiht_amd/_lib.py
@@ -75,6 +75,8 @@
     "spiht_hstream_create", "spiht_hstream_destroy", "spiht_hstream_info", "spiht_hstream_input", "spiht_hstream_decode_input",
     "spiht_hstream_submit", "spiht_hstream_next", "spiht_hstream_pending",
     "spiht_tile_cut_set", "spiht_tile_paste_set",
+    "spiht_decode_lists_rows_batch_i32", "spiht_idwt_level1_rows_batch_f64", "spiht_idwt_level1_rows_batch_u8",
+    "spiht_idwt_level1_rows_batch_u16",
 ]
 
 
@@ -172,6 +174,7 @@
         L.spiht_idwt_coarse_batch_f64.argtypes = [vp, vp, i64, i64, i64, i64, i32, i32, i32, C.c_double, vp, vp]
         L.spiht_idwt_level1_batch_f64.argtypes = [vp, vp, vp, i64, i64, i64, i64, i32, i32, i32, C.c_double, vp, vp]
         L.spiht_idwt_level1_flags_batch_f64.argtypes = [vp, vp, vp, vp, i64, i64, i64, i64, i32, i32, i32, C.c_double, vp, vp]
+        L.spiht_idwt_level1_rows_batch_f64.argtypes = [vp, vp, vp, vp, vp, i64, i64, i64, i64, i32, i32, i32, C.c_double, vp, vp]
         L.spiht_idwt_approx_shape.argtypes = [i64, i64, i32, i32, C.POINTER(i64), C.POINTER(i64)]
         L.spiht_encode_image_host_f64.argtypes = [vp, vp, i64, i64, i64, i32, i32, i32, C.c_double, vp, u64, vp, u64,
                                                   C.POINTER(u64), C.POINTER(u8)]
@@ -196,6 +199,7 @@
         L.spiht_ctx_wide_stats.argtypes = [vp, C.POINTER(C.c_uint32), C.POINTER(C.c_uint32)]
         L.spiht_l1_flags_words.argtypes = [i64, i64, i64, i32, i32, i32, C.POINTER(u64)]
         L.spiht_decode_lists_flags_batch_i32.argtypes = [vp, vp, u64, vp, vp, i64, i64, i64, i64, i32, i32, i32, vp, vp]
+        L.spiht_decode_lists_rows_batch_i32.argtypes = L.spiht_decode_lists_flags_batch_i32.argtypes + [vp]
         L.spiht_geometry_mode.argtypes = [i64, i64, i32, i32, i32, C.POINTER(i32)] + [C.POINTER(i64)] * 6
         L.spiht_dequant_idwt_flags_batch_f64.argtypes = [vp, vp, vp, i64, i64, i64, i64, i32, i32, i32, C.c_double, vp, vp]
         L.spiht_pipeline_create.argtypes = [i32, i64, i64, i64, i64, i32, i32, i32, C.c_double, vp, u64, C.POINTER(vp)]
@@ -219,6 +223,7 @@
         L.spiht_dwt_pyramid_batch_u8.argtypes = [vp, vp, vp, i64, i64, i64, i64, i32, i32, i32, C.c_double, vp, vp, vp, vp, vp]
         L.spiht_dequant_idwt_flags_batch_u8.argtypes = [vp, vp, vp, i64, i64, i64, i64, i32, i32, i32, C.c_double, vp, vp, vp]
         L.spiht_idwt_level1_flags_batch_u8.argtypes = [vp, vp, vp, vp, i64, i64, i64, i64, i32, i32, i32, C.c_double, vp, vp, vp]
+        L.spiht_idwt_level1_rows_batch_u8.argtypes = [vp, vp, vp, vp, vp, i64, i64, i64, i64, i32, i32, i32, C.c_double, vp, vp, vp]
         L.spiht_pipeline_submit_u8.argtypes = [vp, vp, vp, vp, vp, vp, vp, vp]
         L.spiht_check_view_u8.argtypes = [i64, i64, i64, i64, vp, i32]
         L.spiht_reduced_shape.argtypes = [i64, i64, i32, i32, i32, i32, C.POINTER(i32)] + [C.POINTER(i64)] * 8
diff --git a/spiht_amd/csrc/api_coder.cpp b/spiht_amd/csrc/api_coder.cpp
--- a/spiht_amd/csrc/api_coder.cpp
+++ b/spiht_amd/csrc/api_coder.cpp
@@ -241,7 +241,10 @@
     a.tr_ent = d_tr_ent; a.tr_act = d_tr_act; a.tr_stride = tr_stride;
     if (fl && fl->p) {
         a.fl = *fl;
-        HIPCHK(hipMemsetAsync(fl->p, 0, (size_t)B * g.c * fl->gy * fl->gx * 4, ctx->stream));
+        const size_t wb = (size_t)B * g.c * fl->gy * fl->gx * 4;
+        const bool one = fl->rows == fl->p + wb / 4;
+        HIPCHK(hipMemsetAsync(fl->p, 0, one ? 2 * wb : wb, ctx->stream));
+        if (fl->rows && !one) HIPCHK(hipMemsetAsync(fl->rows, 0, wb, ctx->stream));
     }
     if (args_out) {
         CHK(ensure(ctx, ctx->lspcnt, (size_t)nslots * 4));
@@ -691,13 +694,20 @@
                                                   const uint64_t *d_nbytes, const uint8_t *d_max_n, int64_t B, int64_t c,
                                                   int64_t H, int64_t W, int wavelet, int mode, int level, int32_t *d_out_zeroed,
                                                   uint32_t *d_flags) {
+    return spiht_decode_lists_rows_batch_i32(ctx, d_data, slot_stride, d_nbytes, d_max_n, B, c, H, W, wavelet, mode, level,
+                                             d_out_zeroed, d_flags, nullptr);
+}
+extern "C" int spiht_decode_lists_rows_batch_i32(spiht_ctx *ctx, const uint8_t *d_data, uint64_t slot_stride,
+                                                 const uint64_t *d_nbytes, const uint8_t *d_max_n, int64_t B, int64_t c,
+                                                 int64_t H, int64_t W, int wavelet, int mode, int level, int32_t *d_out_zeroed,
+                                                 uint32_t *d_flags, uint32_t *d_rows) {
     if (!ctx || !d_data || !d_nbytes || !d_max_n || !d_out_zeroed || B < 0) return SPIHT_ERR_ARG;
     ImgCall k;
     int st;
     if (!k.open(&st, ctx, 1, c, H, W, wavelet, mode, level, true)) return st;
     L1Flags fl;
     const bool flagged = d_flags && l1flags_geometry(k.ig, k.F, &fl);
-    if (flagged) fl.p = d_flags;
+    if (flagged) { fl.p = d_flags; fl.rows = d_rows; }
     return decode_lists_batch(ctx, d_data, slot_stride, d_nbytes, d_max_n, B, k.g, d_out_zeroed, flagged ? &fl : nullptr);
 }
 
diff --git a/spiht_amd/csrc/api_dwt.cpp b/spiht_amd/csrc/api_dwt.cpp
--- a/spiht_amd/csrc/api_dwt.cpp
+++ b/spiht_amd/csrc/api_dwt.cpp
@@ -370,7 +370,8 @@
 }
 
 int dwt_inverse(spiht_ctx *ctx, const int32_t *d_rec, int planes, int c, const ImgGeom &ig, int wavelet, double q,
-                const double *d_mults, const Pic &out, int l_hi, int l_lo, const double *d_a_in, const uint32_t *d_flags) {
+                const double *d_mults, const Pic &out, int l_hi, int l_lo, const double *d_a_in, const uint32_t *d_flags,
+                const uint32_t *d_rows) {
     const WaveletDef &wv = SPIHT_WAVELETS[wavelet];
     const int F = wv.F;
     if (l_hi < 0) l_hi = ig.L;
@@ -427,7 +428,7 @@
         a.mults = d_mults;
         a.q = q;
         if (color && l == 1) { a.color = 1; a.col = ctx->col_inv; }
-        if (l == 1 && !a.first && !a.color) a.flags = d_flags;
+        if (l == 1 && !a.first && !a.color) { a.flags = d_flags; a.rows = d_flags ? d_rows : nullptr; }
         memcpy(a.lo, wv.rec_lo, sizeof(double) * std::min(F, SPIHT_MAX_TAPS));
         memcpy(a.hi, wv.rec_hi, sizeof(double) * std::min(F, SPIHT_MAX_TAPS));
         const bool conv8 = strided && l == 1 && (ig.per || F > SPIHT_MAX_TAPS);
diff --git a/spiht_amd/csrc/api_image.cpp b/spiht_amd/csrc/api_image.cpp
--- a/spiht_amd/csrc/api_image.cpp
+++ b/spiht_amd/csrc/api_image.cpp
@@ -79,7 +79,7 @@
 
 static int idwt_part(spiht_ctx *ctx, const int32_t *d_rec, double *d_approx, int64_t B, int64_t c, int64_t H, int64_t W,
                      int wavelet, int mode, int level, double q_scale, const double *channel_mults, const Pic &out,
-                     const uint32_t *d_flags = nullptr) {
+                     const uint32_t *d_flags = nullptr, const uint32_t *d_rows = nullptr) {
     if (!ctx || !d_rec || (!d_approx && !out.p)) return SPIHT_ERR_ARG;
     ImgCall k;
     int st;
@@ -100,8 +100,9 @@
         if (coarse)
             return dwt_inverse(ctx, rec, nb * (int)c, (int)c, ig, wavelet, q_scale, k.d_mults, dense_pic(ap, EL_F64, true), ig.L, 2,
                                nullptr);
+        const size_t w0 = flagged ? (size_t)b0 * c * fl.gy * fl.gx : 0;
         return dwt_inverse(ctx, rec, nb * (int)c, (int)c, ig, wavelet, q_scale, k.d_mults, k.at(out, b0), std::min(ig.L, 1), 1,
-                           ig.L >= 2 ? ap : nullptr, flagged ? d_flags + (size_t)b0 * c * fl.gy * fl.gx : nullptr);
+                           ig.L >= 2 ? ap : nullptr, flagged ? d_flags + w0 : nullptr, flagged && d_rows ? d_rows + w0 : nullptr);
     });
 }
 extern "C" int spiht_idwt_coarse_batch_f64(spiht_ctx *ctx, const int32_t *d_rec, int64_t B, int64_t c, int64_t H, int64_t W,
@@ -118,30 +119,50 @@
 extern "C" int spiht_idwt_level1_flags_batch_f64(spiht_ctx *ctx, const int32_t *d_rec, const double *d_approx, const uint32_t *d_flags,
                                                  int64_t B, int64_t c, int64_t H, int64_t W, int wavelet, int mode, int level,
                                                  double q_scale, const double *channel_mults, double *d_img_out) {
+    return spiht_idwt_level1_rows_batch_f64(ctx, d_rec, d_approx, d_flags, nullptr, B, c, H, W, wavelet, mode, level, q_scale,
+                                            channel_mults, d_img_out);
+}
+extern "C" int spiht_idwt_level1_rows_batch_f64(spiht_ctx *ctx, const int32_t *d_rec, const double *d_approx, const uint32_t *d_flags,
+                                                const uint32_t *d_rows, int64_t B, int64_t c, int64_t H, int64_t W, int wavelet,
+                                                int mode, int level, double q_scale, const double *channel_mults, double *d_img_out) {
     if (!d_img_out) return SPIHT_ERR_ARG;
     return idwt_part(ctx, d_rec, const_cast<double *>(d_approx), B, c, H, W, wavelet, mode, level, q_scale, channel_mults,
-                     dense_pic(d_img_out, EL_F64, true), d_flags);
-}
-static int idwt_level1_flags_view(PicElem el, spiht_ctx *ctx, const int32_t *d_rec, const double *d_approx, const uint32_t *d_flags,
-                                  int64_t B, int64_t c, int64_t H, int64_t W, int wavelet, int mode, int level, double q_scale,
-                                  const double *channel_mults, void *d_img_out, const int64_t *out_strides) {
+                     dense_pic(d_img_out, EL_F64, true), d_flags, d_rows);
+}
+static int idwt_level1_rows_view(PicElem el, spiht_ctx *ctx, const int32_t *d_rec, const double *d_approx, const uint32_t *d_flags,
+                                 const uint32_t *d_rows, int64_t B, int64_t c, int64_t H, int64_t W, int wavelet, int mode, int level,
+                                 double q_scale, const double *channel_mults, void *d_img_out, const int64_t *out_strides) {
     Pic out;
     CHK(view_pic(&out, d_img_out, el, true, out_strides, 4, B, c, H, W, PIC_NULL_FIRST));
     return idwt_part(ctx, d_rec, const_cast<double *>(d_approx), B, c, H, W, wavelet, mode, level, q_scale, channel_mults, out,
-                     d_flags);
+                     d_flags, d_rows);
+}
+extern "C" int spiht_idwt_level1_rows_batch_u8(spiht_ctx *ctx, const int32_t *d_rec, const double *d_approx, const uint32_t *d_flags,
+                                               const uint32_t *d_rows, int64_t B, int64_t c, int64_t H, int64_t W, int wavelet,
+                                               int mode, int level, double q_scale, const double *channel_mults, uint8_t *d_img_out,
+                                               const int64_t *out_strides) {
+    return idwt_level1_rows_view(EL_U8, ctx, d_rec, d_approx, d_flags, d_rows, B, c, H, W, wavelet, mode, level, q_scale,
+                                 channel_mults, d_img_out, out_strides);
+}
+extern "C" int spiht_idwt_level1_rows_batch_u16(spiht_ctx *ctx, const int32_t *d_rec, const double *d_approx, const uint32_t *d_flags,
+                                                const uint32_t *d_rows, int64_t B, int64_t c, int64_t H, int64_t W, int wavelet,
+                                                int mode, int level, double q_scale, const double *channel_mults,
+                                                uint16_t *d_img_out, const int64_t *out_strides) {
+    return idwt_level1_rows_view(EL_U16, ctx, d_rec, d_approx, d_flags, d_rows, B, c, H, W, wavelet, mode, level, q_scale,
+                                 channel_mults, d_img_out, out_strides);
 }
 extern "C" int spiht_idwt_level1_flags_batch_u8(spiht_ctx *ctx, const int32_t *d_rec, const double *d_approx, const uint32_t *d_flags,
                                                 int64_t B, int64_t c, int64_t H, int64_t W, int wavelet, int mode, int level,
                                                 double q_scale, const double *channel_mults, uint8_t *d_img_out,
                                                 const int64_t *out_strides) {
-    return idwt_level1_flags_view(EL_U8, ctx, d_rec, d_approx, d_flags, B, c, H, W, wavelet, mode, level, q_scale, channel_mults,
+    return idwt_level1_rows_view(EL_U8, ctx, d_rec, d_approx, d_flags, nullptr, B, c, H, W, wavelet, mode, level, q_scale, channel_mults,
                                   d_img_out, out_strides);
 }
 extern "C" int spiht_idwt_level1_flags_batch_u16(spiht_ctx *ctx, const int32_t *d_rec, const double *d_approx, const uint32_t *d_flags,
                                                  int64_t B, int64_t c, int64_t H, int64_t W, int wavelet, int mode, int level,
                                                  double q_scale, const double *channel_mults, uint16_t *d_img_out,
                                                  const int64_t *out_strides) {
-    return idwt_level1_flags_view(EL_U16, ctx, d_rec, d_approx, d_flags, B, c, H, W, wavelet, mode, level, q_scale, channel_mults,
+    return idwt_level1_rows_view(EL_U16, ctx, d_rec, d_approx, d_flags, nullptr, B, c, H, W, wavelet, mode, level, q_scale, channel_mults,
                                   d_img_out, out_strides);
 }
 
@@ -227,14 +248,16 @@
         L1Flags fl;
         const bool flagged = ctx->opt_l1_flags && reduce == 0 && !(ctx->color_on && c == 3) && l1flags_geometry(k.ig, k.F, &fl);
         if (flagged) {
-            CHK(ensure(ctx, ctx->l1flags, (size_t)nb * c * fl.gy * fl.gx * 4));
+            const size_t nw = (size_t)nb * c * fl.gy * fl.gx;
+            CHK(ensure(ctx, ctx->l1flags, 2 * nw * 4));
             fl.p = (uint32_t *)ctx->l1flags.p;
+            fl.rows = fl.p + nw;
         }
         if (rec) {
             CHK(decode_device(ctx, g, d_data + (size_t)b0 * slot_stride, slot_stride, d_nbytes + b0, d_max_n + b0, nb, rec,
                               nullptr, nullptr, 0, true, nullptr, flagged ? &fl : nullptr));
             return dwt_inverse(ctx, rec, nb * (int)c, (int)c, k.pig, wavelet, k.q, k.d_mults, k.at(out, b0), -1, 1, nullptr,
-                               flagged ? fl.p : nullptr);
+                               flagged ? fl.p : nullptr, flagged ? fl.rows : nullptr);
         }
         const size_t old_cap = ctx->recz.cap;
         CHK(ensure(ctx, ctx->recz, (size_t)nb * g.n * 4));
@@ -248,7 +271,7 @@
         CHK(decode_device(ctx, g, d_data + (size_t)b0 * slot_stride, slot_stride, d_nbytes + b0, d_max_n + b0, nb, rec, nullptr,
                           nullptr, 0, false, &da, flagged ? &fl : nullptr));
         CHK(dwt_inverse(ctx, rec, nb * (int)c, (int)c, k.pig, wavelet, k.q, k.d_mults, k.at(out, b0), -1, 1, nullptr,
-                        flagged ? fl.p : nullptr));
+                        flagged ? fl.p : nullptr, flagged ? fl.rows : nullptr));
         if (da.nslots >= nb) {
             StageTimer t(ctx, ST_MEMSET);
             LAUNCHCHK(spiht_launch_unscatter(&da, ctx->stream));
diff --git a/spiht_amd/csrc/api_internal.h b/spiht_amd/csrc/api_internal.h
--- a/spiht_amd/csrc/api_internal.h
+++ b/spiht_amd/csrc/api_internal.h
@@ -264,7 +264,7 @@
                 const double *d_mults, int32_t *d_coeffs, uint32_t *d_maxabs = nullptr);
 int dwt_inverse(spiht_ctx *ctx, const int32_t *d_rec, int planes, int c, const ImgGeom &ig, int wavelet, double q,
                 const double *d_mults, const Pic &out, int l_hi = -1, int l_lo = 1, const double *d_a_in = nullptr,
-                const uint32_t *d_flags = nullptr);
+                const uint32_t *d_flags = nullptr, const uint32_t *d_rows = nullptr);
 
 int encode_image_batch(spiht_ctx *ctx, const Pic &in, int64_t B, int64_t c, int64_t H, int64_t W, int wavelet, int mode, int level,
                        double q_scale, const double *channel_mults, uint64_t max_bits, uint8_t *d_out, uint64_t slot_stride,
diff --git a/spiht_amd/csrc/common.h b/spiht_amd/csrc/common.h
--- a/spiht_amd/csrc/common.h
+++ b/spiht_amd/csrc/common.h
@@ -116,6 +116,7 @@
 
 struct L1Flags {
     uint32_t *p;
+    uint32_t *rows;
     int32_t off_h, off_w;
     int32_t band_h, band_w;
     int32_t hf1;
@@ -275,6 +276,7 @@
     const double *a_in;
     const int32_t *rec;
     const uint32_t *flags;
+    const uint32_t *rows;
     double *out;
     const double *mults;
     double q;
diff --git a/spiht_amd/csrc/decode.hip b/spiht_amd/csrc/decode.hip
--- a/spiht_amd/csrc/decode.hip
+++ b/spiht_amd/csrc/decode.hip
@@ -339,6 +339,7 @@
     }
 }
 
+static_assert(IW_TH / 2 + IW_TH / 2 <= 32, "a tile's staged rows (IW_TH/2 + hf1, hf1 <= IW_TH/2) are the bits of one word");
 __device__ __forceinline__ void l1_mark(const Geom &g, const L1Flags &f, uint32_t plane0, uint32_t idx) {
     uint32_t k, i, j;
     decomp(g, idx, k, i, j);
@@ -354,6 +355,13 @@
     if (up && ty - 1u < gy && tx < gx) p[(ty - 1u) * gx + tx] = 1u;
     if (lf && ty < gy && tx - 1u < gx) p[ty * gx + tx - 1u] = 1u;
     if (up && lf && ty - 1u < gy && tx - 1u < gx) p[(ty - 1u) * gx + tx - 1u] = 1u;
+    if (f.rows == nullptr) return;
+    uint32_t *rw = f.rows + (size_t)(plane0 + k) * gy * gx;
+    const uint32_t own = 1u << (bi - ty * TR), above = own << TR;
+    if (ty < gy && tx < gx) atomicOr(rw + ty * gx + tx, own);
+    if (up && ty - 1u < gy && tx < gx) atomicOr(rw + (ty - 1u) * gx + tx, above);
+    if (lf && ty < gy && tx - 1u < gx) atomicOr(rw + ty * gx + tx - 1u, own);
+    if (up && lf && ty - 1u < gy && tx - 1u < gx) atomicOr(rw + (ty - 1u) * gx + tx - 1u, above);
 }
 
 __device__ __forceinline__ bool dup_cell(const Geom &g, uint32_t idx) {
diff --git a/spiht_amd/csrc/dwt_inv.hip b/spiht_amd/csrc/dwt_inv.hip
--- a/spiht_amd/csrc/dwt_inv.hip
+++ b/spiht_amd/csrc/dwt_inv.hip
@@ -1,5 +1,55 @@
 #include "dwt_device.h"
 
+
+#define IDWT_ROW(tl, th, r, full)                                                                             \
+    double tl, th;                                                                                            \
+    {                                                                                                         \
+        constexpr uint32_t PAIR_ = 3u;  \
+        double ta_ = 0.0, td_ = 0.0, ua_ = 0.0, ud_ = 0.0;                                                    \
+        if (full) {                                                                                           \
+            _Pragma("unroll") for (int j_ = 0; j_ < F / 2; j_++) {                                            \
+                const int s_ = F / 2 - 1 - j_;                                                                \
+                if (((LOM >> (F - 2 - 2 * s_)) & PAIR_) != 0) {                                               \
+                    ta_ += s_b[0][r][cl + s_] * tlo[s_];                                                      \
+                    ua_ += s_b[2][r][cl + s_] * tlo[s_];                                                      \
+                }                                                                                             \
+                if (((HIM >> (F - 2 - 2 * s_)) & PAIR_) != 0) {                                               \
+                    td_ += s_b[1][r][cl + s_] * thi[s_];                                                      \
+                    ud_ += s_b[3][r][cl + s_] * thi[s_];                                                      \
+                }                                                                                             \
+            }                                                                                                 \
+        } else {                                                                                              \
+            _Pragma("unroll") for (int j_ = 0; j_ < F / 2; j_++) {                                            \
+                const int s_ = F / 2 - 1 - j_;                                                                \
+                if (((LOM >> (F - 2 - 2 * s_)) & PAIR_) != 0) ta_ += s_b[0][r][cl + s_] * tlo[s_];            \
+            }                                                                                                 \
+        }                                                                                                     \
+        tl = (0.0 + ta_) + td_;                                                                               \
+        th = (0.0 + ua_) + ud_;                                                                               \
+    }
+template <int F, uint32_t LOM, uint32_t HIM>
+__device__ __forceinline__ double idwt_col(const double (&wl)[F / 2], const double (&wh)[F / 2], const double *lo, const double *hi,
+                                           int mp, bool full) {
+    constexpr int HF = F / 2;
+    double sa = 0.0, sd = 0.0;
+    if (full) {
+#pragma unroll
+        for (int j = 0; j < HF; j++) {
+            const int s = HF - 1 - j;
+            if ((LOM >> (mp + F - 2 - 2 * s)) & 1u) sa += wl[s] * lo[mp + F - 2 - 2 * s];
+            if ((HIM >> (mp + F - 2 - 2 * s)) & 1u) sd += wh[s] * hi[mp + F - 2 - 2 * s];
+        }
+    } else {
+#pragma unroll
+        for (int j = 0; j < HF; j++) {
+            const int s = HF - 1 - j;
+            if ((LOM >> (mp + F - 2 - 2 * s)) & 1u) sa += wl[s] * lo[mp + F - 2 - 2 * s];
+        }
+    }
+    return (0.0 + sa) + sd;
+}
+template <int F> constexpr bool IDWT_ROW_SKIP = F <= 10;
+__device__ __forceinline__ uint32_t half_rows(uint32_t mask, int rbase) { return __builtin_amdgcn_readfirstlane(mask >> rbase); }
 
 template <int F, uint32_t LOM, uint32_t HIM, int PX = PX_F64>
 __global__ __launch_bounds__(DW_BLOCK) void k_idwt_level(IdwtKArgs a) {
@@ -20,14 +70,15 @@
     const int32_t *__restrict__ rec = a.rec + (size_t)plane * a.enc_h * a.enc_w;
     const double *__restrict__ ain = a.first ? nullptr : a.a_in + (size_t)plane * a.a_h * a.a_w;
     const int tid = threadIdx.x;
-    const bool occupied = a.flags == nullptr ||
-        a.flags[((size_t)plane * ((a.out_h + IW_TH - 1) / IW_TH) + tby) * ((a.out_w + IW_TW - 1) / IW_TW) + tbx] != 0u;
+    const size_t ti = ((size_t)plane * ((a.out_h + IW_TH - 1) / IW_TH) + tby) * ((a.out_w + IW_TW - 1) / IW_TW) + tbx;
+    const uint32_t mask = a.flags == nullptr ? ~0u : a.rows != nullptr ? a.rows[ti] : a.flags[ti] != 0u ? ~0u : 0u;
 
     for (int p = tid; p < KH * KW; p += DW_BLOCK) {
         const int r = p / KW, cidx = p - r * KW;
         const int bi = kh0 + r, bj = kw0 + cidx;
         double vaa = 0.0, vad = 0.0, vda = 0.0, vdd = 0.0;
         if (bi < a.band_h && bj < a.band_w) {
+            const bool occupied = (mask >> r) & 1u;
             const int32_t rad = occupied ? rec[(size_t)bi * a.enc_w + a.off_w + bj] : 0;
             const int32_t rda = occupied ? rec[(size_t)(a.off_h + bi) * a.enc_w + bj] : 0;
             const int32_t rdd = occupied ? rec[(size_t)(a.off_h + bi) * a.enc_w + a.off_w + bj] : 0;
@@ -61,42 +112,21 @@
     double *__restrict__ out = PX ? nullptr : a.out + (size_t)plane * a.out_h * a.out_w;
     uint8_t *__restrict__ out8 = PX ? a.px.out + (int64_t)(plane / a.c) * a.px.sb + (int64_t)(plane % a.c) * a.px.sc : nullptr;
     const int rbase = half * (IW_TH / 4);
+    const uint32_t fm = IDWT_ROW_SKIP<F> ? half_rows(zero_ok ? mask : ~0u, rbase) : ~0u;
 #pragma unroll
     for (int rr = 0; rr < KHH; rr++) {
         const int r = rbase + rr;
-        double ta = 0.0, td = 0.0, ua = 0.0, ud = 0.0;
-#pragma unroll
-        for (int j = 0; j < HF; j++) {
-            const int s = HF - 1 - j;
-            constexpr uint32_t PAIR = 3u;
-            const bool lnz = ((LOM >> (F - 2 - 2 * s)) & PAIR) != 0, hnz = ((HIM >> (F - 2 - 2 * s)) & PAIR) != 0;
-            if (lnz) {
-                ta += s_b[0][r][cl + s] * tlo[s];
-                ua += s_b[2][r][cl + s] * tlo[s];
-            }
-            if (hnz) {
-                td += s_b[1][r][cl + s] * thi[s];
-                ud += s_b[3][r][cl + s] * thi[s];
-            }
-        }
-        const double tl = (0.0 + ta) + td, th = (0.0 + ua) + ud;
+        IDWT_ROW(tl, th, r, (fm >> rr) & 1u)
 #pragma unroll
         for (int s = 0; s < HF - 1; s++) { wl[s] = wl[s + 1]; wh[s] = wh[s + 1]; }
         wl[HF - 1] = tl;
         wh[HF - 1] = th;
         if (rr >= HF - 1) {
             const int m = 2 * (kh0 + r - (HF - 1));
+            const bool wfull = ((fm >> (rr - (HF - 1))) & ((1u << HF) - 1u)) != 0u;
 #pragma unroll
             for (int mp = 0; mp < 2; mp++) {
-                double sa = 0.0, sd = 0.0;
-#pragma unroll
-                for (int j = 0; j < HF; j++) {
-                    const int s = HF - 1 - j;
-                    const bool lnz = (LOM >> (mp + F - 2 - 2 * s)) & 1u, hnz = (HIM >> (mp + F - 2 - 2 * s)) & 1u;
-                    if (lnz) sa += wl[s] * a.lo[mp + F - 2 - 2 * s];
-                    if (hnz) sd += wh[s] * a.hi[mp + F - 2 - 2 * s];
-                }
-                const double sacc = (0.0 + sa) + sd;
+                const double sacc = idwt_col<F, LOM, HIM>(wl, wh, a.lo, a.hi, mp, wfull);
                 if (PX) {
                     if (m + mp < a.px.h && n < a.px.w) PX_STORE(PX, out8, (int64_t)(m + mp) * a.px.sh + (int64_t)n * a.px.sw, sacc, a.px.kind);
                 } else {
@@ -142,7 +172,9 @@
         double vaa[NE];
         double mk;
     };
-    auto request = [&](Stage &g, uint32_t T, uint32_t occ) {
+    auto rows_of = [&](uint32_t w) -> uint32_t { return !FLAGS ? ~0u : a.rows != nullptr ? w : w != 0u ? ~0u : 0u; };
+    auto request = [&](Stage &g, uint32_t T, uint32_t occw) {
+        const uint32_t occ = rows_of(occw);
         const uint32_t bx = T % gx, t2 = T / gx, by = t2 % gy, plane = t2 / gy;
         const int kh0 = (int)(by * IW_TH) / 2, kw0 = (int)(bx * IW_TW) / 2;
         const int32_t *__restrict__ rec = a.rec + (size_t)plane * a.enc_h * a.enc_w;
@@ -156,9 +188,10 @@
             if (FLAGS) {
                 const uint32_t o_ad = ((uint32_t)bi * (uint32_t)a.enc_w + (uint32_t)(a.off_w + bj)) * 4u;
                 const uint32_t o_da = ((uint32_t)(a.off_h + bi) * (uint32_t)a.enc_w + (uint32_t)bj) * 4u;
-                g.rad[e] = __builtin_amdgcn_raw_buffer_load_b32(rrsrc, occ ? o_ad : BUF_OOB, 0, 0);
-                g.rda[e] = __builtin_amdgcn_raw_buffer_load_b32(rrsrc, occ ? o_da : BUF_OOB, 0, 0);
-                g.rdd[e] = __builtin_amdgcn_raw_buffer_load_b32(rrsrc, occ ? o_da + (uint32_t)a.off_w * 4u : BUF_OOB, 0, 0);
+                const bool rd = __builtin_amdgcn_ubfe(occ, (uint32_t)rr, 1u) != 0u;
+                g.rad[e] = __builtin_amdgcn_raw_buffer_load_b32(rrsrc, rd ? o_ad : BUF_OOB, 0, 0);
+                g.rda[e] = __builtin_amdgcn_raw_buffer_load_b32(rrsrc, rd ? o_da : BUF_OOB, 0, 0);
+                g.rdd[e] = __builtin_amdgcn_raw_buffer_load_b32(rrsrc, rd ? o_da + (uint32_t)a.off_w * 4u : BUF_OOB, 0, 0);
             } else {
                 g.rad[e] = rec[(size_t)bi * a.enc_w + a.off_w + bj];
                 g.rda[e] = rec[(size_t)(a.off_h + bi) * a.enc_w + bj];
@@ -177,12 +210,13 @@
         thi[s2] = a.hi[np + F - 2 - 2 * s2];
     }
     const bool has_m = a.mults != nullptr;
-    auto tile = [&](Stage &g, uint32_t kk, uint32_t knext, uint32_t occ_next) {
+    auto tile = [&](Stage &g, uint32_t kk, uint32_t knext, uint32_t occw, uint32_t occ_next) {
         const uint32_t T = base + kk;
         const uint32_t bx = T % gx, t2 = T / gx, by = t2 % gy, plane = t2 / gy;
         const int kh0s = (int)(by * IW_TH) / 2, kw0s = (int)(bx * IW_TW) / 2;
         const double mk = g.mk;
         const bool zero_ok = (!has_m || mk > 0.0) && a.q > 0.0;
+        const uint32_t fmask = !FLAGS || !IDWT_ROW_SKIP<F> || !zero_ok ? ~0u : rows_of(occw);
 #pragma unroll
         for (int e = 0; e < NE; e++) {
             const int p = tid + e * DW_BLOCK;
@@ -191,9 +225,11 @@
                 const bool in = kh0s + rr < a.band_h && kw0s + cidx < a.band_w;
                 const double va = FIRST ? ((g.raa[e] == 0 && zero_ok) ? 0.0 : dequant(g.raa[e], mk, a.q, has_m)) : g.vaa[e];
                 s_b[0][rr][cidx] = in ? va : 0.0;
-                s_b[1][rr][cidx] = (!in || (g.rad[e] == 0 && zero_ok)) ? 0.0 : dequant(g.rad[e], mk, a.q, has_m);
-                s_b[2][rr][cidx] = (!in || (g.rda[e] == 0 && zero_ok)) ? 0.0 : dequant(g.rda[e], mk, a.q, has_m);
-                s_b[3][rr][cidx] = (!in || (g.rdd[e] == 0 && zero_ok)) ? 0.0 : dequant(g.rdd[e], mk, a.q, has_m);
+                if (!FLAGS || !IDWT_ROW_SKIP<F> || __builtin_amdgcn_ubfe(fmask, (uint32_t)rr, 1u) != 0u) {
+                    s_b[1][rr][cidx] = (!in || (g.rad[e] == 0 && zero_ok)) ? 0.0 : dequant(g.rad[e], mk, a.q, has_m);
+                    s_b[2][rr][cidx] = (!in || (g.rda[e] == 0 && zero_ok)) ? 0.0 : dequant(g.rda[e], mk, a.q, has_m);
+                    s_b[3][rr][cidx] = (!in || (g.rdd[e] == 0 && zero_ok)) ? 0.0 : dequant(g.rdd[e], mk, a.q, has_m);
+                }
             }
         }
         uint32_t drawn = 0;
@@ -206,6 +242,7 @@
 #pragma unroll
         for (int s2 = 0; s2 < HF; s2++) { wl[s2] = 0.0; wh[s2] = 0.0; }
         const int rbase = half * (IW_TH / 4);
+        const uint32_t fm = FLAGS && IDWT_ROW_SKIP<F> ? half_rows(fmask, rbase) : ~0u;
         const uint32_t row_bytes = (uint32_t)a.out_w * 8u;
         const __amdgpu_buffer_rsrc_t orsrc = PX ? plane_rsrc(a.px.out + (int64_t)(plane / (uint32_t)a.c) * a.px.sb + (int64_t)(plane % (uint32_t)a.c) * a.px.sc,
                                                              (uint32_t)((int64_t)(a.px.h - 1) * a.px.sh + (int64_t)(a.px.w - 1) * a.px.sw + (PX == PX_FLT ? a.px.es : PX)))
@@ -216,38 +253,16 @@
 #pragma unroll
         for (int rr = 0; rr < KHH; rr++) {
             const int r = rbase + rr;
-            double ta = 0.0, td = 0.0, ua = 0.0, ud = 0.0;
-#pragma unroll
-            for (int j = 0; j < HF; j++) {
-                const int s2 = HF - 1 - j;
-                constexpr uint32_t PAIR = 3u;
-                const bool lnz = ((LOM >> (F - 2 - 2 * s2)) & PAIR) != 0, hnz = ((HIM >> (F - 2 - 2 * s2)) & PAIR) != 0;
-                if (lnz) {
-                    ta += s_b[0][r][cl + s2] * tlo[s2];
-                    ua += s_b[2][r][cl + s2] * tlo[s2];
-                }
-                if (hnz) {
-                    td += s_b[1][r][cl + s2] * thi[s2];
-                    ud += s_b[3][r][cl + s2] * thi[s2];
-                }
-            }
-            const double tl = (0.0 + ta) + td, th = (0.0 + ua) + ud;
+            IDWT_ROW(tl, th, r, (fm >> rr) & 1u)
 #pragma unroll
             for (int s2 = 0; s2 < HF - 1; s2++) { wl[s2] = wl[s2 + 1]; wh[s2] = wh[s2 + 1]; }
             wl[HF - 1] = tl;
             wh[HF - 1] = th;
             if (rr >= HF - 1) {
+                const bool wfull = ((fm >> (rr - (HF - 1))) & ((1u << HF) - 1u)) != 0u;
 #pragma unroll
                 for (int mp = 0; mp < 2; mp++) {
-                    double sa = 0.0, sd = 0.0;
-#pragma unroll
-                    for (int j = 0; j < HF; j++) {
-                        const int s2 = HF - 1 - j;
-                        const bool lnz = (LOM >> (mp + F - 2 - 2 * s2)) & 1u, hnz = (HIM >> (mp + F - 2 - 2 * s2)) & 1u;
-                        if (lnz) sa += wl[s2] * a.lo[mp + F - 2 - 2 * s2];
-                        if (hnz) sd += wh[s2] * a.hi[mp + F - 2 - 2 * s2];
-                    }
-                    const double sacc = (0.0 + sa) + sd;
+                    const double sacc = idwt_col<F, LOM, HIM>(wl, wh, a.lo, a.hi, mp, wfull);
                     if constexpr (PX == PX_U8) {
                         const int dy = 2 * (rr - (HF - 1)) + mp;
                         __builtin_amdgcn_raw_buffer_store_b8(px8_store_value(sacc), orsrc,
@@ -274,19 +289,21 @@
     };
     Stage g0;
     if (k >= cnt) return;
-    auto occupancy = [&](uint32_t kk) -> uint32_t {
-        return FLAGS ? a.flags[base + min(kk, cnt - 1u)] : 1u;
-    };
-    request(g0, base + k, occupancy(k));
+    const uint32_t *const mw = FLAGS ? (a.rows != nullptr ? a.rows : a.flags) : nullptr;
+    auto occupancy = [&](uint32_t kk) -> uint32_t { return FLAGS ? mw[base + min(kk, cnt - 1u)] : 1u; };
+    uint32_t occ = occupancy(k);
+    request(g0, base + k, occ);
     uint32_t occ_n = occupancy(kn);
-    tile(g0, k, kn, occ_n);
+    tile(g0, k, kn, occ, occ_n);
     k = kn;
     kn = __builtin_amdgcn_readfirstlane(s_next[0]);
+    occ = occ_n;
     occ_n = occupancy(kn);
     while (k < cnt) {
-        tile(g0, k, kn, occ_n);
+        tile(g0, k, kn, occ, occ_n);
         k = kn;
         kn = __builtin_amdgcn_readfirstlane(s_next[0]);
+        occ = occ_n;
         occ_n = occupancy(kn);
     }
 }
@@ -418,7 +435,7 @@
     if (a.first) hipLaunchKernelGGL((k_idwt_level_pf<F, LOM, HIM, true, false, PX>), dim3(G), dim3(DW_BLOCK), pad, st, a, gx, gy, ctr, cb);
     else if (a.flags && (uint64_t)a.enc_h * a.enc_w * 4u < (1ull << 31))
         hipLaunchKernelGGL((k_idwt_level_pf<F, LOM, HIM, false, true, PX>), dim3(G), dim3(DW_BLOCK), pad, st, a, gx, gy, ctr, cb);
-    else { a.flags = nullptr; hipLaunchKernelGGL((k_idwt_level_pf<F, LOM, HIM, false, false, PX>), dim3(G), dim3(DW_BLOCK), pad, st, a, gx, gy, ctr, cb); }
+    else { a.flags = nullptr; a.rows = nullptr; hipLaunchKernelGGL((k_idwt_level_pf<F, LOM, HIM, false, false, PX>), dim3(G), dim3(DW_BLOCK), pad, st, a, gx, gy, ctr, cb); }
 }
 template <int F, uint32_t LOM, uint32_t HIM>
 static int launch_idwt_FM(IdwtKArgs a, int planes, hipStream_t st, TileCtr *tc) {
diff --git a/spiht_amd/csrc/pipeline.cpp b/spiht_amd/csrc/pipeline.cpp
--- a/spiht_amd/csrc/pipeline.cpp
+++ b/spiht_amd/csrc/pipeline.cpp
@@ -54,6 +54,7 @@
     double cAf[9], cMf[9], cAi[9], cMi[9], cpf = 1.0, cpi = 1.0;
     int poisoned = SPIHT_OK;
     const double *mp() const { return mults.empty() ? nullptr : mults.data(); }
+    uint32_t *rows(int s) const { return flags[s] ? flags[s] + (uint64_t)B * flag_words : nullptr; }
 };
 
 struct HScope {
@@ -135,7 +136,7 @@
             {(void **)&p->coeffs[s], (uint64_t)B * n * 4}, {(void **)&p->rec[s], (uint64_t)B * n * 4},
             {(void **)&p->dmsb[s], (uint64_t)B * n},       {(void **)&p->lmsb[s], (uint64_t)B * n},
             {(void **)&p->maxabs[s], (uint64_t)B * 4},     {(void **)&p->nbytes[s], (uint64_t)B * 8},
-            {(void **)&p->flags[s], (uint64_t)B * p->flag_words * 4}};
+            {(void **)&p->flags[s], 2 * (uint64_t)B * p->flag_words * 4}};
         for (auto &a : al) {
             if (a.bytes == 0) continue;
             if ((st = spiht_dev_alloc(p->Hc, a.bytes, a.ptr)) != SPIHT_OK) break;
@@ -203,20 +204,20 @@
 static int queue_inverse_level1(spiht_pipeline *p, int s, const StepPics &out) {
     if (out.es == 2) {
         if (p->approx)
-            CHK(spiht_idwt_level1_flags_batch_u16(p->Hc, p->rec[s], p->approx, p->flags[s], p->B, p->c, p->H, p->W, p->wavelet, p->mode,
+            CHK(spiht_idwt_level1_rows_batch_u16(p->Hc, p->rec[s], p->approx, p->flags[s], p->rows(s), p->B, p->c, p->H, p->W, p->wavelet, p->mode,
                                                   p->level, p->q, p->mp(), (uint16_t *)out.p, out.strides()));
         else
             CHK(spiht_dequant_idwt_flags_batch_u16(p->Hc, p->rec[s], p->flags[s], p->B, p->c, p->H, p->W, p->wavelet, p->mode, p->level,
                                                    p->q, p->mp(), (uint16_t *)out.p, out.strides()));
     } else if (out.es == 1) {
         if (p->approx)
-            CHK(spiht_idwt_level1_flags_batch_u8(p->Hc, p->rec[s], p->approx, p->flags[s], p->B, p->c, p->H, p->W, p->wavelet, p->mode,
+            CHK(spiht_idwt_level1_rows_batch_u8(p->Hc, p->rec[s], p->approx, p->flags[s], p->rows(s), p->B, p->c, p->H, p->W, p->wavelet, p->mode,
                                                  p->level, p->q, p->mp(), (uint8_t *)out.p, out.strides()));
         else
             CHK(spiht_dequant_idwt_flags_batch_u8(p->Hc, p->rec[s], p->flags[s], p->B, p->c, p->H, p->W, p->wavelet, p->mode, p->level,
                                                   p->q, p->mp(), (uint8_t *)out.p, out.strides()));
     } else if (p->approx)
-        CHK(spiht_idwt_level1_flags_batch_f64(p->Hc, p->rec[s], p->approx, p->flags[s], p->B, p->c, p->H, p->W, p->wavelet, p->mode,
+        CHK(spiht_idwt_level1_rows_batch_f64(p->Hc, p->rec[s], p->approx, p->flags[s], p->rows(s), p->B, p->c, p->H, p->W, p->wavelet, p->mode,
                                               p->level, p->q, p->mp(), (double *)out.p));
     else
         CHK(spiht_dequant_idwt_flags_batch_f64(p->Hc, p->rec[s], p->flags[s], p->B, p->c, p->H, p->W, p->wavelet, p->mode, p->level,
@@ -275,8 +276,8 @@
         CHK(spiht_ctx_wait_event(L, p->ev_c));
         CHK(spiht_ctx_wait_resident(L, ctr, target, 1000));
     }
-    CHK(spiht_decode_lists_flags_batch_i32(L, x_out, p->slot_stride, p->nbytes[s], x_maxn, p->B, p->c, p->H, p->W, p->wavelet,
-                                           p->mode, p->level, p->rec[s], p->flags[s]));
+    CHK(spiht_decode_lists_rows_batch_i32(L, x_out, p->slot_stride, p->nbytes[s], x_maxn, p->B, p->c, p->H, p->W, p->wavelet,
+                                          p->mode, p->level, p->rec[s], p->flags[s], p->rows(s)));
     CHK(spiht_event_record(p->ev_d[s], L));
     p->used[s] = true;
     p->pending = true;
```

New measurement: 35070 Mpixels/s (median of 6 runs). +3.5%, better.
